# K-Wu/HET

Hardware: AMD Instinct MI355X
Metric: million edges/s (fwd+bwd) RGAT layer, ogbn-mag feat=64 (higher is better)
Workload: dtype f32; 1 GPU; RGAT layer fwd+bwd, ogbn-mag-shaped synthetic graph (N=1939743, E=21111007, R=4), feat=64, heads=4, self_loop, no optimizer step, layer flags: default; LAYER SWAP: the model script builds het_amd.layers.HET_RGATLayer (the reference's layer class name and arguments); swapping only hrt/python/backend or only kernels/__init__.py under the reference's own model code gives variants.op_by_op / variants.; edge_order=src_dst, device=AMD Radeon Graphics, torch=2.10.0+rocm7.0, hip=7.0.51831, parallelism=single GPU

## Files before the change

het_amd/_lib.py:

```python
from __future__ import annotations

import ctypes as C
import os

_HERE = os.path.dirname(os.path.abspath(__file__))
LIB_PATH = os.environ.get("HET_AMD_LIB") or os.path.join(_HERE, "libhet_amd.so")

P, I64, INT, DBL = C.c_void_p, C.c_int64, C.c_int, C.c_double

_SIGNATURES = {
    "het_grouping_create": [P, I64, P, I64, I64, P, P, P, C.POINTER(P)],
    "het_grouping_rank_of_position": [P, P, P],
    "het_grouping_segment_map": [P, I64, P, P],
    "het_grouping_gather_payload1": [P, P, I64, P, P],
    "het_rows_add_bias": [P, P, P, P, I64, I64, P],
    "het_rows_gather": [P, P, I64, I64, P, P],
    "het_rows_scatter_add": [P, P, I64, I64, P, P],
    "het_rows_scatter_add_grouped": [P, P, I64, P, I64, P],
    "het_layout_separate_coo": [P, P, P, P, I64, I64, I64, P, P, P, P, P],
    "het_layout_coo_to_csr": [P, P, P, P, I64, I64, P, P, P, P, P],
    "het_layout_transpose_csr": [P, P, P, P, I64, I64, I64, P, P, P, P, P],
    "het_layout_unique_rel_nodes": [P, I64, P, P, I64, I64, P, P, P, P, P],
    "het_rgnn_relational_matmul": [I64, P, I64, P, P, I64, P, P, P, I64, I64, I64, INT, P, P, I64, P],
    "het_backward_rgnn_relational_matmul_attn_dot_only": [P, I64, P, P, I64, I64, P, P, P, P, P, P, I64, I64, I64, INT, P, P, I64, P, P, P],
    "het_rgnn_relational_matmul_attn_dot": [I64, P, I64, P, P, I64, P, P, P, P, P, I64, I64, I64, P, P, I64, P, P, P],
    "het_backward_rgnn_relational_matmul": [I64, P, I64, P, P, I64, I64, P, P, P, P, P, I64, I64, I64, INT, INT, P, P, I64, P],
    "het_rgnn_relational_matmul_no_scatter_gather_list": [P, I64, I64, P, P, P, I64, I64, I64, INT, P],
    "het_backward_rgnn_relational_matmul_no_scatter_gather_list": [P, I64, I64, P, P, P, P, P, I64, I64, I64, INT, INT, P],
    "het_relational_fused_gat_separate_coo": [P, P, P, P, I64, I64, I64, I64, P, P, P, P, P, P, P, P, P, P, P, I64, I64, DBL, P, P, P, P],
    "het_backward_relational_fused_gat_separate_coo": [P, P, P, P, I64, I64, I64, I64, P, P, P, P, P, P, P, P, P, P, P, P, P, P, P, I64, I64, DBL, P, P, P, I64, I64, P, I64, P, P, P, P, P],
    "het_relational_fused_gat_csr": [P, P, P, P, I64, I64, P, P, I64, P, P, P, P, P, P, I64, I64, DBL, INT, P],
    "het_backward_relational_fused_gat_csr": [P, P, P, P, I64, I64, P, P, I64, P, P, P, P, P, P, P, P, P, P, I64, I64, DBL, INT, P],
    "het_hgt_fold_source_weights": [P, P, P, P, P, P, I64, I64, I64, I64, I64, INT, P, P],
    "het_hgt_fold_source_weights_backward": [P, P, P, P, P, P, P, I64, I64, I64, I64, I64, INT, P, P, P, P, P, P],
    "het_rgat_aggregate_compact": [P, P, P, P, P, P, I64, I64, I64, DBL, P, I64, P, I64, P],
    "het_rows_matmul_backward_dx": [P, I64, P, P, I64, P, P, P, I64, I64, I64, INT, P],
    "het_rows_matmul_backward_dw": [P, I64, P, P, I64, P, P, P, I64, I64, I64, INT, P],
    "het_rows_matmul_backward_dw_colsum": [P, I64, P, P, I64, P, P, P, P, I64, I64, I64, INT, P],
    "het_rows_linear_bias": [P, P, P, P, P, I64, I64, I64, P],
    "het_node_row_map": [P, I64, P, I64, I64, P, P],
    "het_rgat_node_backward_dx": [I64, I64, I64, I64, I64, P, P, P, P, P, P, P, P, P, I64, I64, I64, P, P],
    "het_node_rows_matmul_sum": [I64, I64, I64, I64, P, P, P, P, P, P, I64, I64, P, P],
    "het_node_rows_matmul_sum_bias": [I64, I64, I64, I64, P, P, P, P, P, P, P, I64, I64, P, P],
    "het_rgcn_layer_forward": [P, I64, I64, P, P, P, P, P, P, P, P, P, I64, I64, P],
    "het_rgcn_layer_backward": [P, P, I64, I64, I64, P, P, P, P, P, P, P, P, P, P, I64, I64, P, I64, P],
    "het_rgcn_layer_forward_bf16": [P, I64, I64, P, P, P, P, P, P, P, P, P, I64, I64, P],
    "het_rgcn_layer_backward_bf16": [P, P, I64, I64, I64, P, P, P, P, P, P, P, P, P, P, I64, I64, P, I64, P],
    "het_rgat_backward_compact": [P, P, P, P, P, P, P, P, P, P, P, P, P, I64, P, I64, I64, I64, I64, I64, I64, DBL, P, I64, P],
    "het_rgat_aggregate_compact_runs": [P, P, I64, P, P, P, P, P, I64, I64, I64, DBL, P, I64, P, P, P, I64, P, P, P, I64, P],
    "het_rgat_backward_compact_runs": [P, P, P, P, P, P, P, P, P, P, P, P, P, P, P, P, I64, P, I64, I64, I64, I64, I64, I64, DBL, P, P, I64, P],
    "het_hgt_aggregate_compact": [P, P, P, P, P, I64, I64, I64, I64, P, I64, P],
    "het_hgt_backward_compact": [P, P, P, P, P, P, P, P, P, I64, I64, I64, I64, P, I64, P],
    "het_hgt_aggregate_compact_bf16": [P, P, P, P, P, I64, I64, I64, I64, P, I64, P],
    "het_hgt_backward_compact_bf16": [P, P, P, P, P, P, P, P, P, I64, I64, I64, I64, P, I64, P],
    "het_rows_matmul_bf16": [P, I64, P, P, I64, P, P, P, I64, I64, P],
    "het_rows_matmul_backward_dw_bf16": [P, I64, P, P, I64, P, P, P, I64, I64, INT, P],
    "het_rows_matmul_backward_dw_bf16_bf16": [P, I64, P, P, I64, P, P, P, I64, I64, INT, P],
    "het_node_rows_matmul_sum_bf16": [I64, I64, I64, I64, P, P, P, P, P, P, I64, I64, P, P],
    "het_rgcn_layer1_separate_coo": [P, P, P, P, I64, I64, I64, P, P, P, P, I64, I64, P, P, I64, P],
    "het_backward_rgcn_layer1_separate_coo": [P, P, P, P, I64, I64, I64, P, P, P, P, P, P, P, I64, I64, P, P, I64, P],
    "het_rgcn_node_mean_aggregation_compact_as_of_node_separate_coo": [P, P, P, P, I64, I64, I64, P, P, P, P, P, I64, INT, P, P],
    "het_backward_rgcn_node_mean_aggregation_compact_as_of_node_separate_coo": [P, P, P, P, I64, I64, I64, P, P, P, P, P, P, P, I64, INT, P, I64, P],
    "het_hgt_full_graph_edge_softmax_ops_separate_coo": [P, P, P, P, I64, I64, I64, P, P, P, P, P, I64, P, P],
    "het_backward_hgt_full_graph_enorm_to_unnormalized_attn_score_separate_coo": [P, P, P, P, I64, I64, I64, P, P, P, P, P, P, P, I64, P, P],
    "het_hgt_full_graph_edge_softmax_ops_csr": [P, I64, P, P, P, I64, I64, P, P, P, P, P, I64, P, P],
    "het_hgt_full_graph_message_mean_aggregation_csr": [P, I64, P, P, P, I64, I64, P, P, P, P, P, I64, I64, P, P],
    "het_backward_hgt_full_graph_message_mean_aggregation_csr": [P, I64, P, P, P, I64, I64, P, P, P, P, I64, I64, P],
    "het_backward_hgt_full_graph_edge_softmax_ops_csr": [P, I64, P, P, P, I64, I64, I64, P, P, P, P, P, P, P, P, I64, I64, P, P],
    "het_backward_hgt_full_graph_enorm_to_unnormalized_attn_score_csr": [P, I64, P, P, P, I64, I64, I64, P, P, P, P, P, P, I64, P, P, I64, P],
    "het_hgt_full_graph_fused_message_calc_and_mean_aggregation_separate_coo": [P, P, P, P, I64, I64, I64, P, P, P, P, I64, I64, I64, P, P, I64, P],
    "het_backward_hgt_full_graph_fused_message_calc_and_mean_aggregation_separate_coo": [P, P, P, P, I64, I64, I64, P, P, P, P, P, P, P, P, I64, I64, I64, P, P, I64, P],
    "het_rgnn_inner_product_right_node_separatecoo": [I64, P, P, P, P, P, P, I64, I64, P, P, P, I64, I64, P],
    "het_backward_inner_product_right_node_separatecoo": [I64, P, P, P, P, P, P, I64, I64, P, P, P, P, P, I64, I64, INT, P, P, I64, I64, P],
    "het_hgt_full_graph_hetero_attention_ops_coo": [P, P, P, P, I64, I64, P, P, P, P, P, I64, I64, I64, P],
    "het_backward_hgt_full_graph_hetero_attention_ops_coo": [P, P, P, P, I64, I64, P, P, P, P, P, P, P, P, I64, I64, I64, P, P, I64, P, I64, P],
}


class HetError(RuntimeError):
    pass


class HetUnsupported(HetError, NotImplementedError):
    """A configuration of the reference's model code that this build names but does not implement (the message says which
    reference op it would need and what to use instead) -- raised where the reference's name is reached, instead of an
    AttributeError from a missing function."""


_lib = None


def lib() -> C.CDLL:
    global _lib
    if _lib is None:
        if not os.path.exists(LIB_PATH):
            raise HetError(
                f"{LIB_PATH} not found: build the HIP library first (python -c 'import __graft_entry__ as g; g.build()' "
                "or make -C het_amd/csrc). het_amd has no CPU fallback.")
        L = C.CDLL(LIB_PATH)
        L.het_build_info.restype = C.c_char_p
        L.het_last_error.restype = C.c_char_p
        L.het_grouping_destroy.argtypes = [P]
        L.het_grouping_destroy.restype = None
        L.het_grouping_note_stream.argtypes = [P, P]
        L.het_grouping_note_stream.restype = None
        L.het_grouping_num_segments.argtypes = [P]
        L.het_grouping_num_segments.restype = I64
        L.het_grouping_bytes.argtypes = [P]
        L.het_grouping_bytes.restype = I64
        L.het_rgat_aggregate_compact_workspace.argtypes = [P, I64, I64]
        L.het_rgat_aggregate_compact_workspace.restype = I64
        L.het_rgat_aggregate_compact_runs_workspace.argtypes = [P, P, I64, I64, I64, P]
        L.het_rgat_aggregate_compact_runs_workspace.restype = I64
        L.het_rgat_backward_compact_runs_workspace.argtypes = [P, I64, I64, I64, I64, INT, INT, P]
        L.het_rgat_backward_compact_runs_workspace.restype = I64
        L.het_rgat_backward_compact_workspace.argtypes = [I64, I64, I64, I64, INT]
        L.het_rgat_backward_compact_workspace.restype = I64
        L.het_hgt_aggregate_compact_workspace.argtypes = [P, I64, I64]
        L.het_hgt_aggregate_compact_workspace.restype = I64
        L.het_hgt_backward_compact_workspace.argtypes = [I64, I64]
        L.het_hgt_backward_compact_workspace.restype = I64
        L.het_hgt_compact_shape_ok.argtypes = [I64, I64]
        L.het_hgt_compact_shape_ok.restype = INT
        L.het_node_rows_matmul_sum_ok.argtypes = [I64, I64, I64]
        L.het_node_rows_matmul_sum_ok.restype = INT
        L.het_rgcn_layer_ok.argtypes = [I64, I64, I64]
        L.het_rgcn_layer_ok.restype = INT
        L.het_rgcn_layer_backward_workspace.argtypes = [I64, I64]
        L.het_rgcn_layer_backward_workspace.restype = I64
        L.het_rgat_node_gemm_ok.argtypes = [I64, I64, I64, I64]
        L.het_rgat_node_gemm_ok.restype = INT
        L.het_set_allocator.argtypes = [P, P, P]
        L.het_set_allocator.restype = INT
        L.het_allocator_is_external.argtypes = []
        L.het_allocator_is_external.restype = INT
        L.het_kernel_timing_enable.argtypes = [INT]
        L.het_kernel_timing_enable.restype = INT
        L.het_kernel_timing_read.argtypes = [C.c_char_p, C.POINTER(C.c_double), C.POINTER(I64)]
        L.het_kernel_timing_read.restype = INT
        for name, args in _SIGNATURES.items():
            f = getattr(L, name, None)
            if f is None:
                raise HetError(f"{LIB_PATH} does not export {name}: rebuild it (make -C het_amd/csrc)")
            f.argtypes = args
            f.restype = INT
        _lib = L
    return _lib


_ALLOC_FN = C.CFUNCTYPE(C.c_void_p, C.c_size_t, C.c_void_p, C.c_void_p)
_FREE_FN = C.CFUNCTYPE(None, C.c_void_p, C.c_void_p)
_alloc_cbs = None


def use_torch_allocator(on: bool = True) -> bool:
    global _alloc_cbs
    L = lib()
    if not on:
        L.het_set_allocator(None, None, None)
        return False
    import torch

    def _alloc(nbytes, stream, _user):
        try:
            return int(torch.cuda.caching_allocator_alloc(int(nbytes), stream=int(stream or 0)))
        except BaseException:
            return None

    def _free(ptr, _user):
        try:
            torch.cuda.caching_allocator_delete(int(ptr))
        except BaseException:
            pass

    cbs = (_ALLOC_FN(_alloc), _FREE_FN(_free))
    rc = L.het_set_allocator(C.cast(cbs[0], C.c_void_p), C.cast(cbs[1], C.c_void_p), None)
    if rc != 0:
        raise HetError(f"het_set_allocator failed (code {rc}): {L.het_last_error().decode()}")
    _alloc_cbs = (_alloc_cbs or ()) + (cbs,)
    return True


def allocator_is_external() -> bool:
    return bool(lib().het_allocator_is_external())


def call(name: str, *args) -> None:
    L = lib()
    rc = getattr(L, name)(*args)
    if rc != 0:
        raise HetError(f"{name} failed (code {rc}): {L.het_last_error().decode()}")


def kernel_timing(on: bool) -> None:
    rc = lib().het_kernel_timing_enable(int(bool(on)))
    if rc != 0:
        raise HetError(f"het_kernel_timing_enable failed (code {rc})")


def kernel_timing_read(prefix: str):
    L = lib()
    ms, n = C.c_double(0.0), C.c_int64(0)
    rc = L.het_kernel_timing_read(prefix.encode(), C.byref(ms), C.byref(n))
    if rc != 0:
        raise HetError(f"het_kernel_timing_read failed (code {rc}): {L.het_last_error().decode()}")
    return ms.value, n.value


def build_info() -> str:
    return lib().het_build_info().decode()
```

het_amd/backend/rgat_fused_layer.py:

```python
import os

import torch as th

from ..plan import consistent as _consistent_plan

from .. import kernels as _k
from ..kernels import K


_OFFS = {}
PER_EDGE = os.environ.get("HET_RGAT_PER_EDGE") == "1"
LITERAL_ER = os.environ.get("HET_RGAT_LITERAL_ER") == "1"
OVERLAP = os.environ.get("HET_RGAT_OVERLAP", "1") != "0"


def _mulfirst_shape_ok(H, Kd):
    return H in (1, 2, 4, 8) and Kd >= 4 * H and Kd & (Kd - 1) == 0 and Kd <= 256


def _has_single_sided_lists(g):
    return "unique_node_indices_single_sided" in getattr(g, "graph_data", {}).get("separate", {})


def effective_flags(g, W, compact, direct, mulfirst):
    R, H, Kd, D = W.shape
    if not compact and not PER_EDGE and (_has_single_sided_lists(g) or hasattr(g, "generate_separate_unique_node_indices_single_sided_for_each_etype")):
        compact, direct = True, True
    if not mulfirst and not LITERAL_ER and _mulfirst_shape_ok(H, Kd):
        mulfirst = True
    return bool(compact), bool(direct), bool(mulfirst)


def _destinations_below(col, nd):
    return col.numel() == 0 or _k._derived_get("col_max", (col,), lambda: int(col.max())) < nd


def _lists(g):
    s = g.get_separate_coo_original()
    by_src = {"separate_coo_rel_ptrs": s["rel_ptrs"], "separate_coo_node_indices": s["row_indices"], "separate_coo_eids": s["eids"]}
    by_dst = {"separate_coo_rel_ptrs": s["rel_ptrs"], "separate_coo_node_indices": s["col_indices"], "separate_coo_eids": s["eids"]}
    return s, by_src, by_dst


def _compact_dicts(g, direct):
    ss = g.get_separate_unique_node_indices_single_sided()
    if direct:
        inv = g.get_separate_unique_node_indices_single_sided_inverse_idx()
        d = {"edata_idx_to_inverse_idx_row": inv["inverse_indices_row"], "edata_idx_to_inverse_idx_col": inv["inverse_indices_col"]}
        return ss, 4, d, d
    fwd = {"unique_srcs_and_dests_rel_ptrs": ss["rel_ptrs_row"], "unique_srcs_and_dests_rel_ptrs_col": ss["rel_ptrs_col"],
           "unique_srcs_and_dests_node_indices_row": ss["node_indices_row"],
           "unique_srcs_and_dests_node_indices_col": ss["node_indices_col"]}
    bwd = {"unique_srcs_and_dests_rel_ptrs": ss["rel_ptrs_row"], "unique_srcs_and_dests_rel_col": ss["rel_ptrs_col"],
           "unique_srcs_and_dests_node_indices_row": ss["node_indices_row"],
           "unique_srcs_and_dests_node_indices_col": ss["node_indices_col"]}
    return ss, 3, fwd, bwd


def _edge_rows(g, ss, direct, rp, row, col, eids):
    sep = getattr(g, "graph_data", {}).get("separate", {}).get("unique_node_indices_single_sided", {})
    if "inverse_indices_row" in sep and getattr(g, "sequential_eids_format", None) == "separate_coo":
        return sep["inverse_indices_row"], sep["inverse_indices_col"]
    maps = (ss["rel_ptrs_row"], ss["node_indices_row"], ss["rel_ptrs_col"], ss["node_indices_col"])
    return _k._src_rows_by_position(3, maps, rp, row, eids), _k._dst_rows_by_position(3, maps, rp, col, eids)


def rgat_layer_fused_ok(g, x, W, slope, compact, mulfirst=False):
    R, H, Kd, D = W.shape
    if not (_k._plan.is_enabled() and x.is_cuda and x.dim() == 2 and slope >= 0 and g.get_num_edges() > 0
            and _k.gat_grouped_shape_ok(H, D)):
        return False
    compact, _, mulfirst_eff = effective_flags(g, W, compact, True, mulfirst)
    if mulfirst and not _mulfirst_shape_ok(H, Kd):
        return False
    mulfirst = mulfirst_eff
    if not _k.matmul_attn_dot_ok(H, Kd, D):
        return compact and mulfirst and H & (H - 1) == 0
    if compact or mulfirst:
        return True
    _, _, by_dst = _lists(g)
    return _k.matmul_attn_dot_only_ok(by_dst, W, x)


_SIDE = {}


def _side_stream(dev):
    s = _SIDE.get(dev)
    if s is None:
        s = _SIDE[dev] = th.cuda.Stream(device=dev)
    return s


def _halo_pieces(g, ss, plan):
    key = ("halo_pieces", plan.chunks, plan.n_own, plan.n_halo)
    hit = g._plans.get(key)
    if hit is None:
        rp_row, nodes = ss["rel_ptrs_row"], ss["node_indices_row"]
        R = rp_row.numel() - 1
        rel = th.repeat_interleave(th.arange(R, device=nodes.device), rp_row[1:] - rp_row[:-1])
        cuts = [(0, plan.n_own + plan.halo_chunk_ptr[1])] + [(plan.n_own + plan.halo_chunk_ptr[c], plan.n_own + plan.halo_chunk_ptr[c + 1])
                                                             for c in range(1, plan.chunks)]
        hit = []
        for a, b in cuts:
            sel = th.nonzero((nodes >= a) & (nodes < b)).flatten()
            rp_c = th.zeros(R + 1, dtype=th.int64, device=nodes.device)
            rp_c[1:] = th.cumsum(th.bincount(rel[sel], minlength=R), 0)
            hit.append((rp_c, nodes[sel].contiguous(), sel.contiguous()))
        assert sum(int(h[2].numel()) for h in hit) == nodes.numel()
        g._plans[key] = hit
    return hit


@_consistent_plan
class RgatLayerFunction(th.autograd.Function):
    @staticmethod
    def forward(ctx, g, compact, direct, mulfirst, slope, num_dst, halo, x, W, attn_l, attn_r, loop_w, bias):
        x, W, attn_l, attn_r = x.contiguous(), W.contiguous(), attn_l.contiguous(), attn_r.contiguous()
        if halo is not None:
            assert compact and mulfirst and loop_w is not None, "rgat_layer_halo_ok guards this path"
            x = halo.start_push(x)
        s, by_src, by_dst = _lists(g)
        rp, row, col, eids = s["rel_ptrs"], s["row_indices"], s["col_indices"], s["eids"]
        E, N = eids.numel(), x.shape[0]
        R, H, Kd, D = W.shape
        X = H * D
        new = lambda *shape: th.empty(shape, dtype=x.dtype, device=x.device)
        sm, ret = new(N, H), new(N, H, D)
        nd = N if num_dst is None else min(int(num_dst), N)
        offs = h = None
        if loop_w is not None:
            loop_w = loop_w.contiguous()
            offs = _OFFS.get((nd, x.device))
            if offs is None:
                if len(_OFFS) > 64:
                    _OFFS.clear()
                offs = _OFFS[(nd, x.device)] = th.tensor([0, nd], dtype=th.int64, device=x.device)
        wa = None
        if mulfirst:
            wa = th.bmm(W.view(-1, Kd, D), attn_r.view(-1, D, 1)).view(R, H, Kd, 1)
        if compact:
            ss = g.get_separate_unique_node_indices_single_sided()
            d_row = {"unique_srcs_and_dests_rel_ptrs": ss["rel_ptrs_row"], "unique_srcs_and_dests_node_indices": ss["node_indices_row"]}
            d_col = {"unique_srcs_and_dests_rel_ptrs": ss["rel_ptrs_col"], "unique_srcs_and_dests_node_indices": ss["node_indices_col"]}
            featc = new(ss["node_indices_row"].numel(), H, D)
            elc = new(featc.shape[0], H)
            erc = new(ss["node_indices_col"].numel(), H)
            side = None
            fused_loop = loop_w is not None and _k.rows_linear_bias_ok(Kd, X)
            if OVERLAP and halo is None and fused_loop and mulfirst:
                main, side = th.cuda.current_stream(x.device), _side_stream(x.device)
                h = x.new_empty((nd, X))
                side.wait_stream(main)
            if mulfirst:
                with th.cuda.stream(side if side is not None else th.cuda.current_stream(x.device)):
                    K.rgnn_relational_matmul(d_col, 1, wa, x, erc.view(-1, H, 1), True)
                saved = (featc, elc, erc)
            else:
                featd = new(erc.shape[0], H, D)
                _k.matmul_attn_dot(d_col, 1, W, x, featd, attn_r, erc)
                saved = (featc, elc, erc, featd)
            if fused_loop:
                bias_c = None if bias is None else bias.contiguous()
                if side is not None:
                    with th.cuda.stream(side):
                        _k.rows_linear_bias(offs, x[:nd], loop_w, bias_c, out=h)
                else:
                    h = _k.rows_linear_bias(offs, x[:nd], loop_w, bias_c)
            dot_ok = _k.matmul_attn_dot_ok(H, Kd, D)
            piecewise = halo is not None and halo.chunks > 1 and dot_ok
            if piecewise:
                for c, (rp_c, nodes_c, rows_c) in enumerate(_halo_pieces(g, ss, halo.plan)):
                    halo.wait_push_piece(c)
                    _k.matmul_attn_dot_rows(rp_c, nodes_c, rows_c, W, x, featc, attn_l, elc)
                halo.finish_push()
            elif halo is not None:
                halo.finish_push()
            if piecewise:
                pass
            elif dot_ok:
                _k.matmul_attn_dot(d_row, 1, W, x, featc, attn_l, elc)
            else:
                K.rgnn_relational_matmul(d_row, 1, W, x, featc, True)
                K.rgnn_relational_matmul_no_scatter_gather_list(ss["rel_ptrs_row"], attn_l.unsqueeze(-1), featc, elc.view(-1, H, 1))
            if side is not None:
                th.cuda.current_stream(x.device).wait_stream(side)
            srow, drow = _edge_rows(g, ss, direct, rp, row, col, eids)
            run_sums = _k.rgat_runs_shape_ok(H, D)
            grp = _k.rgat_compact_groupings(col, srow, drow, N, featc.shape[0], erc.shape[0], rel_ptrs=rp if run_sums else None,
                                            drow_nodes=ss["node_indices_col"], drow_rel_ptrs=ss["rel_ptrs_col"])
            ctx.runs = _k.rgat_aggregate_compact(grp, featc, elc, erc, sm, ret, slope, h_inout=h, num_rels=R,
                                                 attn_l=attn_l.contiguous() if run_sums else None, feat_rel_ptrs=ss["rel_ptrs_row"] if run_sums else None)
            ctx.grp = grp
            ex = x.new_empty(0)
        else:
            rank = _k.gat_rank_of_position(rp, row, col, eids, N)
            by_dst_s = {"separate_coo_rel_ptrs": rp, "separate_coo_node_indices": col, "separate_coo_eids": rank}
            feat, el_s, er_s, exs = new(E, H, D), new(E, H), new(E, H), new(E, H)
            _k.matmul_attn_dot(by_src, 0, W, x, feat, attn_l, el_s, dot_rows=rank)
            if mulfirst:
                K.rgnn_relational_matmul(by_dst_s, 0, wa, x, er_s.view(E, H, 1), True)
                saved = (feat, exs)
            else:
                comp = _k.matmul_attn_dot(by_dst_s, 0, W, x, None, attn_r, er_s)
                assert comp is not None
                saved = (feat, exs, comp)
            used = _k.fused_gat_forward(eids, rp, row, col, 0, {}, feat, None, None, sm, None, ret, slope, exs,
                                        el_sorted=el_s, er_sorted=er_s)
            assert used
            ex = x.new_empty(0)
        if h is None:
            out = ret.view(N, X)[:nd]
            loop = None
            if loop_w is not None:
                loop = new(nd, X)
                K.rgnn_relational_matmul_no_scatter_gather_list(offs, loop_w.view(1, 1, Kd, X), x[:nd], loop)
            h = _k.rows_add_bias(out, loop, None if bias is None else bias.contiguous()) if (loop is not None or bias is not None) else out.clone()
        ctx.halo = halo
        ctx.g, ctx.compact, ctx.mulfirst, ctx.slope, ctx.nd = g, compact, mulfirst, slope, nd
        ctx.has_loop, ctx.has_bias = loop_w is not None, bias is not None
        ctx.save_for_backward(x, W, attn_l, attn_r, loop_w if loop_w is not None else x.new_empty(0), offs if offs is not None else eids,
                              sm, ex, ret, *saved)
        return h

    @staticmethod
    def backward(ctx, grad_h):
        x, W, attn_l, attn_r, loop_w, offs, sm, ex, ret, *saved = ctx.saved_tensors
        g, nd, slope = ctx.g, ctx.nd, ctx.slope
        s, by_src, by_dst = _lists(g)
        rp, row, col, eids = s["rel_ptrs"], s["row_indices"], s["col_indices"], s["eids"]
        N, Kd = x.shape
        E = eids.numel()
        R, H, _, D = W.shape
        X = H * D
        grad_h = grad_h.contiguous()
        if ctx.halo is not None:
            return RgatLayerFunction._backward_with_halo(ctx, grad_h)
        grad_bias = grad_h.sum(0) if (ctx.has_bias and not ctx.compact) else None
        Wt = th.transpose(W, 2, 3).contiguous()
        if ctx.compact and ctx.mulfirst and _k.rgat_node_gemm_ok(R, H, Kd, D) and _destinations_below(col, nd):
            return RgatLayerFunction._backward_node_major(ctx, grad_h, Wt)
        grad_W = th.zeros_like(W)
        grad_loop = None
        if ctx.has_loop:
            grad_x = th.empty_like(x) if nd == N else th.zeros_like(x)
            grad_loop = th.empty_like(loop_w)
            _k.matmul_no_scatter_gather_backward(offs, loop_w.view(1, 1, Kd, X).transpose(2, 3).contiguous(), x[:nd], grad_h,
                                                 grad_x[:nd], grad_loop.view(1, 1, Kd, X), accumulate=False)
        else:
            grad_x = th.zeros_like(x)
        dst_prefix = ctx.compact and _destinations_below(col, nd)
        if nd == N or dst_prefix:
            go = grad_h.view(nd, H, D)
        else:
            go = th.zeros((N, H, D), dtype=x.dtype, device=x.device)
            go.view(N, X)[:nd] = grad_h
        ndp = nd if dst_prefix else N
        mulfirst = ctx.mulfirst
        if mulfirst:
            wa_t = th.bmm(W.view(-1, Kd, D), attn_r.view(-1, D, 1)).view(R, H, 1, Kd)
            grad_wa = th.zeros((R, H, Kd, 1), dtype=x.dtype, device=x.device)
        if ctx.compact:
            featc, elc, erc = saved[:3]
            featd = None if mulfirst else saved[3]
            ss = g.get_separate_unique_node_indices_single_sided()
            d_row = {"unique_srcs_and_dests_rel_ptrs": ss["rel_ptrs_row"], "unique_srcs_and_dests_node_indices": ss["node_indices_row"]}
            d_col = {"unique_srcs_and_dests_rel_ptrs": ss["rel_ptrs_col"], "unique_srcs_and_dests_node_indices": ss["node_indices_col"]}
            g_featc, g_elc, g_erc = th.empty_like(featc), th.empty_like(elc), th.empty_like(erc)
            if ctx.has_bias:
                grad_bias = th.empty(X, dtype=x.dtype, device=x.device)
            _k.rgat_backward_compact(ctx.grp, featc, elc, erc, sm[:ndp], ret[:ndp], go, g_featc, g_elc, g_erc, slope, fold_attn_l=attn_l,
                                     row_rel_ptrs=ss["rel_ptrs_row"], grad_bias=grad_bias if ctx.has_bias else None, bias_rows=nd,
                                     runs=ctx.runs, drow_nodes=ss["node_indices_col"])
            grad_attn_l, grad_attn_r = th.empty_like(attn_l), th.empty_like(attn_r)
            _k.matmul_no_scatter_gather_backward(ss["rel_ptrs_row"], attn_l.unsqueeze(2), featc, g_elc, None,
                                                 grad_attn_l.unsqueeze(-1), accumulate=False)
            _k.matmul_backward(d_row, 1, Wt, x, g_featc, grad_x, grad_W, True, accumulate=True, distinct_rows=True)
            if mulfirst:
                _k.matmul_backward(d_col, 1, wa_t, x, g_erc.view(-1, H, 1), grad_x, grad_wa, True, accumulate=True, distinct_rows=True)
            else:
                g_featd = th.empty_like(featd)
                _k.matmul_no_scatter_gather_backward(ss["rel_ptrs_col"], attn_r.unsqueeze(2), featd, g_erc, g_featd,
                                                     grad_attn_r.unsqueeze(-1), accumulate=False)
                _k.matmul_backward(d_col, 1, Wt, x, g_featd, grad_x, grad_W, True, accumulate=True, distinct_rows=True)
        else:
            feat, exs = saved[:2]
            rank = _k.gat_rank_of_position(rp, row, col, eids, N)
            by_dst = {"separate_coo_rel_ptrs": rp, "separate_coo_node_indices": col, "separate_coo_eids": rank}
            g_feat, g_el = th.empty_like(feat), th.empty_like(exs)
            grad_attn_l = th.zeros_like(attn_l)
            if R <= 8:
                _k.fused_gat_backward(eids, rp, row, col, 0, {}, feat, None, None, sm, None, ret, go, g_feat, None, None, slope,
                                      exs, fold_attn_l=attn_l, grad_fold_attn_l=grad_attn_l, grad_el_sorted=g_el)
            else:
                g_el_e = th.empty_like(exs)
                _k.fused_gat_backward(eids, rp, row, col, 0, {}, feat, None, None, sm, None, ret, go, g_feat, g_el_e, g_el_e, slope,
                                      exs, fold_attn_l=attn_l, grad_el_sorted=g_el)
                by_eid = {"separate_coo_rel_ptrs": rp, "separate_coo_node_indices": eids, "separate_coo_eids": eids}
                _k.matmul_backward(by_eid, 0, attn_l.unsqueeze(2), feat, g_el_e, None, grad_attn_l.unsqueeze(-1), False,
                                   accumulate=False)
            _k.matmul_backward(by_src, 0, Wt, x, g_feat, grad_x, grad_W, True, accumulate=True)
            if mulfirst:
                _k.matmul_backward(by_dst, 0, wa_t, x, g_el.view(E, H, 1), grad_x, grad_wa, True, accumulate=True)
            else:
                grad_attn_r = th.zeros_like(attn_r)
                ok = _k.matmul_attn_dot_only_backward(by_dst, Wt, x, attn_r, g_el, grad_x, grad_W, comp_rows=saved[2],
                                                      grad_dot_w=grad_attn_r, accumulate=True)
                assert ok, "the grouping of the forward pass is gone"
        if mulfirst:
            grad_W.addcmul_(grad_wa, attn_r.view(R, H, 1, D))
            grad_attn_r = (W * grad_wa).sum(2)
        return None, None, None, None, None, None, None, grad_x, grad_W, grad_attn_l, grad_attn_r, grad_loop, grad_bias


    @staticmethod
    def _backward_node_major(ctx, grad_h, Wt):
        x, W, attn_l, attn_r, loop_w, offs, sm, ex, ret, featc, elc, erc = ctx.saved_tensors
        g, nd, slope = ctx.g, ctx.nd, ctx.slope
        N, Kd = x.shape
        R, H, _, D = W.shape
        X = H * D
        ss = g.get_separate_unique_node_indices_single_sided()
        rp_row = ss["rel_ptrs_row"]
        row_map = _k.node_row_map(rp_row, ss["node_indices_row"], N)
        dst_map = _k.node_row_map(ss["rel_ptrs_col"], ss["node_indices_col"], N)
        go = grad_h.view(nd, H, D)
        attn_in_pass = ctx.runs is not None and R <= 8
        g_featc, g_erc = th.empty_like(featc), th.empty_like(erc)
        g_elc = None if attn_in_pass else th.empty_like(elc)
        grad_bias = th.empty(X, dtype=x.dtype, device=x.device) if ctx.has_bias else None
        grad_loop = th.empty_like(loop_w) if ctx.has_loop else None
        bias_in_dw = ctx.has_bias and ctx.has_loop
        main, side = th.cuda.current_stream(x.device), _side_stream(x.device) if OVERLAP else None
        if side is not None and ctx.has_loop:
            side.wait_stream(main)
            with th.cuda.stream(side):
                _k.rows_matmul_backward_dw(offs, None, x[:nd], grad_h, grad_loop.view(1, 1, Kd, X), accumulate=False,
                                           colsum=grad_bias if bias_in_dw else None)
        grad_attn_l = th.empty_like(attn_l)
        _k.rgat_backward_compact(ctx.grp, featc, elc, erc, sm[:nd], ret[:nd], go, g_featc, g_elc, g_erc, slope, fold_attn_l=attn_l,
                                 row_rel_ptrs=rp_row, grad_bias=None if bias_in_dw else grad_bias, bias_rows=nd, runs=ctx.runs,
                                 drow_nodes=ss["node_indices_col"], grad_attn_l=grad_attn_l if attn_in_pass else None)
        wa_t = th.bmm(W.view(-1, Kd, D), attn_r.view(-1, D, 1)).view(R, H, Kd)
        grad_x = th.empty_like(x)
        grad_W, grad_wa = th.empty_like(W), th.empty((R, H, Kd), dtype=x.dtype, device=x.device)
        gh = grad_h if ctx.has_loop else None
        loop_wt = loop_w.t().contiguous() if ctx.has_loop else None
        d_col = {"unique_srcs_and_dests_rel_ptrs": ss["rel_ptrs_col"], "unique_srcs_and_dests_node_indices": ss["node_indices_col"]}

        def weight_gradients():
            if not attn_in_pass:
                _k.matmul_no_scatter_gather_backward(rp_row, attn_l.unsqueeze(2), featc, g_elc, None, grad_attn_l.unsqueeze(-1),
                                                     accumulate=False)
            if ctx.has_loop and side is None:
                _k.rows_matmul_backward_dw(offs, None, x[:nd], grad_h, grad_loop.view(1, 1, Kd, X), accumulate=False,
                                           colsum=grad_bias if bias_in_dw else None)
            _k.rows_matmul_backward_dw(rp_row, ss["node_indices_row"], x, g_featc.view(-1, X), grad_W, accumulate=False)
            _k.matmul_backward(d_col, 1, wa_t.view(R, H, 1, Kd), x, g_erc.view(-1, H, 1), None, grad_wa.view(R, H, Kd, 1), True,
                               accumulate=False)

        order = _k.node_order_by_presence(row_map, dst_map, split=nd if nd < N else None)

        def input_gradient():
            _k.rgat_node_backward_dx(0, N, nd, gh, loop_wt, g_featc.view(-1, X), Wt, row_map, g_erc, wa_t, dst_map, grad_x,
                                     node_order=order)
        if side is not None:
            side.wait_stream(main)
            with th.cuda.stream(side):
                weight_gradients()
            input_gradient()
            main.wait_stream(side)
        else:
            input_gradient()
            weight_gradients()
        grad_W.addcmul_(grad_wa.unsqueeze(-1), attn_r.view(R, H, 1, D))
        grad_attn_r = (W * grad_wa.unsqueeze(-1)).sum(2)
        return None, None, None, None, None, None, None, grad_x, grad_W, grad_attn_l, grad_attn_r, grad_loop, grad_bias

    @staticmethod
    def _backward_with_halo(ctx, grad_h):
        x, W, attn_l, attn_r, loop_w, offs, sm, ex, ret, featc, elc, erc = ctx.saved_tensors
        g, nd, slope, halo = ctx.g, ctx.nd, ctx.slope, ctx.halo
        N, Kd = x.shape
        R, H, _, D = W.shape
        X = H * D
        ss = g.get_separate_unique_node_indices_single_sided()
        rp_row, rows_node = ss["rel_ptrs_row"], ss["node_indices_row"]
        d_col = {"unique_srcs_and_dests_rel_ptrs": ss["rel_ptrs_col"], "unique_srcs_and_dests_node_indices": ss["node_indices_col"]}
        Wt = th.transpose(W, 2, 3).contiguous()
        s_coo = g.get_separate_coo_original()
        assert _destinations_below(s_coo["col_indices"], nd), "a partition's edges point at owned nodes"
        go = grad_h.view(nd, H, D)
        g_featc, g_elc, g_erc = th.empty_like(featc), th.empty_like(elc), th.empty_like(erc)
        grad_bias = th.empty(X, dtype=x.dtype, device=x.device) if ctx.has_bias else None
        wa_t = th.bmm(W.view(-1, Kd, D), attn_r.view(-1, D, 1)).view(R, H, 1, Kd)
        grad_x = th.empty_like(x)
        grad_W, grad_loop = th.empty_like(W), th.empty_like(loop_w)
        grad_attn_l = th.empty_like(attn_l)
        node_major = _k.rgat_node_gemm_ok(R, H, Kd, D)
        main, side = th.cuda.current_stream(x.device), (_side_stream(x.device) if OVERLAP and x.is_cuda else None)
        bias_in_dw = ctx.has_bias
        if side is not None:
            side.wait_stream(main)
            with th.cuda.stream(side):
                _k.rows_matmul_backward_dw(offs, None, x[:nd], grad_h, grad_loop.view(1, 1, Kd, X), accumulate=False,
                                           colsum=grad_bias if bias_in_dw else None)
        if not node_major:
            grad_x[nd:].zero_()
            _k.rows_matmul_backward_dx(offs, None, loop_w.t().contiguous().view(1, 1, X, Kd), grad_h, grad_x[:nd], atomic=False)
        attn_in_pass = ctx.runs is not None and R <= 8 and x.is_cuda
        _k.rgat_backward_compact(ctx.grp, featc, elc, erc, sm[:nd], ret[:nd], go, g_featc, g_elc, g_erc, slope, fold_attn_l=attn_l,
                                 row_rel_ptrs=rp_row, grad_bias=None if bias_in_dw else grad_bias, bias_rows=nd, runs=ctx.runs,
                                 drow_nodes=ss["node_indices_col"], grad_attn_l=grad_attn_l if attn_in_pass else None)
        grad_wa = th.empty((R, H, Kd, 1), dtype=x.dtype, device=x.device) if node_major else th.zeros((R, H, Kd, 1), dtype=x.dtype, device=x.device)

        def weight_gradients():
            if side is None:
                _k.rows_matmul_backward_dw(offs, None, x[:nd], grad_h, grad_loop.view(1, 1, Kd, X), accumulate=False,
                                           colsum=grad_bias if bias_in_dw else None)
            _k.rows_matmul_backward_dw(rp_row, rows_node, x, g_featc.view(-1, X), grad_W, accumulate=False)
            if not attn_in_pass:
                _k.matmul_no_scatter_gather_backward(rp_row, attn_l.unsqueeze(2), featc, g_elc, None, grad_attn_l.unsqueeze(-1),
                                                     accumulate=False)
            if node_major:
                _k.matmul_backward(d_col, 1, wa_t, x, g_erc.view(-1, H, 1), None, grad_wa, True, accumulate=False)

        if node_major:
            row_map = _k.node_row_map(rp_row, rows_node, N)
            dst_map = _k.node_row_map(ss["rel_ptrs_col"], ss["node_indices_col"], N)
            loop_wt = loop_w.t().contiguous()
            order = _k.node_order_by_presence(row_map, dst_map, split=nd)
            args = (grad_h, loop_wt, g_featc.view(-1, X), Wt, row_map, g_erc, wa_t.view(R, H, Kd), dst_map, grad_x, order)
            _k.rgat_node_backward_dx(nd, N, nd, *args)
            halo.start_return(grad_x)
            if side is not None:
                side.wait_stream(main)
                with th.cuda.stream(side):
                    weight_gradients()
            _k.rgat_node_backward_dx(0, nd, nd, *args)
            if side is None:
                weight_gradients()
        else:
            _k.rows_matmul_backward_dx(rp_row, rows_node, Wt, g_featc.view(-1, X), grad_x, atomic=2)
            halo.start_return(grad_x)
            weight_gradients()
            _k.matmul_backward(d_col, 1, wa_t, x, g_erc.view(-1, H, 1), grad_x, grad_wa, True, accumulate=True, distinct_rows=True)
        if side is not None:
            main.wait_stream(side)
        grad_W.addcmul_(grad_wa, attn_r.view(R, H, 1, D))
        grad_attn_r = (W * grad_wa).sum(2)
        grad_own = halo.finish_return(grad_x[:nd])
        return None, None, None, None, None, None, None, grad_own, grad_W, grad_attn_l, grad_attn_r, grad_loop, grad_bias


def rgat_layer_halo_ok(g, x_own, W, slope, compact, mulfirst=False):
    R, H, Kd, D = W.shape
    if not rgat_layer_fused_ok(g, x_own, W, slope, compact, mulfirst):
        return False
    c, _, m = effective_flags(g, W, compact, True, mulfirst)
    return c and m and _k.rows_linear_bias_ok(Kd, H * D) and _k.rows_matmul_backward_split_ok(H, Kd, D)


def rgat_layer_fused(g, x, W, attn_l, attn_r, loop_w, bias, slope, compact, direct, num_dst=None, mulfirst=False, halo=None):
    compact, direct, mulfirst = effective_flags(g, W, compact, direct, mulfirst)
    if compact and not _has_single_sided_lists(g):
        g.generate_separate_unique_node_indices_single_sided_for_each_etype()
    return RgatLayerFunction.apply(g, compact, direct, mulfirst, float(slope), num_dst, halo, x, W, attn_l, attn_r, loop_w, bias)
```

het_amd/csrc/gat_compact.hip:

```cpp
#include <stdlib.h>

#include "coop.hip.h"
#include "fused_gat.hip.h"
#include "seg_reduce.hip.h"

namespace {

__device__ __forceinline__ float lrelu(float z, float slope) { return z > 0.f ? z : slope * z; }
__device__ __forceinline__ float lse_of(float m, float ssum) {
  const float L = m + __logf(ssum);
  return L == 0.f ? 1.17549435e-38f : L;
}

template <int LPR>
__global__ __launch_bounds__(kBlock) void HET_rgat_aggregate_compact(Items it, const int32_t* __restrict__ p_srow,
                                                                      const int32_t* __restrict__ p_drow,
                                                                      const float* __restrict__ feat,
                                                                      const float* __restrict__ el,
                                                                      const float* __restrict__ er,
                                                                      float* __restrict__ lse, float* __restrict__ ret,
                                                                      int H, int D, float slope, float* __restrict__ hio,
                                                                      int64_t hio_rows, float* __restrict__ part) {
  constexpr int EPW = 64 / LPR, U = 4;
  const int lane = threadIdx.x & 63;
// ... 752 lines not shown
      aq.x = fmaf(a.x, ci, aq.x); aq.y = fmaf(a.y, ci, aq.y); aq.z = fmaf(a.z, ci, aq.z); aq.w = fmaf(a.w, ci, aq.w);
      sq = fmaf(pp[2 * X + 2 * H + h], ci, sq);
    }
#pragma unroll
    for (int off = LPR; off < 64; off <<= 1) {
      aq.x += __shfl_xor(aq.x, off); aq.y += __shfl_xor(aq.y, off);
      aq.z += __shfl_xor(aq.z, off); aq.w += __shfl_xor(aq.w, off);
      sq += __shfl_xor(sq, off);
    }
    __syncthreads();
    if (slot == 0) { s_acc[wave][sub] = aq; s_sum[wave][sub] = sq; }
    __syncthreads();
    if (wave == 0 && slot == 0) {
      float4 t = s_acc[0][sub];
      float ts = s_sum[0][sub];
#pragma unroll
      for (int w = 1; w < NW; ++w) {
        const float4 a = s_acc[w][sub];
        t.x += a.x; t.y += a.y; t.z += a.z; t.w += a.w;
        ts += s_sum[w][sub];
      }
      const int64_t wrow = p_drow[it.seg_ptr[s2]];
      st4(qrow + wrow * X + x, t);
      if (x % D == 0) { qsum[wrow * H + h] = ts; qref[wrow * H + h] = L; }
    }
    i0 += n_items;
  }
}

template <int LPR>
__device__ __forceinline__ void ga_flush_atomic(float* __restrict__ out, int rel, int x, const float4& v) {
  float* p = out + (int64_t)rel * (LPR * 4) + x;
  atomic_add4(p, v);
}
template <int LPR>
__device__ __forceinline__ void ga_block_reduce(float4 ga, int rel, float* __restrict__ part, int* __restrict__ part_rel,
                                                float* __restrict__ out) {
  constexpr int X = LPR * 4, NW = kBlock / 64;
  __shared__ float sg[NW][X];
  __shared__ int sr[NW];
  const int lane = threadIdx.x & 63, wave = threadIdx.x >> 6, slot = lane / LPR, x = (lane % LPR) * 4;
  int r0 = rel;
#pragma unroll
  for (int off = LPR; off < 64; off <<= 1) r0 = max(r0, __shfl_xor(r0, off));
  if (rel >= 0 && rel != r0) {
    ga_flush_atomic<LPR>(out, rel, x, ga);
    ga = make_float4(0.f, 0.f, 0.f, 0.f);
  }
  if (rel < 0) ga = make_float4(0.f, 0.f, 0.f, 0.f);
#pragma unroll
  for (int off = LPR; off < 64; off <<= 1) {
    ga.x += __shfl_xor(ga.x, off); ga.y += __shfl_xor(ga.y, off);
    ga.z += __shfl_xor(ga.z, off); ga.w += __shfl_xor(ga.w, off);
  }
  if (slot == 0) st4(&sg[wave][x], ga);
  if (lane == 0) sr[wave] = r0;
  __syncthreads();
  if (wave == 0 && slot == 0) {
    int R0 = -1;
#pragma unroll
    for (int w = 0; w < NW; ++w) R0 = max(R0, sr[w]);
    float4 t = make_float4(0.f, 0.f, 0.f, 0.f);
#pragma unroll
    for (int w = 0; w < NW; ++w) {
      const float4 v = ld4(&sg[w][x]);
      if (sr[w] == R0) { t.x += v.x; t.y += v.y; t.z += v.z; t.w += v.w; }
      else if (sr[w] >= 0) ga_flush_atomic<LPR>(out, sr[w], x, v);
    }
    st4(part + (int64_t)blockIdx.x * X + x, t);
    if (lane == 0) part_rel[blockIdx.x] = R0;
  }
}
constexpr int kAttnFinishRows = 128;
__global__ __launch_bounds__(kBlock) void HET_rgat_attn_grad_finish(const float* __restrict__ part, const int* __restrict__ part_rel,
                                                                     int64_t P, int X, float* __restrict__ out) {
  const int x = threadIdx.x % X, sub = threadIdx.x / X, nsub = kBlock / X;
  constexpr int kRowsPerBlock = kAttnFinishRows;
  const int64_t p0 = (int64_t)blockIdx.x * kRowsPerBlock, p1 = p0 + kRowsPerBlock < P ? p0 + kRowsPerBlock : P;
  int cur = -1;
  float a = 0.f;
  for (int64_t p = p0 + sub; p < p1; p += nsub) {
    const int r = part_rel[p];
    if (r != cur) {
      if (cur >= 0) atomicAdd(out + (int64_t)cur * X + x, a);
      cur = r;
      a = 0.f;
    }
    if (r >= 0) a += part[p * X + x];
  }
  if (cur >= 0) atomicAdd(out + (int64_t)cur * X + x, a);
}

template <int LPR, int DL, bool GA, bool REC, bool W64>
__global__ __launch_bounds__(kBlock, GA ? 5 : 1) void HET_rgat_backward_src_coop(
    Packs pk, const int4* __restrict__ kp01, const float* __restrict__ feat,
    const float* __restrict__ el, const float* __restrict__ er, const float* __restrict__ pack2,
    const float* __restrict__ gradout, float* __restrict__ grad_feat, float* __restrict__ grad_el,
    float* __restrict__ tbuf, float slope, const float* __restrict__ fold_w,
    const idx_t* __restrict__ fold_row_rel_ptrs, int R, float* __restrict__ ga_part, int* __restrict__ ga_rel,
    float* __restrict__ ga_out) {
  constexpr int EPW = 64 / LPR, U = 4, X = LPR * 4, H = LPR / DL;
  constexpr int RS = het_log2_ce(LPR * 16), HS = het_log2_ce(H * 4);
  typedef typename OffSel<W64>::type O;
  static_assert(DL >= U, "a head needs at least U lanes");
  const int lane = threadIdx.x & 63;
  const int slot = lane / LPR, sub = lane % LPR, x = sub * 4, h = sub / DL, d = sub % DL;
  const O xb = (O)(sub * 16), hb = (O)(h * 4);
  const int dq = d < U ? d : U - 1;
  const int64_t pid = ((int64_t)blockIdx.x * (kBlock / 64) + (threadIdx.x >> 6)) * EPW + slot;
  if (!GA && pid >= pk.n) return;
  const int64_t pidc = pid < pk.n ? pid : pk.n - 1;
  const uint32_t pb = (uint32_t)pk.ptr[pidc];
  int b = (int)(pb & 0x7fffffffu), e = (int)((uint32_t)pk.ptr[pidc + 1] & 0x7fffffffu);
  if (!GA && (pb >> 31)) return;
  if (GA && (pid >= pk.n || (pb >> 31))) e = b;
  float4 ga = make_float4(0.f, 0.f, 0.f, 0.f);
  int jn = b + dq < e ? b + dq : e - 1;
  if (GA && jn < 0) jn = 0;
  int4 idn = kp01[jn];
  asm volatile("" ::"v"(idn.x), "v"(idn.y), "v"(idn.z), "v"(idn.w));
  int rel_cur = -1;
  float4 fcur = make_float4(0.f, 0.f, 0.f, 0.f), wcur = fcur, acc = fcur;
  float acc_el = 0.f;
  for (int j0 = b; j0 < e; j0 += U) {
    const int keyv = idn.x, dstv = idn.y, drowv = idn.z, tagv = idn.w;
    float zrv;
    float2 pkv;
    if (REC) {
      const float4 rv = ld4_at<O>(er, ((O)drowv << (HS + 2)) | (O)(h * 16));
      zrv = rv.x; pkv = make_float2(rv.y, rv.z);
    } else {
      zrv = ld1_at<O>(er, ((O)drowv << HS) | hb);
      pkv = ld2_at<O>(pack2, ((O)dstv << (HS + 1)) | (O)(h * 8));
    }
    const float zlv = ld1_at<O>(el, ((O)keyv << HS) | hb);
    int tag[U];
    float4 g[U], fl[U];
#pragma unroll
    for (int q = 0; q < U; ++q) tag[q] = head_bcast_i<DL>(tagv, q, lane);
#pragma unroll
    for (int q = 0; q < U; ++q) g[q] = ld4_at<O>(gradout, ((O)head_bcast_i<DL>(dstv, q, lane) << RS) | xb);
#pragma unroll
    for (int q = 0; q < U; ++q)
      if (j0 + q < e && (tag[q] & HET_TAG_FIRST_KEY)) fl[q] = ld4_at<O>(feat, ((O)head_bcast_i<DL>(keyv, q, lane) << RS) | xb);
    jn = j0 + U + dq < e ? j0 + U + dq : e - 1;
    idn = kp01[jn];
    const float zv = zlv + zrv;
    const float av = j0 + dq < e ? __expf(lrelu(zv, slope) - pkv.x) : 0.f;
    const float adv = av * (zv > 0.f ? 1.f : slope);
    asm volatile("" ::"v"(idn.x), "v"(idn.y), "v"(idn.z), "v"(idn.w));
    float tq[U];
#pragma unroll
    for (int q = 0; q < U; ++q) {
      const bool ok = j0 + q < e;
      if (ok && (tag[q] & HET_TAG_FIRST_KEY)) {
        fcur = fl[q];
        if (fold_w) {
          const int rel = tag[q] >> HET_TAG_REL_SHIFT;
          if (rel != rel_cur) {
            if (GA) {
              if (rel_cur >= 0) ga_flush_atomic<LPR>(ga_out, rel_cur, x, ga);
              ga = make_float4(0.f, 0.f, 0.f, 0.f);
            }
            wcur = ld4(fold_w + (int64_t)rel * X + x);
            rel_cur = rel;
          }
        }
      }
      const float a = head_bcast<DL>(av, q, lane), ad = head_bcast<DL>(adv, q, lane), gr = head_bcast<DL>(pkv.y, q, lane);
      acc.x = fmaf(a, g[q].x, acc.x); acc.y = fmaf(a, g[q].y, acc.y);
      acc.z = fmaf(a, g[q].z, acc.z); acc.w = fmaf(a, g[q].w, acc.w);
      const float dot = head_sum<DL>(dot4(g[q], fcur));
      const float t = ad * (dot - gr);
      tq[q] = t;
      acc_el += t;
      if (ok && (tag[q] & HET_TAG_LAST_KEY)) {
        const int u = head_bcast_i<DL>(keyv, q, lane);
        float4 o = acc;
        if (fold_w) {
          o.x = fmaf(acc_el, wcur.x, o.x); o.y = fmaf(acc_el, wcur.y, o.y);
          o.z = fmaf(acc_el, wcur.z, o.z); o.w = fmaf(acc_el, wcur.w, o.w);
        }
        st4_at<O>(grad_feat, ((O)u << RS) | xb, o);
        if (grad_el && d == 0) st1_at<O>(grad_el, ((O)u << HS) | hb, acc_el);
        if (GA) {
          ga.x = fmaf(acc_el, fcur.x, ga.x); ga.y = fmaf(acc_el, fcur.y, ga.y);
          ga.z = fmaf(acc_el, fcur.z, ga.z); ga.w = fmaf(acc_el, fcur.w, ga.w);
        }
        acc = make_float4(0.f, 0.f, 0.f, 0.f);
        acc_el = 0.f;
      }
    }
    if (tbuf) {
      float ts = tq[0];
#pragma unroll
      for (int q = 1; q < U; ++q) ts = d == q ? tq[q] : ts;
      if (d < U && j0 + d < e) tbuf[(int64_t)(j0 + d) * H + h] = ts;
    }
  }
  if (GA) ga_block_reduce<LPR>(ga, rel_cur, ga_part, ga_rel, ga_out);
}


template <int LPR, int DL, bool GA, bool REC, bool W64>
__global__ __launch_bounds__(kBlock) void HET_rgat_backward_src_long(
    Items it, const int32_t* __restrict__ long_items, int64_t num_long_items, const int2* __restrict__ p01,
    const float* __restrict__ feat, const float* __restrict__ el,
    const float* __restrict__ er, const float* __restrict__ pack2, const float* __restrict__ gradout,
    float* __restrict__ grad_feat, float* __restrict__ grad_el, float* __restrict__ tbuf, float slope,
    const float* __restrict__ fold_w, const idx_t* __restrict__ fold_row_rel_ptrs, int R, float* __restrict__ ga_part,
    int* __restrict__ ga_rel, float* __restrict__ ga_out) {
  constexpr int EPW = 64 / LPR, U = 4, X = LPR * 4, H = LPR / DL;
  constexpr int RS = het_log2_ce(LPR * 16), HS = het_log2_ce(H * 4);
  typedef typename OffSel<W64>::type O;
  static_assert(DL >= U, "a head needs at least U lanes");
  const int lane = threadIdx.x & 63;
  const int slot = lane / LPR, sub = lane % LPR, x = sub * 4, h = sub / DL, d = sub % DL;
  const O xb = (O)(sub * 16), hb = (O)(h * 4);
  const int dq = d < U ? d : U - 1;
  const int64_t wid = (int64_t)blockIdx.x * (kBlock / 64) + (threadIdx.x >> 6);
  if (wid >= num_long_items) {
    if (GA) ga_block_reduce<LPR>(make_float4(0.f, 0.f, 0.f, 0.f), -1, ga_part, ga_rel, ga_out);
    return;
  }
  const int item = long_items[wid];
  const int seg = it.seg[item], b = it.begin[item], e = it.end[item];
  int jn = b + slot + dq * EPW < e ? b + slot + dq * EPW : e - 1;
  int2 idn = p01[jn];
  const int64_t u = it.seg_key[seg];
  const bool whole = b == it.seg_ptr[seg] && e == it.seg_ptr[seg + 1];
  const float4 f = ld4(feat + u * X + x);
  const float zl = el[u * H + h];
  float4 acc = make_float4(0.f, 0.f, 0.f, 0.f);
  float acc_el = 0.f;
  for (int j0 = b + slot; j0 < e; j0 += EPW * U) {
    const int dstv = idn.x, drowv = idn.y;
    float zrv;
    float2 pkv;
    if (REC) {
      const float4 rv = ld4_at<O>(er, ((O)drowv << (HS + 2)) | (O)(h * 16));
      zrv = rv.x; pkv = make_float2(rv.y, rv.z);
    } else {
      zrv = ld1_at<O>(er, ((O)drowv << HS) | hb);
      pkv = ld2_at<O>(pack2, ((O)dstv << (HS + 1)) | (O)(h * 8));
    }
    float4 g[U];
#pragma unroll
    for (int q = 0; q < U; ++q) g[q] = ld4_at<O>(gradout, ((O)head_bcast_i<DL>(dstv, q, lane) << RS) | xb);
    jn = j0 + (U + dq) * EPW < e ? j0 + (U + dq) * EPW : e - 1;
    idn = p01[jn];
    const float zv = zl + zrv;
    const float av = j0 + dq * EPW < e ? __expf(lrelu(zv, slope) - pkv.x) : 0.f;
    const float adv = av * (zv > 0.f ? 1.f : slope);
    float tq[U];
#pragma unroll
    for (int q = 0; q < U; ++q) {
      const float a = head_bcast<DL>(av, q, lane), ad = head_bcast<DL>(adv, q, lane), gr = head_bcast<DL>(pkv.y, q, lane);
      acc.x = fmaf(a, g[q].x, acc.x); acc.y = fmaf(a, g[q].y, acc.y);
      acc.z = fmaf(a, g[q].z, acc.z); acc.w = fmaf(a, g[q].w, acc.w);
      const float dot = head_sum<DL>(dot4(g[q], f));
      tq[q] = ad * (dot - gr);
      acc_el += tq[q];
    }
    if (tbuf) {
      float ts = tq[0];
#pragma unroll
      for (int q = 1; q < U; ++q) ts = d == q ? tq[q] : ts;
      if (d < U && j0 + d * EPW < e) tbuf[(int64_t)(j0 + d * EPW) * H + h] = ts;
    }
  }
#pragma unroll
  for (int off = LPR; off < 64; off <<= 1) {
    acc.x += __shfl_xor(acc.x, off); acc.y += __shfl_xor(acc.y, off);
    acc.z += __shfl_xor(acc.z, off); acc.w += __shfl_xor(acc.w, off);
    acc_el += __shfl_xor(acc_el, off);
  }
  if (GA) {
    const int rel = find_segment(fold_row_rel_ptrs, R, (idx_t)u);
    const float s0 = slot == 0 ? acc_el : 0.f;
    ga_block_reduce<LPR>(make_float4(s0 * f.x, s0 * f.y, s0 * f.z, s0 * f.w), rel, ga_part, ga_rel, ga_out);
  }
  if (slot != 0) return;
  if (fold_w) {
    const float4 w = ld4(fold_w + (int64_t)find_segment(fold_row_rel_ptrs, R, (idx_t)u) * X + x);
    acc.x = fmaf(acc_el, w.x, acc.x); acc.y = fmaf(acc_el, w.y, acc.y);
    acc.z = fmaf(acc_el, w.z, acc.z); acc.w = fmaf(acc_el, w.w, acc.w);
  }
  float* gp = grad_feat + u * X + x;
  if (whole) {
    st4(gp, acc);
    if (grad_el && d == 0) grad_el[u * H + h] = acc_el;
  } else {
    atomic_add4(gp, acc);
    if (grad_el && d == 0) atomicAdd(&grad_el[u * H + h], acc_el);
  }
}

template <int LPR, int DL>
__global__ __launch_bounds__(kBlock) void HET_rgat_drow_pass(const float* __restrict__ er, const float* __restrict__ lse,
                                                              const float* __restrict__ ret, const float* __restrict__ gradout,
                                                              const float* __restrict__ qrow, const float* __restrict__ qsum,
                                                              const float* __restrict__ qref, const int64_t* __restrict__ drow_nodes,
                                                              const int32_t* __restrict__ order, int64_t n_rows,
                                                              float* __restrict__ rec4, float* __restrict__ grad_er) {
  constexpr int EPW = 64 / LPR, X = LPR * 4, H = LPR / DL, U = 2;
  const int lane = threadIdx.x & 63, wave = threadIdx.x >> 6;
  const int slot = lane / LPR, sub = lane % LPR, x = sub * 4, h = sub / DL, d = sub % DL;
  const int64_t w0 = (((int64_t)blockIdx.x * (kBlock / 64) + wave) * U) * EPW + slot;
  int64_t w[U], v[U];
  bool ok[U];
#pragma unroll
  for (int u = 0; u < U; ++u) {
    ok[u] = w0 + u * EPW < n_rows;
    const int64_t j = ok[u] ? w0 + u * EPW : n_rows - 1;
    w[u] = order ? (int64_t)order[j] : j;
    v[u] = drow_nodes[w[u]];
  }
  float4 g[U], r[U], q[U];
  float erv[U], ls[U], qs[U], rf[U];
#pragma unroll
  for (int u = 0; u < U; ++u) {
    g[u] = ld4(gradout + v[u] * X + x);
    r[u] = ld4(ret + v[u] * X + x);
    q[u] = ld4(qrow + w[u] * X + x);
    erv[u] = er[w[u] * H + h];
    ls[u] = lse[v[u] * H + h];
    qs[u] = qsum[w[u] * H + h];
    rf[u] = qref[w[u] * H + h];
  }
#pragma unroll
  for (int u = 0; u < U; ++u) {
    const float dr = head_sum<DL>(dot4(g[u], r[u])), dq = head_sum<DL>(dot4(g[u], q[u]));
    if (ok[u] && d == 0) {
      const bool has = qs[u] != 0.f;
      st4(rec4 + (w[u] * H + h) * 4, make_float4(erv[u], ls[u], has ? dr : 0.f, 0.f));
      grad_er[w[u] * H + h] = has ? __expf(rf[u] - ls[u]) * (dq - dr * qs[u]) : 0.f;
    }
  }
}

template <int LPR>
__global__ __launch_bounds__(kBlock) void HET_rgat_colsum_rows(const float* __restrict__ g, int64_t n, float* __restrict__ bias_part) {
  constexpr int EPW = 64 / LPR, X = LPR * 4, U = 4;
  const int lane = threadIdx.x & 63, wave = threadIdx.x >> 6;
  const int slot = lane / LPR, x = (lane % LPR) * 4;
  const int64_t step = (int64_t)gridDim.x * (kBlock / 64) * EPW * U;
  float4 bs = make_float4(0.f, 0.f, 0.f, 0.f);
  for (int64_t v0 = ((int64_t)blockIdx.x * (kBlock / 64) + wave) * EPW * U + slot; v0 < n; v0 += step) {
    float4 a[U];
#pragma unroll
    for (int u = 0; u < U; ++u) a[u] = v0 + u * EPW < n ? ld4(g + (v0 + u * EPW) * X + x) : make_float4(0.f, 0.f, 0.f, 0.f);
#pragma unroll
    for (int u = 0; u < U; ++u) { bs.x += a[u].x; bs.y += a[u].y; bs.z += a[u].z; bs.w += a[u].w; }
  }
#pragma unroll
  for (int off = LPR; off < 64; off <<= 1) {
    bs.x += __shfl_xor(bs.x, off); bs.y += __shfl_xor(bs.y, off);
    bs.z += __shfl_xor(bs.z, off); bs.w += __shfl_xor(bs.w, off);
  }
  if (slot == 0) st4(bias_part + ((int64_t)blockIdx.x * (kBlock / 64) + wave) * X + x, bs);
}

template <int LPR>
__global__ __launch_bounds__(kBlock) void HET_rgat_zero_long_rows(const int32_t* __restrict__ long_seg,
                                                                   const int32_t* __restrict__ seg_key, int64_t n,
                                                                   float* __restrict__ grad_feat, float* __restrict__ grad_el,
                                                                   int H) {
  constexpr int X = LPR * 4;
  const int64_t total = n * LPR;
  for (int64_t t = (int64_t)blockIdx.x * kBlock + threadIdx.x; t < total; t += (int64_t)gridDim.x * kBlock) {
    const int64_t k = t / LPR;
    const int sub = (int)(t - k * LPR);
    const int64_t u = seg_key[long_seg[k]];
    st4(grad_feat + u * X + sub * 4, make_float4(0.f, 0.f, 0.f, 0.f));
    if (grad_el && sub < H) grad_el[u * H + sub] = 0.f;
  }
}

}

static bool compact_shape_ok(int64_t H, int64_t D) {
  const int64_t X = H * D;
  return is_pow2(D) && D >= 4 && is_pow2(X) && X / 4 <= 64 && H <= X / 4;
}

extern "C" int64_t het_rgat_aggregate_compact_workspace(const het_grouping* by_dst, int64_t H, int64_t D) {
  if (!by_dst || by_dst->num_split == 0) return 0;
  return (int64_t)sizeof(float) * by_dst->num_items * (H * D + 2 * H);
}

extern "C" int het_rgat_aggregate_compact(const het_grouping* by_dst, const float* feat_c, const float* el_c,
                                          const float* er_c, float* sum, float* ret, int64_t num_nodes, int64_t H,
                                          int64_t D, double slope, float* h_inout, int64_t h_rows, void* workspace,
                                          int64_t workspace_bytes, het_stream stream) {
  const char* op = "het_rgat_aggregate_compact";
  hipStream_t s = (hipStream_t)stream;
  HET_REQUIRE(by_dst && sum && ret && num_nodes >= 0, "%s: null argument", op);
  if (!compact_shape_ok(H, D)) { het_set_error("%s: unsupported shape H=%lld D=%lld", op, (long long)H, (long long)D); return HET_ERR_UNSUPPORTED; }
  HET_REQUIRE(by_dst->R == 0 && by_dst->key_bound <= num_nodes && (by_dst->E == 0 || (by_dst->p0 && by_dst->p1 && feat_c && el_c && er_c)),
              "%s: by_dst must group the positions by destination with payload0 = feat row and payload1 = er row", op);
  const int64_t need = het_rgat_aggregate_compact_workspace(by_dst, H, D);
  HET_REQUIRE(need == 0 || (workspace && workspace_bytes >= need && aligned16(workspace)),
              "%s: a 16-byte aligned workspace of %lld bytes is needed (het_rgat_aggregate_compact_workspace)", op, (long long)need);
  const int64_t X = H * D;
  HET_HIP(hipMemsetAsync(sum, 0, sizeof(float) * num_nodes * H, s));
  if (!h_inout) HET_HIP(hipMemsetAsync(ret, 0, sizeof(float) * num_nodes * X, s));
  if (by_dst->E == 0) return HET_OK;
  const Items it = items_of(by_dst);
  const unsigned nb = (unsigned)ceil_div64(by_dst->num_items, kBlock / 64);
  float* part = static_cast<float*>(workspace);
  if (coop_shape_ok(H, D))
    if (int rc = grouping_packed_ids(by_dst, false, s)) return rc;
  {
    HET_KTIME("HET_rgat_aggregate", s);
    if (coop_shape_ok(H, D)) {
      HET_DISPATCH_COOP((int)(X / 4), (int)(D / 4),
                        hipLaunchKernelGGL((HET_rgat_aggregate_coop<LPR, DL>), dim3(nb), dim3(kBlock), 0, s, it, by_dst->p01,
                                           feat_c, el_c, er_c, sum, ret, (int)H, (float)slope, h_inout, h_rows, part));
    } else {
      HET_DISPATCH_LPR((int)(X / 4), hipLaunchKernelGGL(HET_rgat_aggregate_compact<LPR>, dim3(nb), dim3(kBlock), 0, s, it,
                                                        by_dst->p0, by_dst->p1, feat_c, el_c, er_c, sum, ret, (int)H, (int)D,
                                                        (float)slope, h_inout, h_rows, part));
    }
  }
  HET_LAUNCH_CHECK("HET_rgat_aggregate_compact");
  if (by_dst->num_split > 0) {
    const unsigned nbs = (unsigned)ceil_div64(by_dst->num_split, kBlock / 64);
    HET_DISPATCH_LPR((int)(X / 4), hipLaunchKernelGGL(HET_rgat_finish_split<LPR>, dim3(nbs), dim3(kBlock), 0, s, by_dst->split_seg,
                                                      by_dst->num_split, it, part, sum, ret, (int)H, (int)D, h_inout, h_rows));
    HET_LAUNCH_CHECK("HET_rgat_finish_split");
  }
  return HET_OK;
}

static int rgat_hub_min() {
  static const int v = [] {
    const char* e = getenv("HET_RGAT_HUB_MIN");
    const int t = e ? atoi(e) : 256;
    return t < HET_PACK_T ? HET_PACK_T : t;
  }();
  return v;
}

static int rgat_bwd_pack_t() {
  static const int v = [] {
    const char* e = getenv("HET_RGAT_BWD_PACK_T");
    const int t = e ? atoi(e) : 64;
    return t < 8 ? 8 : (t > 256 ? 256 : t);
  }();
  return v;
}

extern "C" int64_t het_rgat_aggregate_compact_runs_workspace(const het_grouping* by_dst, const het_grouping* by_dst_rel,
                                                             int64_t num_rels, int64_t H, int64_t D, het_stream stream) {
  if (!by_dst || !by_dst_rel || num_rels <= 0) return -1;
  if (grouping_hub_items(by_dst_rel, by_dst, (int)num_rels, rgat_hub_min(), (hipStream_t)stream) != HET_OK) return -1;
  return (int64_t)sizeof(float) * by_dst_rel->num_hub_items * (2 * H * D + 3 * H);
}

extern "C" int het_rgat_aggregate_compact_runs(const het_grouping* by_dst, const het_grouping* by_dst_rel, int64_t num_rels,
                                               const float* feat_c, const float* el_c, const float* er_c, float* sum, float* ret,
                                               int64_t num_nodes, int64_t H, int64_t D, double slope, float* h_inout,
                                               int64_t h_rows, float* q_rows, float* q_sum, float* q_ref, int64_t num_dst_rows,
                                               const float* attn_l, const int64_t* feat_rel_ptrs_host, void* workspace,
                                               int64_t workspace_bytes, het_stream stream) {
  const char* op = "het_rgat_aggregate_compact_runs";
  hipStream_t s = (hipStream_t)stream;
  HET_REQUIRE(by_dst && by_dst_rel && sum && ret && q_rows && q_sum && q_ref && num_nodes >= 0 && num_rels > 0, "%s: null argument", op);
  if (!compact_shape_ok(H, D) || !coop_shape_ok(H, D)) {
    het_set_error("%s: unsupported shape H=%lld D=%lld", op, (long long)H, (long long)D);
    return HET_ERR_UNSUPPORTED;
  }
  HET_REQUIRE(by_dst->R == 0 && by_dst->key_bound <= num_nodes && (by_dst->E == 0 || (by_dst->p0 && by_dst->p1 && feat_c && el_c && er_c)),
              "%s: by_dst must group the positions by destination with payload0 = feat row and payload1 = er row", op);
  HET_REQUIRE(by_dst_rel->R == 0 && by_dst_rel->E == by_dst->E && by_dst_rel->key_bound <= num_nodes * num_rels,
              "%s: by_dst_rel must group the same positions by destination * num_rels + relation", op);
  const int64_t need = het_rgat_aggregate_compact_runs_workspace(by_dst, by_dst_rel, num_rels, H, D, stream);
  if (need < 0) return HET_ERR_INVALID_ARG;
  HET_REQUIRE(need == 0 || (workspace && workspace_bytes >= need && aligned16(workspace)),
              "%s: a 16-byte aligned workspace of %lld bytes is needed (het_rgat_aggregate_compact_runs_workspace)", op, (long long)need);
  const int64_t X = H * D;
  HET_HIP(hipMemsetAsync(sum, 0, sizeof(float) * num_nodes * H, s));
  HET_HIP(hipMemsetAsync(q_sum, 0, sizeof(float) * num_dst_rows * H, s));
  if (!h_inout) HET_HIP(hipMemsetAsync(ret, 0, sizeof(float) * num_nodes * X, s));
  if (by_dst->E == 0) return HET_OK;
  if (int rc = grouping_packed_ids(by_dst, true, s)) return rc;
  if (by_dst_rel->num_hub_items > 0)
    if (int rc = grouping_packed_ids(by_dst, false, s)) return rc;
  float* part = static_cast<float*>(workspace);
  ElFold ef{};
  const bool elr = attn_l && feat_rel_ptrs_host && D == 16 && num_rels <= kElMaxRels &&
                   aligned16(attn_l);
  if (elr) {
    ef.attn = attn_l; ef.R = (int)num_rels;
    for (int k = 0; k < kElMaxRels - 1; ++k)
      ef.thr[k] = k + 1 < num_rels && feat_rel_ptrs_host[k + 1] < 0x7fffffffll ? (int)feat_rel_ptrs_host[k + 1] : 0x7fffffff;
  }
  if (int rc = grouping_tag_kp01(by_dst, 1, elr ? ef.thr : nullptr, s)) return rc;
  static const bool wide_env = [] { const char* v = getenv("HET_RGAT_WIDE_OFFSETS"); return v && v[0] == '1'; }();
  const bool w64 = wide_env || !(het_fits_u32(by_dst->key_bound, X * 4) && het_fits_u32(by_dst->p0_max + 1, X * 4) &&
                                 het_fits_u32(by_dst->p1_max + 1, X * 4));
  const int hio_rows32 = (int)(h_rows < 0 ? 0 : (h_rows > 0x7fffffffll ? 0x7fffffffll : h_rows));
  HetFork fk(s);
  {
    HET_KTIME("HET_rgat_aggregate_packs", s);
    Packs pk{by_dst->pack_ptr, by_dst->key_of_rank, by_dst->num_packs};
    const unsigned nb = (unsigned)ceil_div64(by_dst->num_packs, (int64_t)(kBlock / 64) * (64 / (X / 4)));
#define HET_PACKS_LAUNCH2(ELRV, WV)                                                                                                \
  hipLaunchKernelGGL((HET_rgat_aggregate_runs_packed<LPR, DL, ELRV, WV>), dim3(nb), dim3(kBlock), 0, s, pk, by_dst->kp01, feat_c,   \
                     el_c, er_c, sum, ret, (float)slope, h_inout, hio_rows32, q_rows, q_sum, q_ref, rgat_hub_min(), ef)
#define HET_PACKS_LAUNCH(ELRV) do { if (w64) { HET_PACKS_LAUNCH2(ELRV, true); } else { HET_PACKS_LAUNCH2(ELRV, false); } } while (0)
    if (elr) {
      switch (X / 4) {
        case 8: { constexpr int LPR = 8, DL = 4; HET_PACKS_LAUNCH(true); break; }
        case 16: { constexpr int LPR = 16, DL = 4; HET_PACKS_LAUNCH(true); break; }
        default: { constexpr int LPR = 32, DL = 4; HET_PACKS_LAUNCH(true); break; }
      }
    } else {
      HET_DISPATCH_COOP((int)(X / 4), (int)(D / 4), HET_PACKS_LAUNCH(false));
    }
#undef HET_PACKS_LAUNCH
#undef HET_PACKS_LAUNCH2
  }
  HET_LAUNCH_CHECK("HET_rgat_aggregate_runs_packed");
  if (by_dst_rel->num_hub_items > 0) {
    hipStream_t s2 = fk.side;
    const Items it = items_of(by_dst_rel);
    const int64_t n_hub = by_dst_rel->num_hub_items;
    {
      HET_KTIME("HET_rgat_aggregate_hubs", s2);
      const unsigned nbh = (unsigned)ceil_div64(n_hub, kBlock / 64);
#define HET_HUBS_LAUNCH2(ELRV, WV)                                                                                              \
  hipLaunchKernelGGL((HET_rgat_aggregate_hub_items<LPR, DL, ELRV, WV>), dim3(nbh), dim3(kBlock), 0, s2, it, by_dst_rel->hub_items,  \
                     by_dst_rel->hub_order, n_hub, by_dst->p01, feat_c, el_c, er_c,                 \
                     (float)slope, part, ef)
#define HET_HUBS_LAUNCH(ELRV) do { if (w64) { HET_HUBS_LAUNCH2(ELRV, true); } else { HET_HUBS_LAUNCH2(ELRV, false); } } while (0)
      if (elr) {
        switch (X / 4) {
          case 8: { constexpr int LPR = 8, DL = 4; HET_HUBS_LAUNCH(true); break; }
          case 16: { constexpr int LPR = 16, DL = 4; HET_HUBS_LAUNCH(true); break; }
          default: { constexpr int LPR = 32, DL = 4; HET_HUBS_LAUNCH(true); break; }
        }
      } else {
        HET_DISPATCH_COOP((int)(X / 4), (int)(D / 4), HET_HUBS_LAUNCH(false));
      }
#undef HET_HUBS_LAUNCH
#undef HET_HUBS_LAUNCH2
    }
    HET_LAUNCH_CHECK("HET_rgat_aggregate_hub_items");
    const unsigned nbs = (unsigned)by_dst_rel->num_hub_segs;
    {
    HET_KTIME("HET_rgat_aggregate_finish", s2);
    HET_DISPATCH_LPR((int)(X / 4), hipLaunchKernelGGL(HET_rgat_finish_hubs<LPR>, dim3(nbs), dim3(kBlock), 0, s2, by_dst_rel->hub_rec,
                                                      by_dst_rel->num_hub_segs, it, by_dst->p1, part, sum, ret, (int)H, (int)D,
                                                      h_inout, h_rows, q_rows, q_sum, q_ref));
    }
    HET_LAUNCH_CHECK("HET_rgat_finish_hubs");
  }
  HET_HIP(fk.join());
  return HET_OK;
}

extern "C" int64_t het_rgat_backward_compact_workspace(int64_t num_nodes, int64_t num_edges, int64_t H, int64_t D, int with_bias) {
  const int64_t n_pack = (num_nodes * 2 * H + 3) / 4 * 4, n_tbuf = (num_edges * H + 3) / 4 * 4;
  return (int64_t)sizeof(float) * (n_pack + n_tbuf + (with_bias ? (int64_t)2048 * (kBlock / 64) * H * D : 0));
}

struct RunSums {
  const float *q_rows, *q_sum, *q_ref;
  const int64_t* drow_nodes;
};
static int64_t attn_grad_partial_rows(const PackView& pv, int64_t X) {
  const int64_t nb = ceil_div64(pv.num_packs, (int64_t)(kBlock / 64) * (64 / (X / 4)));
  const int64_t nbl = ceil_div64(pv.num_long_items, kBlock / 64);
  return nb + nbl;
}

static int rgat_backward_compact_impl(const char* op, const het_grouping* by_srow, const het_grouping* by_drow, const RunSums* runs,
                                      float* grad_attn_l, const float* feat_c, const float* el_c, const float* er_c, const float* sum, const float* ret,
                                      const float* gradout, float* grad_feat_c, float* grad_el_c, float* grad_er_c,
                                      const float* fold_attn_l, const int64_t* row_rel_ptrs, int64_t num_rels,
                                      float* grad_bias, int64_t bias_rows, int64_t num_nodes, int64_t num_src_rows,
                                      int64_t num_dst_rows, int64_t H, int64_t D, double slope, void* workspace,
                                      int64_t workspace_bytes, het_stream stream) {
  hipStream_t s = (hipStream_t)stream;
  HET_REQUIRE(by_srow && (by_drow || runs) && sum && ret && gradout && grad_feat_c && grad_er_c, "%s: null argument", op);
  HET_REQUIRE(grad_el_c || (runs && fold_attn_l && grad_attn_l && coop_shape_ok(H, D)),
              "%s: grad_el_c may only be NULL in the run-sum form with fold_attn_l and grad_attn_l (cooperative shapes)", op);
  if (!compact_shape_ok(H, D) || !segment_rows_supported((int)H) || slope < 0 || (runs && !coop_shape_ok(H, D))) {
    het_set_error("%s: unsupported shape H=%lld D=%lld (or slope < 0)", op, (long long)H, (long long)D);
    return HET_ERR_UNSUPPORTED;
  }
  const int64_t E = by_srow->E, X = H * D;
  HET_REQUIRE(by_srow->R == 0 && by_srow->key_bound <= num_src_rows && (E == 0 || (by_srow->p0 && by_srow->p1)),
              "%s: by_srow groups the positions by feat row (payload0 = destination, payload1 = er row)", op);
  HET_REQUIRE(runs || (by_drow->R == 0 && by_drow->E == E && by_drow->S == num_dst_rows && (E == 0 || by_drow->p0)),
              "%s: by_drow groups the positions by er row with payload0 = their rank in by_srow and has one segment per er row", op);
  HET_REQUIRE(!fold_attn_l || (row_rel_ptrs && num_rels > 0), "%s: fold_attn_l needs the relation pointers of the feat rows", op);
  const bool coop = coop_shape_ok(H, D);
  HET_REQUIRE(!grad_attn_l || (coop && fold_attn_l && num_rels <= 8), "%s: grad_attn_l needs the cooperative shapes, fold_attn_l and <= 8 relations", op);
  PackView pv;
  if (int rc = grouping_pack_view(by_srow, s, rgat_bwd_pack_t(), &pv)) return rc;
  constexpr int kBiasBlocks = 2048;
  const int64_t bias_part_rows = grad_bias ? (int64_t)kBiasBlocks * (kBlock / 64) : 0;
  const int64_t ga_rows = (grad_attn_l && E > 0) ? attn_grad_partial_rows(pv, X) : 0, n_ga = (ga_rows * (X + 1) + 3) / 4 * 4;
  const int64_t n_pack = (num_nodes * 2 * H + 3) / 4 * 4, n_tbuf = runs ? 0 : (E * H + 3) / 4 * 4;
  const bool use_rec = runs && E > 0 && num_dst_rows > 0;
  const int64_t n_rec = runs ? num_dst_rows * H * 4 : 0;
  const int64_t need = (int64_t)sizeof(float) * (n_pack + n_tbuf + bias_part_rows * X + n_ga + n_rec);
  HET_REQUIRE(workspace && workspace_bytes >= need && aligned16(workspace),
              "%s: a 16-byte aligned workspace of %lld bytes is needed (het_rgat_backward_compact_workspace)", op, (long long)need);
  float* pack = (float*)workspace;
  float* tbuf = runs ? nullptr : pack + n_pack;
  float* bias_part = grad_bias ? pack + n_pack + n_tbuf : nullptr;
  float* ga_part = ga_rows ? pack + n_pack + n_tbuf + bias_part_rows * X : nullptr;
  int* ga_rel = ga_rows ? reinterpret_cast<int*>(ga_part + ga_rows * X) : nullptr;
  float* rec4 = use_rec ? pack + n_pack + n_tbuf + bias_part_rows * X + n_ga : nullptr;
  if (grad_attn_l) HET_HIP(hipMemsetAsync(grad_attn_l, 0, sizeof(float) * num_rels * X, s));
  if (by_srow->S != num_src_rows) {
    HET_HIP(hipMemsetAsync(grad_feat_c, 0, sizeof(float) * num_src_rows * X, s));
    if (grad_el_c) HET_HIP(hipMemsetAsync(grad_el_c, 0, sizeof(float) * num_src_rows * H, s));
  }
  if (num_nodes > 0 && !use_rec) {
    const unsigned nbp = grad_bias ? kBiasBlocks : grid_for(num_nodes * (X / 4));
    {
      HET_KTIME("HET_rgat_backward_dst_pack", s);
      HET_DISPATCH_LPR((int)(X / 4), hipLaunchKernelGGL(HET_rgat_dst_pack<LPR>, dim3(nbp), dim3(kBlock), 0, s, sum, ret, gradout,
                                                        pack, num_nodes, (int)H, (int)D, bias_part, bias_rows, (int)coop));
    }
    HET_LAUNCH_CHECK("HET_rgat_dst_pack");
  } else if (grad_bias && num_nodes <= 0) {
    HET_HIP(hipMemsetAsync(grad_bias, 0, sizeof(float) * X, s));
  }
  if (E == 0) {
    if (grad_bias && num_nodes > 0) {
      hipLaunchKernelGGL(HET_rgat_colsum_finish, dim3((unsigned)X), dim3(kBlock), 0, s, bias_part, bias_part_rows, (int)X, grad_bias);
      HET_LAUNCH_CHECK("HET_rgat_colsum_finish");
    }
    HET_HIP(hipMemsetAsync(grad_er_c, 0, sizeof(float) * num_dst_rows * H, s));
    return HET_OK;
  }
  Packs pk{pv.pack_ptr, by_srow->key_of_rank, pv.num_packs};
  const unsigned nb = (unsigned)ceil_div64(pv.num_packs, (int64_t)(kBlock / 64) * (64 / (X / 4)));
  if (use_rec) {
    if (int rc = grouping_value_order(by_srow, runs->drow_nodes, num_dst_rows, s)) return rc;
    HET_KTIME("HET_rgat_backward_drow_pass", s);
    const unsigned nbd = (unsigned)ceil_div64(num_dst_rows, (int64_t)(kBlock / 64) * (64 / (X / 4)) * 2);
    HET_DISPATCH_COOP((int)(X / 4), (int)(D / 4),
                      hipLaunchKernelGGL((HET_rgat_drow_pass<LPR, DL>), dim3(nbd), dim3(kBlock), 0, s, er_c, sum, ret, gradout,
                                         runs->q_rows, runs->q_sum, runs->q_ref, runs->drow_nodes, by_srow->val_order, num_dst_rows, rec4,
                                         grad_er_c));
    HET_LAUNCH_CHECK("HET_rgat_drow_pass");
  }
  const float* er_arg = use_rec ? rec4 : er_c;
  bool w64 = true;
  if (coop) {
    if (int rc = grouping_packed_ids(by_srow, true, s)) return rc;
    if (pv.num_long_items > 0)
      if (int rc = grouping_packed_ids(by_srow, false, s)) return rc;
    if (fold_attn_l) {
      if (int rc = grouping_tag_kp01_dev(by_srow, 0, row_rel_ptrs, (int)num_rels, s)) return rc;
    } else {
      if (int rc = grouping_tag_kp01(by_srow, 0, nullptr, s)) return rc;
    }
    static const bool wide_env = [] { const char* v = getenv("HET_RGAT_WIDE_OFFSETS"); return v && v[0] == '1'; }();
    w64 = wide_env || !(het_fits_u32(num_src_rows, X * 4) && het_fits_u32(by_srow->p0_max + 1, X * 4) &&
                        het_fits_u32(by_srow->p1_max + 1, H * 16) && het_fits_u32(by_srow->p1_max + 1, X * 4));
  }
  HetFork fk(s);
  hipStream_t s2 = fk.side;
  if (grad_bias && num_nodes > 0) {
    if (use_rec) {
      HET_DISPATCH_LPR((int)(X / 4), hipLaunchKernelGGL(HET_rgat_colsum_rows<LPR>, dim3(kBiasBlocks), dim3(kBlock), 0, s2, gradout,
                                                        bias_rows < num_nodes ? bias_rows : num_nodes, bias_part));
      HET_LAUNCH_CHECK("HET_rgat_colsum_rows");
    }
    hipLaunchKernelGGL(HET_rgat_colsum_finish, dim3((unsigned)X), dim3(kBlock), 0, s2, bias_part, bias_part_rows, (int)X, grad_bias);
    HET_LAUNCH_CHECK("HET_rgat_colsum_finish");
  }
  if (by_srow->num_split > 0) {
    HET_DISPATCH_LPR((int)(X / 4), hipLaunchKernelGGL(HET_rgat_zero_long_rows<LPR>, dim3(grid_for(by_srow->num_split * (X / 4))),
                                                      dim3(kBlock), 0, s2, by_srow->split_seg, by_srow->seg_key, by_srow->num_split,
                                                      grad_feat_c, grad_el_c, (int)H));
    HET_LAUNCH_CHECK("HET_rgat_zero_long_rows");
  }
  if (coop) {
    {
      HET_KTIME("HET_rgat_backward_src_short", s);
#define HET_SRC_COOP2(GA_, REC_, W_, gp_, gr_, go_)                                                                              \
  HET_DISPATCH_COOP((int)(X / 4), (int)(D / 4),                                                                                 \
                    hipLaunchKernelGGL((HET_rgat_backward_src_coop<LPR, DL, GA_, REC_, W_>), dim3(nb), dim3(kBlock), 0, s, pk,   \
                                       by_srow->kp01, feat_c, el_c, er_arg, pack, gradout, grad_feat_c, grad_el_c, tbuf,         \
                                       (float)slope, fold_attn_l, row_rel_ptrs, (int)num_rels, gp_, gr_, go_))
#define HET_SRC_COOP(GA_, REC_, gp_, gr_, go_) \
  do { if (w64) { HET_SRC_COOP2(GA_, REC_, true, gp_, gr_, go_); } else { HET_SRC_COOP2(GA_, REC_, false, gp_, gr_, go_); } } while (0)
      if (ga_rows) {
        if (use_rec) { HET_SRC_COOP(true, true, ga_part, ga_rel, grad_attn_l); } else { HET_SRC_COOP(true, false, ga_part, ga_rel, grad_attn_l); }
      } else {
        if (use_rec) { HET_SRC_COOP(false, true, nullptr, nullptr, nullptr); } else { HET_SRC_COOP(false, false, nullptr, nullptr, nullptr); }
      }
#undef HET_SRC_COOP
#undef HET_SRC_COOP2
    }
    HET_LAUNCH_CHECK("HET_rgat_backward_src_coop");
    if (pv.num_long_items > 0) {
      const Items it = items_of(by_srow);
      const unsigned nbl = (unsigned)ceil_div64(pv.num_long_items, kBlock / 64);
      int* ga_rel_long = ga_rel ? ga_rel + nb : nullptr;
      HET_KTIME("HET_rgat_backward_src_long", s2);
#define HET_SRC_LONG2(GA_, REC_, W_, gp_, gr_, go_)                                                                              \
  HET_DISPATCH_COOP((int)(X / 4), (int)(D / 4),                                                                                 \
                    hipLaunchKernelGGL((HET_rgat_backward_src_long<LPR, DL, GA_, REC_, W_>), dim3(nbl), dim3(kBlock), 0, s2, it, \
                                       pv.long_items, pv.num_long_items, by_srow->p01, feat_c, el_c, er_arg, pack,   \
                                       gradout, grad_feat_c, grad_el_c, tbuf, (float)slope, fold_attn_l, row_rel_ptrs,           \
                                       (int)num_rels, gp_, gr_, go_))
#define HET_SRC_LONG(GA_, REC_, gp_, gr_, go_) \
  do { if (w64) { HET_SRC_LONG2(GA_, REC_, true, gp_, gr_, go_); } else { HET_SRC_LONG2(GA_, REC_, false, gp_, gr_, go_); } } while (0)
      if (ga_rows) {
        if (use_rec) { HET_SRC_LONG(true, true, ga_part + (int64_t)nb * X, ga_rel_long, grad_attn_l); }
        else { HET_SRC_LONG(true, false, ga_part + (int64_t)nb * X, ga_rel_long, grad_attn_l); }
      } else {
        if (use_rec) { HET_SRC_LONG(false, true, nullptr, nullptr, nullptr); } else { HET_SRC_LONG(false, false, nullptr, nullptr, nullptr); }
      }
#undef HET_SRC_LONG
#undef HET_SRC_LONG2
    }
  } else {
    const int skip_long = pv.num_long_items > 0 ? 1 : 0;
    {
      HET_KTIME("HET_rgat_backward_src_short", s);
      HET_DISPATCH_LPR((int)(X / 4),
                       hipLaunchKernelGGL((HET_rgat_backward_src_packed<LPR, 4>), dim3(nb), dim3(kBlock), 0, s, pk, by_srow->p0,
                                          by_srow->p1, feat_c, el_c, er_c, pack, gradout, grad_feat_c, grad_el_c, tbuf, (int)H,
                                          (int)D, (float)slope, fold_attn_l, row_rel_ptrs, (int)num_rels, skip_long));
    }
    if (skip_long) {
      HET_LAUNCH_CHECK("HET_rgat_backward_src_packed");
      const Items it = items_of(by_srow);
      const unsigned nbl = (unsigned)ceil_div64(pv.num_long_items, kBlock / 64);
      HET_KTIME("HET_rgat_backward_src_long", s2);
      HET_DISPATCH_LPR((int)(X / 4),
                       hipLaunchKernelGGL(HET_rgat_backward_src_long_any<LPR>, dim3(nbl), dim3(kBlock), 0, s2, it, pv.long_items,
                                          pv.num_long_items, by_srow->p0, by_srow->p1, feat_c, el_c, er_c, pack, gradout,
                                          grad_feat_c, grad_el_c, tbuf, (int)H, (int)D, (float)slope, fold_attn_l, row_rel_ptrs,
                                          (int)num_rels));
    }
  }
  HET_LAUNCH_CHECK("HET_rgat_backward_src_packed");
  HET_HIP(fk.join());
  if (ga_rows) {
    hipLaunchKernelGGL(HET_rgat_attn_grad_finish, dim3((unsigned)ceil_div64(ga_rows, kAttnFinishRows)), dim3(kBlock), 0, s, ga_part, ga_rel, ga_rows,
                       (int)X, grad_attn_l);
    HET_LAUNCH_CHECK("HET_rgat_attn_grad_finish");
  }
  if (runs) return HET_OK;
  return launch_segment_sum(by_drow, tbuf, grad_er_c, (int)H, nullptr, s);
}

extern "C" int het_rgat_backward_compact(const het_grouping* by_srow, const het_grouping* by_drow, const float* feat_c,
                                         const float* el_c, const float* er_c, const float* sum, const float* ret,
                                         const float* gradout, float* grad_feat_c, float* grad_el_c, float* grad_er_c,
                                         const float* fold_attn_l, const int64_t* row_rel_ptrs, int64_t num_rels,
                                         float* grad_bias, int64_t bias_rows, int64_t num_nodes, int64_t num_src_rows,
                                         int64_t num_dst_rows, int64_t H, int64_t D, double slope, void* workspace,
                                         int64_t workspace_bytes, het_stream stream) {
  HET_REQUIRE(by_drow, "het_rgat_backward_compact: null argument");
  return rgat_backward_compact_impl("het_rgat_backward_compact", by_srow, by_drow, nullptr, nullptr, feat_c, el_c, er_c, sum, ret, gradout,
                                    grad_feat_c, grad_el_c, grad_er_c, fold_attn_l, row_rel_ptrs, num_rels, grad_bias, bias_rows,
                                    num_nodes, num_src_rows, num_dst_rows, H, D, slope, workspace, workspace_bytes, stream);
}

extern "C" int64_t het_rgat_backward_compact_runs_workspace(const het_grouping* by_srow, int64_t num_nodes, int64_t num_dst_rows,
                                                            int64_t H, int64_t D, int with_bias, int with_attn_grad,
                                                            het_stream stream) {
  if (!by_srow || num_dst_rows < 0) return -1;
  int64_t bytes = het_rgat_backward_compact_workspace(num_nodes, 0, H, D, with_bias);
  if (coop_shape_ok(H, D)) bytes += (int64_t)sizeof(float) * num_dst_rows * H * 4;
  if (with_attn_grad && by_srow->E > 0) {
    PackView pv;
    if (grouping_pack_view(by_srow, (hipStream_t)stream, rgat_bwd_pack_t(), &pv) != HET_OK) return -1;
    bytes += (int64_t)sizeof(float) * ((attn_grad_partial_rows(pv, H * D) * (H * D + 1) + 3) / 4 * 4);
  }
  return bytes;
}

extern "C" int het_rgat_backward_compact_runs(const het_grouping* by_srow, const float* q_rows, const float* q_sum, const float* q_ref,
                                              const int64_t* drow_nodes, const float* feat_c, const float* el_c, const float* er_c,
                                              const float* sum, const float* ret, const float* gradout, float* grad_feat_c,
                                              float* grad_el_c, float* grad_er_c, const float* fold_attn_l,
                                              const int64_t* row_rel_ptrs, int64_t num_rels, float* grad_bias, int64_t bias_rows,
                                              int64_t num_nodes, int64_t num_src_rows, int64_t num_dst_rows, int64_t H, int64_t D,
                                              double slope, float* grad_attn_l, void* workspace, int64_t workspace_bytes,
                                              het_stream stream) {
  HET_REQUIRE(q_rows && q_sum && q_ref && (drow_nodes || num_dst_rows == 0), "het_rgat_backward_compact_runs: null argument");
  const RunSums runs{q_rows, q_sum, q_ref, drow_nodes};
  return rgat_backward_compact_impl("het_rgat_backward_compact_runs", by_srow, nullptr, &runs, grad_attn_l, feat_c, el_c, er_c, sum, ret, gradout,
                                    grad_feat_c, grad_el_c, grad_er_c, fold_attn_l, row_rel_ptrs, num_rels, grad_bias, bias_rows,
                                    num_nodes, num_src_rows, num_dst_rows, H, D, slope, workspace, workspace_bytes, stream);
}
```

het_amd/kernels.py:

```python
from __future__ import annotations

import ctypes as C
from collections import OrderedDict
from typing import Dict, List, Optional

import torch

from . import _lib, graph as _graph, plan as _plan

Tensor = torch.Tensor
NAMESPACE = "torch_hrt"
import os as _os
COMPILED_LIB = _os.environ.get("HET_TORCH_HRT_LIB") or None
if COMPILED_LIB:
    torch.ops.load_library(COMPILED_LIB)
    _libdef = None
else:
    _libdef = torch.library.Library(NAMESPACE, "DEF")
_registered: List[str] = []
if _os.environ.get("HET_TORCH_ALLOCATOR", "1") != "0" and torch.cuda.is_available():
    _lib.use_torch_allocator()


def _p(t: Optional[Tensor]):
# ... 296 lines not shown


def matmul_no_scatter_gather_backward(ntype_offset_ptrs, weights_transposed, inputs, gradout, grad_input, grad_weights,
                                      accumulate: bool):
    _chk("backward_rgnn_relational_matmul_no_scatter_gather_list",
         tuple(t for t in (weights_transposed, inputs, gradout, grad_input, grad_weights) if t is not None), (ntype_offset_ptrs,))
    T, H, D, K = weights_transposed.shape
    n = inputs.shape[0]
    per_head = int(H > 1 and inputs.numel() == n * H * K)
    _call(gradout, "het_backward_rgnn_relational_matmul_no_scatter_gather_list", _p(ntype_offset_ptrs), T, n,
          _p(weights_transposed), _p(inputs), _p(gradout), _p(grad_input), _p(grad_weights), H, K, D, per_head,
          int(accumulate), _stream(gradout))


def _gat_maps(kind: int, d: Dict[str, Tensor], backward: bool):
    if kind == 0:
        return None, None, None, None
    if kind == 1:
        rp, nodes = d["unique_srcs_and_dests_rel_ptrs"], d["unique_srcs_and_dests_node_indices"]
        return rp, nodes, rp, nodes
    if kind == 3:
        rpc = d.get("unique_srcs_and_dests_rel_ptrs_col")
        if rpc is None:
            rpc = d["unique_srcs_and_dests_rel_col"]
        return (d["unique_srcs_and_dests_rel_ptrs"], d["unique_srcs_and_dests_node_indices_row"], rpc,
                d["unique_srcs_and_dests_node_indices_col"])
    if kind == 4:
        return d["edata_idx_to_inverse_idx_row"], None, d["edata_idx_to_inverse_idx_col"], None
    if kind == 2:
        m = d["edata_idx_to_inverse_idx"]
        return m, None, m, None
    raise _lib.HetError(f"relational_fused_gat: CompactAsOfNodeKind {kind} is not supported")


_derived: "OrderedDict[tuple, tuple]" = OrderedDict()
_DERIVED_MAX = 64
import threading as _threading
_derived_lock = _threading.RLock()


def _derived_get(tag, tensors, build):
    key = (tag,) + tuple(_plan._ident(t) for t in tensors)
    with _derived_lock:
        hit = _derived.get(key)
        if hit is None:
            hit = (build(), tensors)
            _derived[key] = hit
            while len(_derived) > _DERIVED_MAX:
                _derived.popitem(last=False)
        else:
            _derived.move_to_end(key)
        return hit[0]


def _rows_by_search(rel_ptrs, nodes, ua, ub):
    R = rel_ptrs.numel() - 1
    bound = int(max(int(nodes.max().item()), int(ub.max().item()))) + 1
    rel_e = torch.repeat_interleave(torch.arange(R, device=nodes.device), rel_ptrs[1:] - rel_ptrs[:-1])
    rel_u = torch.repeat_interleave(torch.arange(R, device=nodes.device), ua[1:] - ua[:-1])
    return torch.searchsorted(rel_u * bound + ub, rel_e * bound + nodes).contiguous()


def _gat_direct(kind, maps, rel_ptrs, row, col, eids):
    if kind == 2:
        return 4, maps
    if kind not in (1, 3) or not _plan.is_enabled() or eids.numel() == 0:
        return kind, maps

    def build():
        srow = _src_rows_by_position(kind, maps, rel_ptrs, row, eids)
        drow = _dst_rows_by_position(kind, maps, rel_ptrs, col, eids)
        n = int(eids.max().item()) + 1
        mr = torch.empty(n, dtype=torch.int64, device=eids.device)
        mc = torch.empty(n, dtype=torch.int64, device=eids.device)
        mr[eids] = srow
        mc[eids] = drow
        return (mr, None, mc, None)

    return 4, _derived_get(("gatmap", kind), (maps[0], maps[1], maps[2], maps[3], rel_ptrs, row, col, eids), build)


def _src_rows_by_position(kind, maps, rel_ptrs, row, eids):
    ra, rb = maps[0], maps[1]
    if kind == 4:
        return _derived_get("srow4", (ra, eids), lambda: ra[eids].contiguous())
    return _derived_get("srow", (ra, rb, rel_ptrs, row), lambda: _rows_by_search(rel_ptrs, row, ra, rb))


def _dst_rows_by_position(kind, maps, rel_ptrs, col, eids):
    ca, cb = maps[2], maps[3]
    if kind == 4:
        return _derived_get("drow4", (ca, eids), lambda: ca[eids].contiguous())
    return _derived_get("drow", (ca, cb, rel_ptrs, col), lambda: _rows_by_search(rel_ptrs, col, ca, cb))


def _csr_compact_maps(row_ptrs, col, eids, reltypes, uniq_rel_ptrs, uniq_nodes, rows_are_dst: bool):
    def build():
        E = eids.numel()
        rows = _graph.csr_to_coo_rows(row_ptrs).contiguous()
        src, dst = (col, rows) if rows_are_dst else (rows, col)
        R = uniq_rel_ptrs.numel() - 1
        bound = int(max(int(row_ptrs.numel()) - 1, int(uniq_nodes.max().item()) + 1 if uniq_nodes.numel() else 1))
        rel_u = torch.repeat_interleave(torch.arange(R, device=col.device), uniq_rel_ptrs[1:] - uniq_rel_ptrs[:-1])
        keys = rel_u * bound + uniq_nodes
        n = int(eids.max().item()) + 1 if E else 0
        mr = torch.empty(n, dtype=torch.int64, device=col.device)
        mc = torch.empty(n, dtype=torch.int64, device=col.device)
        mr[eids] = torch.searchsorted(keys, reltypes * bound + src)
        mc[eids] = torch.searchsorted(keys, reltypes * bound + dst)
        return rows, {"edata_idx_to_inverse_idx_row": mr, "edata_idx_to_inverse_idx_col": mc}
    return _derived_get(("csrcompact", rows_are_dst), (row_ptrs, col, eids, reltypes, uniq_rel_ptrs, uniq_nodes), build)


def _csr_expanded_rows(row_ptrs, num_edges):
    return _derived_get(("csr", num_edges), (row_ptrs,),
                        lambda: (_graph.csr_to_coo_rows(row_ptrs).contiguous(),
                                 torch.tensor([0, num_edges], dtype=torch.int64, device=row_ptrs.device)))


def _rel_by_position(rel_ptrs, num_positions):
    R = rel_ptrs.numel() - 1
    return _derived_get(("rel", num_positions), (rel_ptrs,),
                        lambda: torch.repeat_interleave(torch.arange(R, device=rel_ptrs.device), rel_ptrs[1:] - rel_ptrs[:-1],
                                                        output_size=num_positions).contiguous())


def _by_dst(kind, maps, rel_ptrs, row, col, eids, num_nodes):
    if not _plan.is_enabled():
        return None
    p1 = _rel_by_position(rel_ptrs, eids.numel()) if kind == 0 else _src_rows_by_position(kind, maps, rel_ptrs, row, eids)
    return _plan.get_grouping(None, col, num_nodes, eids, p1)


@_op("relational_fused_gat_separate_coo(Tensor separate_coo_eids, Tensor separate_coo_rel_ptrs, "
     "Tensor separate_coo_row_indices, Tensor separate_coo_col_indices, int IntKind, "
     "Dict(str, Tensor) args_tensor_dict, Tensor feat_src, Tensor el, Tensor er, Tensor(a!) sum, Tensor(b!) exp, "
     "Tensor(c!) ret, float slope) -> ()")
def relational_fused_gat_separate_coo(separate_coo_eids, separate_coo_rel_ptrs, separate_coo_row_indices,
                                      separate_coo_col_indices, IntKind, args_tensor_dict, feat_src, el, er, sum, exp,
                                      ret, slope):
    exs = None
    if (A5_SORTED_STREAM and IntKind == 0 and slope >= 0 and _plan.is_enabled() and separate_coo_eids.numel() > 0 and exp.dim() >= 2
            and gat_grouped_shape_ok(sum.shape[1], ret.numel() // max(1, ret.shape[0] * sum.shape[1]))):
        exs = torch.empty((separate_coo_eids.numel(), sum.shape[1]), dtype=exp.dtype, device=exp.device)
    wrote = fused_gat_forward(separate_coo_eids, separate_coo_rel_ptrs, separate_coo_row_indices, separate_coo_col_indices,
                              IntKind, args_tensor_dict, feat_src, el, er, sum, exp, ret, slope, exs)
    _sorted_stream_put(exp, el, er, separate_coo_eids, separate_coo_col_indices, float(slope), exs if wrote else None)


def gat_grouped_shape_ok(H: int, D: int) -> bool:
    X = H * D
    return D >= 4 and D & (D - 1) == 0 and X & (X - 1) == 0 and X // 4 <= 64


def fused_gat_forward(separate_coo_eids, separate_coo_rel_ptrs, separate_coo_row_indices, separate_coo_col_indices,
                      IntKind, args_tensor_dict, feat_src, el, er, sum, exp, ret, slope, exp_sorted, el_sorted=None,
                      er_sorted=None):
    name = "relational_fused_gat_separate_coo"
    maps = _gat_maps(IntKind, args_tensor_dict, False)
    _chk(name, tuple(t for t in (feat_src, el, er, sum, exp, ret, el_sorted, er_sorted) if t is not None),
         (separate_coo_eids, separate_coo_rel_ptrs, separate_coo_row_indices, separate_coo_col_indices)
         + tuple(m for m in maps if m is not None))
    IntKind, maps = _gat_direct(IntKind, maps, separate_coo_rel_ptrs, separate_coo_row_indices, separate_coo_col_indices,
                                separate_coo_eids)
    E, N, H = separate_coo_eids.numel(), ret.shape[0], sum.shape[1]
    D = feat_src.numel() // (feat_src.shape[0] * H) if feat_src.numel() else ret.numel() // max(1, N * H)
    g = _by_dst(IntKind, maps, separate_coo_rel_ptrs, separate_coo_row_indices, separate_coo_col_indices,
                separate_coo_eids, N)
    _call(ret, "het_relational_fused_gat_separate_coo", _p(separate_coo_eids), _p(separate_coo_rel_ptrs),
          _p(separate_coo_row_indices), _p(separate_coo_col_indices), separate_coo_rel_ptrs.numel() - 1, E, N, IntKind,
          _p(maps[0]), _p(maps[1]), _p(maps[2]), _p(maps[3]), _p(feat_src), _p(el), _p(er), _p(sum), _p(exp), _p(ret),
          None if g is None else _p(exp_sorted), H, D, float(slope), None if g is None else g.handle, _p(el_sorted),
          _p(er_sorted), _stream(ret))
    return g is not None and exp_sorted is not None



import weakref as _weakref
A5_SORTED_STREAM = _os.environ.get("HET_A5_SORTED_STREAM", "1") != "0"
_sorted_streams: "OrderedDict[tuple, tuple]" = OrderedDict()
_SORTED_STREAMS_MAX = 2
sorted_stream_hits = 0


def _sorted_stream_key(exp, el, er, eids, col, slope):
    return (_plan._ident(exp)[:2], _plan._ident(el), _plan._ident(er), _plan._ident(eids), _plan._ident(col), slope, exp.device.index)


def _sorted_stream_put(exp, el, er, eids, col, slope, exs):
    key = _sorted_stream_key(exp, el, er, eids, col, slope)
    with _derived_lock:
        _sorted_streams.pop(key, None)
        if exs is not None:
            _sorted_streams[key] = (exs, exp._version, tuple(_weakref.ref(t) for t in (exp, el, er)))
            while len(_sorted_streams) > _SORTED_STREAMS_MAX:
                _sorted_streams.popitem(last=False)


def _sorted_stream_get(exp, el, er, eids, col, slope):
    global sorted_stream_hits
    if not (A5_SORTED_STREAM and _plan.is_enabled()) or exp is None or el is None or er is None:
        return None
    with _derived_lock:
        hit = _sorted_streams.get(_sorted_stream_key(exp, el, er, eids, col, slope))
        if hit is None:
            return None
        exs, version, refs = hit
        if exp._version != version or any(r() is None for r in refs):
            return None
        sorted_stream_hits += 1
        return exs


@_op("backward_relational_fused_gat_separate_coo(Tensor separate_coo_eids, Tensor separate_coo_rel_ptrs, "
     "Tensor separate_coo_row_indices, Tensor separate_coo_col_indices, int IntKind, "
     "Dict(str, Tensor) args_tensor_dict, Tensor feat_src, Tensor el, Tensor er, Tensor sum, Tensor exp, Tensor ret, "
     "Tensor gradout, Tensor(a!) grad_feat_src, Tensor(b!) grad_el, Tensor(c!) grad_er, float slope) -> ()")
def backward_relational_fused_gat_separate_coo(separate_coo_eids, separate_coo_rel_ptrs, separate_coo_row_indices,
                                               separate_coo_col_indices, IntKind, args_tensor_dict, feat_src, el, er,
                                               sum, exp, ret, gradout, grad_feat_src, grad_el, grad_er, slope):
    exs = _sorted_stream_get(exp, el, er, separate_coo_eids, separate_coo_col_indices, float(slope)) if IntKind == 0 else None
    fused_gat_backward(separate_coo_eids, separate_coo_rel_ptrs, separate_coo_row_indices, separate_coo_col_indices,
                       IntKind, args_tensor_dict, feat_src, el, er, sum, exp, ret, gradout, grad_feat_src, grad_el,
                       grad_er, slope, exs)


def fused_gat_backward(separate_coo_eids, separate_coo_rel_ptrs, separate_coo_row_indices, separate_coo_col_indices,
                       IntKind, args_tensor_dict, feat_src, el, er, sum, exp, ret, gradout, grad_feat_src, grad_el,
                       grad_er, slope, exp_sorted, fold_attn_l=None, grad_fold_attn_l=None, fold_row_rel_ptrs=None,
                       grad_el_sorted=None):
    name = "backward_relational_fused_gat_separate_coo"
    maps = _gat_maps(IntKind, args_tensor_dict, True)
    _chk(name, tuple(t for t in (feat_src, el, er, sum, exp, ret, gradout, grad_feat_src, grad_el, grad_er, grad_el_sorted,
                                 exp_sorted) if t is not None),
         (separate_coo_eids, separate_coo_rel_ptrs, separate_coo_row_indices, separate_coo_col_indices)
         + tuple(m for m in maps if m is not None))
    IntKind, maps = _gat_direct(IntKind, maps, separate_coo_rel_ptrs, separate_coo_row_indices, separate_coo_col_indices,
                                separate_coo_eids)
    E, N, H = separate_coo_eids.numel(), ret.shape[0], sum.shape[1]
    D = ret.numel() // max(1, N * H)
    g = _by_dst(0, maps, separate_coo_rel_ptrs, separate_coo_row_indices, separate_coo_col_indices,
                separate_coo_eids, N) if IntKind == 0 else None
    gs = gd = ws = None
    if IntKind != 0 and _plan.is_enabled() and slope >= 0 and gat_grouped_shape_ok(H, D) and E > 0:
        srow = _src_rows_by_position(IntKind, maps, separate_coo_rel_ptrs, separate_coo_row_indices, separate_coo_eids)
        drow = _dst_rows_by_position(IntKind, maps, separate_coo_rel_ptrs, separate_coo_col_indices, separate_coo_eids)
        gs = _plan.get_grouping(None, srow, feat_src.shape[0], separate_coo_eids, separate_coo_col_indices)
        gd = _plan.get_grouping(None, drow, er.shape[0], separate_coo_eids, None)
        ws = torch.empty(N * 2 * H + E * H, dtype=torch.float32, device=ret.device)
    if IntKind == 0 and g is not None and grad_fold_attn_l is not None:
        ws = torch.empty(64 * grad_fold_attn_l.numel(), dtype=torch.float32, device=ret.device)
    _call(ret, "het_backward_relational_fused_gat_separate_coo", _p(separate_coo_eids), _p(separate_coo_rel_ptrs),
          _p(separate_coo_row_indices), _p(separate_coo_col_indices), separate_coo_rel_ptrs.numel() - 1, E, N, IntKind,
          _p(maps[0]), _p(maps[1]), _p(maps[2]), _p(maps[3]), _p(feat_src), _p(el), _p(er), _p(sum), _p(exp), _p(ret),
          None if g is None else _p(exp_sorted), _p(gradout), _p(grad_feat_src), _p(grad_el), _p(grad_er), H, D,
          float(slope), None if g is None else g.handle, None if gs is None else gs.handle,
          None if gd is None else gd.handle, feat_src.shape[0], E if er is None else er.shape[0], _p(ws), 0 if ws is None else ws.numel() * 4,
          None if fold_attn_l is None else _p(fold_attn_l), None if grad_fold_attn_l is None else _p(grad_fold_attn_l),
          None if fold_row_rel_ptrs is None else _p(fold_row_rel_ptrs), _p(grad_el_sorted), _stream(ret))


def grouping_rank_of_position(g):
    r = getattr(g, "rank_of_position", None)
    if r is None:
        keys = g._keep[1]
        r = torch.empty(keys.numel(), dtype=torch.int64, device=keys.device)
        _call(r, "het_grouping_rank_of_position", g.handle, _p(r), _stream(r))
        g.rank_of_position = r
    return r


def rgat_runs_shape_ok(H: int, D: int) -> bool:
    X = H * D
    return X in (32, 64, 128) and D >= 16 and D & (D - 1) == 0 and X % D == 0


def rgat_compact_groupings(col, srow, drow, num_nodes, num_src_rows, num_dst_rows, rel_ptrs=None, drow_nodes=None,
                           drow_rel_ptrs=None):
    by_dst = _plan.get_grouping(None, col, num_nodes, srow, drow)
    by_srow = _plan.get_grouping(None, srow, num_src_rows, col, drow)
    if by_dst is None or by_srow is None:
        return None
    if rel_ptrs is not None and num_nodes * (rel_ptrs.numel() - 1) >= 2 ** 31:
        rel_ptrs = None
    if rel_ptrs is not None:
        R = rel_ptrs.numel() - 1

        def build():
            rel = torch.repeat_interleave(torch.arange(R, dtype=torch.int64, device=col.device), rel_ptrs[1:] - rel_ptrs[:-1])
            if drow_nodes is not None:
                ok = bool((drow_nodes[drow] == col).all()) and drow.numel() == rel.numel()
                if ok and drow_rel_ptrs is not None:
                    ok = bool(((drow >= drow_rel_ptrs[rel]) & (drow < drow_rel_ptrs[rel + 1])).all())
                if not ok:
                    raise _lib.HetError("rgat_compact_groupings: the run-sum form needs every er row to be the (relation, "
                                        "destination) pair of its edges")
            return (col * R + rel).contiguous()
        key = _derived_get("dst_rel_key", (col, rel_ptrs, drow) + ((drow_nodes,) if drow_nodes is not None else ()), build)
        return by_dst, by_srow, None, _plan.get_grouping(None, key, num_nodes * R, None, None)
    by_drow = _plan.get_grouping(None, drow, num_dst_rows, grouping_rank_of_position(by_srow), None)
    return by_dst, by_srow, by_drow, None


def rgat_aggregate_compact(groupings, feat_c, el_c, er_c, sum, ret, slope, h_inout=None, num_rels=None, attn_l=None,
                           feat_rel_ptrs=None):
    _chk("rgat_aggregate_compact", tuple(t for t in (feat_c, el_c, er_c, sum, ret, h_inout) if t is not None))
    N, H = sum.shape[0], sum.shape[1]
    D = ret.numel() // max(1, N * H)
    if groupings[3] is not None:
        S_col = er_c.shape[0]
        q_rows = torch.empty((S_col, H, D), dtype=ret.dtype, device=ret.device)
        q_sum, q_ref = torch.empty_like(er_c), torch.empty_like(er_c)
        with torch.cuda.device(ret.device):
            nbytes = int(_lib.lib().het_rgat_aggregate_compact_runs_workspace(groupings[0].handle, groupings[3].handle, int(num_rels), H, D,
                                                                              _stream(ret)))
        if nbytes < 0:
            raise _lib.HetError("het_rgat_aggregate_compact_runs_workspace: " + _lib.lib().het_last_error().decode())
        ws = torch.empty((nbytes + 3) // 4, dtype=torch.float32, device=ret.device) if nbytes else None
        host_ptrs = None
        if attn_l is not None and feat_rel_ptrs is not None:
            _chk("rgat_aggregate_compact", (attn_l,), (feat_rel_ptrs,))
            lst = _derived_get("rel_ptrs_host", (feat_rel_ptrs,), lambda: feat_rel_ptrs.tolist())
            host_ptrs = (C.c_int64 * len(lst))(*lst)
        _call(ret, "het_rgat_aggregate_compact_runs", groupings[0].handle, groupings[3].handle, int(num_rels), _p(feat_c), _p(el_c),
              _p(er_c), _p(sum), _p(ret), N, H, D, float(slope), _p(h_inout), 0 if h_inout is None else h_inout.shape[0],
              _p(q_rows), _p(q_sum), _p(q_ref), S_col, _p(attn_l) if host_ptrs is not None else None, host_ptrs, _p(ws), nbytes,
              _stream(ret))
        return q_rows, q_sum, q_ref
    nbytes = int(_lib.lib().het_rgat_aggregate_compact_workspace(groupings[0].handle, H, D))
    ws = torch.empty((nbytes + 3) // 4, dtype=torch.float32, device=ret.device) if nbytes else None
    _call(ret, "het_rgat_aggregate_compact", groupings[0].handle, _p(feat_c), _p(el_c), _p(er_c), _p(sum), _p(ret), N, H, D,
          float(slope), _p(h_inout), 0 if h_inout is None else h_inout.shape[0], _p(ws), nbytes, _stream(ret))
    return None


def rows_matmul_backward_split_ok(H: int, K: int, D: int) -> bool:
    return K in (32, 64, 128) and H * D in (32, 64, 128)


def rows_matmul_backward_dx(rel_ptrs, gather_idx, weights_transposed, gradout, grad_x, atomic):
    _chk("rows_matmul_backward_dx", (weights_transposed, gradout, grad_x), (rel_ptrs,) + (() if gather_idx is None else (gather_idx,)))
    R, H, D, K = weights_transposed.shape
    _call(gradout, "het_rows_matmul_backward_dx", _p(rel_ptrs), R, _p(gather_idx), None, gradout.shape[0], _p(weights_transposed),
          _p(gradout), _p(grad_x), H, K, D, int(atomic), _stream(gradout))


def rows_matmul_backward_dw(rel_ptrs, gather_idx, x, gradout, grad_w, accumulate: bool, colsum: Optional[Tensor] = None):
    _chk("rows_matmul_backward_dw", (x, gradout, grad_w) + (() if colsum is None else (colsum,)),
         (rel_ptrs,) + (() if gather_idx is None else (gather_idx,)))
    R, H, K, D = grad_w.shape
    if colsum is None:
        _call(gradout, "het_rows_matmul_backward_dw", _p(rel_ptrs), R, _p(gather_idx), None, gradout.shape[0], _p(x), _p(gradout),
              _p(grad_w), H, K, D, int(accumulate), _stream(gradout))
        return
    assert colsum.numel() == H * D, "rows_matmul_backward_dw: colsum must hold H*D floats"
    _call(gradout, "het_rows_matmul_backward_dw_colsum", _p(rel_ptrs), R, _p(gather_idx), None, gradout.shape[0], _p(x), _p(gradout),
          _p(grad_w), _p(colsum), H, K, D, int(accumulate), _stream(gradout))


def rgat_node_gemm_ok(R: int, H: int, K: int, D: int) -> bool:
    return bool(_lib.lib().het_rgat_node_gemm_ok(R, H, K, D))


def node_row_map(rel_ptrs, nodes, num_nodes: int):
    def build():
        R = rel_ptrs.numel() - 1
        m = torch.empty((R, num_nodes), dtype=torch.int32, device=nodes.device)
        _call(nodes, "het_node_row_map", _p(rel_ptrs), R, _p(nodes), nodes.numel(), num_nodes, _p(m), _stream(nodes))
        return m
    _chk("node_row_map", (), (rel_ptrs, nodes))
    return _derived_get(("nodemap", num_nodes), (rel_ptrs, nodes), build)


def node_order_by_presence(row_map, dst_map=None, split=None):
    def build():
        R, N = row_map.shape
        w = (1 << torch.arange(R, device=row_map.device, dtype=torch.int64)).view(R, 1)
        mask = ((row_map >= 0).to(torch.int64) * w).sum(0)
        if dst_map is not None:
            mask = mask | (((dst_map >= 0).to(torch.int64) * w).sum(0) << R)
        if split is not None:
            mask = mask | ((torch.arange(N, device=row_map.device) >= int(split)).to(torch.int64) << (2 * R))
        return torch.argsort(mask, stable=True).to(torch.int32).contiguous()
    return _derived_get(("node_order", None if split is None else int(split)), (row_map,) + (() if dst_map is None else (dst_map,)), build)


def rgat_node_backward_dx(n_begin, n_end, n_loop, grad_h, loop_wt, g_rows, weights_t, row_map, g_er, wa_t, dst_map, grad_x,
                          node_order=None):
    _chk("rgat_node_backward_dx", tuple(t for t in (grad_h, loop_wt, g_rows, weights_t, g_er, wa_t, grad_x) if t is not None))
    R, H, D, K = weights_t.shape
    _call(grad_x, "het_rgat_node_backward_dx", int(n_begin), int(n_end), int(n_loop), grad_x.shape[0], R, _p(grad_h), _p(loop_wt),
          _p(g_rows), _p(weights_t), _p(row_map), _p(g_er), _p(wa_t), _p(dst_map), _p(grad_x), H, K, D, _p(node_order),
          _stream(grad_x))


def node_rows_matmul_sum_ok(num_sources: int, KS: int, XO: int) -> bool:
    return bool(_lib.lib().het_node_rows_matmul_sum_ok(int(num_sources), int(KS), int(XO)))


def _node_rows_matmul_sum(entry, n_begin, n_end, sources, out, node_order, bias_slot):
    N, XO = out.shape
    S = len(sources)
    KS = sources[0][3].shape[0]
    ptrs = (C.c_void_p * S)(*[src[0].data_ptr() + 4 * int(src[1]) for src in sources])
    strides = (C.c_int64 * S)(*[src[0].shape[1] if src[0].dim() == 2 else src[0].numel() // src[0].shape[0] for src in sources])
    maps = (C.c_void_p * S)(*[None if src[2] is None else src[2].data_ptr() for src in sources])
    ident = (C.c_int64 * S)(*[min(N, src[0].shape[0]) if src[2] is None else 0 for src in sources])
    wts = (C.c_void_p * S)(*[src[3].data_ptr() for src in sources])
    for src in sources:
        assert src[3].shape == (KS, XO) and src[3].is_contiguous() and (src[2] is None or (src[2].dtype == torch.int32 and src[2].numel() == N))
    _call(out, entry, int(n_begin), int(n_end), N, S, ptrs, strides, maps, ident, wts, *((None,) if bias_slot else ()), _p(out), KS, XO,
          _p(node_order), _stream(out))


def node_rows_matmul_sum(n_begin, n_end, sources, out, node_order=None):
    _chk("node_rows_matmul_sum", tuple(t for src in sources for t in (src[0], src[3])) + (out,))
    _node_rows_matmul_sum("het_node_rows_matmul_sum_bias", n_begin, n_end, sources, out, node_order, True)


def rows_linear_bias_ok(K: int, X: int) -> bool:
    return K in (32, 64, 128) and X in (32, 64, 128)


def rows_linear_bias(offsets, x, w, bias, out=None):
    _chk("rows_linear_bias", tuple(t for t in (x, w, bias, out) if t is not None), (offsets,))
    if out is None:
        out = torch.empty((x.shape[0], w.shape[1]), dtype=x.dtype, device=x.device)
    _call(x, "het_rows_linear_bias", _p(offsets), _p(x), _p(w), _p(bias), _p(out), x.shape[0], w.shape[0], w.shape[1], _stream(x))
    return out


def rgat_backward_compact(groupings, feat_c, el_c, er_c, sum, ret, gradout, grad_feat_c, grad_el_c, grad_er_c, slope,
                          fold_attn_l=None, row_rel_ptrs=None, grad_bias=None, bias_rows=0, runs=None, drow_nodes=None,
                          grad_attn_l=None):
    _chk("rgat_backward_compact", tuple(t for t in (feat_c, el_c, er_c, sum, ret, gradout, grad_feat_c, grad_el_c, grad_er_c,
                                                    fold_attn_l, grad_bias, grad_attn_l) + (tuple(runs) if runs else ()) if t is not None),
         tuple(t for t in (row_rel_ptrs, drow_nodes) if t is not None))
    N, H = sum.shape[0], sum.shape[1]
    D = ret.numel() // max(1, N * H)
    if runs:
        with torch.cuda.device(ret.device):
            nbytes = int(_lib.lib().het_rgat_backward_compact_runs_workspace(groupings[1].handle, N, er_c.shape[0], H, D, int(grad_bias is not None),
                                                                             int(grad_attn_l is not None), _stream(ret)))
        if nbytes < 0:
            raise _lib.HetError("het_rgat_backward_compact_runs_workspace: " + _lib.lib().het_last_error().decode())
    else:
        assert grad_attn_l is None, "grad_attn_l comes with the run-sum form"
        nbytes = int(_lib.lib().het_rgat_backward_compact_workspace(N, groupings[1]._keep[1].numel(), H, D, int(grad_bias is not None)))
    ws = torch.empty((nbytes + 3) // 4, dtype=torch.float32, device=ret.device)
    head = (_p(feat_c), _p(el_c), _p(er_c), _p(sum), _p(ret), _p(gradout), _p(grad_feat_c), _p(grad_el_c), _p(grad_er_c),
            _p(fold_attn_l), _p(row_rel_ptrs), 0 if row_rel_ptrs is None else row_rel_ptrs.numel() - 1, _p(grad_bias),
            int(bias_rows), N, feat_c.shape[0], er_c.shape[0], H, D, float(slope))
    tail = (_p(ws), ws.numel() * 4, _stream(ret))
    if runs:
        _call(ret, "het_rgat_backward_compact_runs", groupings[1].handle, _p(runs[0]), _p(runs[1]), _p(runs[2]), _p(drow_nodes), *head,
              _p(grad_attn_l), *tail)
    else:
        _call(ret, "het_rgat_backward_compact", groupings[1].handle, groupings[2].handle, *head, *tail)


def hgt_fold_source_weights(k_lin, v_lin, rel_att, rel_msg, rel_pri, src_type, transpose_att: bool):
    _chk("hgt_fold_source_weights", (k_lin, v_lin, rel_att, rel_msg, rel_pri), (src_type,))
    R, H, dk, _ = rel_att.shape
    T, K_in = k_lin.shape[0], k_lin.shape[2]
    w = torch.empty((R, 1, K_in, 2 * H * dk), dtype=k_lin.dtype, device=k_lin.device)
    _call(w, "het_hgt_fold_source_weights", _p(k_lin), _p(v_lin), _p(rel_att), _p(rel_msg), _p(rel_pri), _p(src_type), T, R, H, dk, K_in,
          int(transpose_att), _p(w), _stream(w))
    return w


def hgt_fold_source_weights_backward(grad_w, k_lin, v_lin, rel_att, rel_msg, rel_pri, src_type, transpose_att: bool):
    _chk("hgt_fold_source_weights_backward", (grad_w, k_lin, v_lin, rel_att, rel_msg, rel_pri), (src_type,))
    R, H, dk, _ = rel_att.shape
    T, K_in = k_lin.shape[0], k_lin.shape[2]
    outs = tuple(torch.empty_like(t) for t in (k_lin, v_lin, rel_att, rel_msg, rel_pri))
    _call(grad_w, "het_hgt_fold_source_weights_backward", _p(grad_w), _p(k_lin), _p(v_lin), _p(rel_att), _p(rel_msg), _p(rel_pri),
          _p(src_type), T, R, H, dk, K_in, int(transpose_att), *(_p(o) for o in outs), _stream(grad_w))
    return outs


def hgt_compact_shape_ok(H: int, D: int) -> bool:
    return bool(_lib.lib().het_hgt_compact_shape_ok(int(H), int(D)))


def destination_lists(col, offsets):
    def build():
        nodes, inv = torch.unique(col, return_inverse=True)
        ptrs = torch.searchsorted(nodes, offsets.to(nodes.dtype)).contiguous()
        return nodes.contiguous(), inv.contiguous(), ptrs
    return _derived_get("dst_lists", (col, offsets), build)


def hgt_compact_groupings(col, srow, num_nodes, num_src_rows):
    by_dst = _plan.get_grouping(None, col, num_nodes, srow, None)
    by_srow = _plan.get_grouping(None, srow, num_src_rows, col, None)
    return None if by_dst is None or by_srow is None else (by_dst, by_srow)


def hgt_aggregate_compact(groupings, kv_c, q, lsum, out):
    _chk("hgt_aggregate_compact", (kv_c, q, lsum, out))
    N, H = lsum.shape
    D = out.numel() // max(1, N * H)
    nbytes = int(_lib.lib().het_hgt_aggregate_compact_workspace(groupings[0].handle, H, D))
    ws = torch.empty((nbytes + 3) // 4, dtype=torch.float32, device=out.device) if nbytes else None
    _call(out, "het_hgt_aggregate_compact", groupings[0].handle, _p(kv_c), _p(q), _p(lsum), _p(out), N, kv_c.shape[0], H, D,
          _p(ws), nbytes, _stream(out))


def hgt_backward_compact(groupings, kv_c, q, lsum, out, gradout, grad_kv_c, grad_q):
    _chk("hgt_backward_compact", (kv_c, q, lsum, out, gradout, grad_kv_c, grad_q))
    N, H = lsum.shape
    D = out.numel() // max(1, N * H)
    nbytes = int(_lib.lib().het_hgt_backward_compact_workspace(N, H))
    ws = torch.empty((nbytes + 3) // 4, dtype=torch.float32, device=out.device)
    _call(out, "het_hgt_backward_compact", groupings[0].handle, groupings[1].handle, _p(kv_c), _p(q), _p(lsum), _p(out),
          _p(gradout), _p(grad_kv_c), _p(grad_q), N, kv_c.shape[0], H, D, _p(ws), ws.numel() * 4, _stream(out))


def gat_rank_of_position(rel_ptrs, row, col, eids, num_nodes):
    g = _by_dst(0, (None, None, None, None), rel_ptrs, row, col, eids, num_nodes)
    if g is None:
        return None
    r = getattr(g, "rank_of_position", None)
    if r is None:
        r = torch.empty(eids.numel(), dtype=torch.int64, device=eids.device)
        _call(r, "het_grouping_rank_of_position", g.handle, _p(r), _stream(r))
        g.rank_of_position = r
    return r


@_op("relational_fused_gat_csr(Tensor incsr_row_ptr, Tensor incsr_col_indices, Tensor incsr_eids, Tensor incsr_reltypes, "
     "Tensor unique_srcs_and_dests_rel_ptrs, Tensor unique_srcs_and_dests_node_indices, Tensor feat_src, Tensor el, "
     "Tensor er, Tensor(a!) sum, Tensor(b!) exp, Tensor(c!) ret, float slope, bool CompactAsOfNodeFlag=False) -> ()")
def relational_fused_gat_csr(incsr_row_ptr, incsr_col_indices, incsr_eids, incsr_reltypes,
                             unique_srcs_and_dests_rel_ptrs, unique_srcs_and_dests_node_indices, feat_src, el, er, sum,
                             exp, ret, slope, CompactAsOfNodeFlag=False):
    _chk("relational_fused_gat_csr", (feat_src, el, er, sum, exp, ret),
         (incsr_row_ptr, incsr_col_indices, incsr_eids, incsr_reltypes))
    N, E, H = incsr_row_ptr.numel() - 1, incsr_eids.numel(), el.shape[1]
    D = ret.numel() // max(1, N * H)
    if not CompactAsOfNodeFlag and _plan.is_enabled() and E > 0 and gat_grouped_shape_ok(H, D):
        dst, rp1 = _csr_expanded_rows(incsr_row_ptr, E)
        fused_gat_forward(incsr_eids, rp1, incsr_col_indices, dst, 0, {}, feat_src, el, er, sum, exp, ret, slope, None)
        return
    if CompactAsOfNodeFlag and _plan.is_enabled() and E > 0 and gat_grouped_shape_ok(H, D):
        dst, maps = _csr_compact_maps(incsr_row_ptr, incsr_col_indices, incsr_eids, incsr_reltypes,
                                      unique_srcs_and_dests_rel_ptrs, unique_srcs_and_dests_node_indices, True)
        _, rp1 = _csr_expanded_rows(incsr_row_ptr, E)
        fused_gat_forward(incsr_eids, rp1, incsr_col_indices, dst, 4, maps, feat_src, el, er, sum, exp, ret, slope, None)
        return
    _call(ret, "het_relational_fused_gat_csr", _p(incsr_row_ptr), _p(incsr_col_indices), _p(incsr_eids),
          _p(incsr_reltypes), N, E, _p(unique_srcs_and_dests_rel_ptrs), _p(unique_srcs_and_dests_node_indices),
          max(0, unique_srcs_and_dests_rel_ptrs.numel() - 1), _p(feat_src), _p(el), _p(er), _p(sum), _p(exp), _p(ret),
          H, D, float(slope), int(CompactAsOfNodeFlag), _stream(ret))


@_op("backward_relational_fused_gat_csr(Tensor outcsr_row_ptr, Tensor outcsr_col_indices, Tensor outcsr_eids, "
     "Tensor outcsr_reltypes, Tensor unique_srcs_and_dests_rel_ptrs, Tensor unique_srcs_and_dests_node_indices, "
     "Tensor feat_src, Tensor el, Tensor er, Tensor sum, Tensor exp, Tensor ret, Tensor gradout, "
     "Tensor(a!) grad_feat_src, Tensor(b!) grad_el, Tensor(c!) grad_er, float slope, bool CompactAsOfNodeFlag=False) -> ()")
def backward_relational_fused_gat_csr(outcsr_row_ptr, outcsr_col_indices, outcsr_eids, outcsr_reltypes,
                                      unique_srcs_and_dests_rel_ptrs, unique_srcs_and_dests_node_indices, feat_src, el,
                                      er, sum, exp, ret, gradout, grad_feat_src, grad_el, grad_er, slope,
                                      CompactAsOfNodeFlag=False):
    _chk("backward_relational_fused_gat_csr", (feat_src, el, er, sum, exp, ret, gradout, grad_feat_src, grad_el, grad_er),
         (outcsr_row_ptr, outcsr_col_indices, outcsr_eids, outcsr_reltypes))
    N, E, H = outcsr_row_ptr.numel() - 1, outcsr_eids.numel(), el.shape[1]
    D = ret.numel() // max(1, N * H)
    if not CompactAsOfNodeFlag and _plan.is_enabled() and E > 0 and gat_grouped_shape_ok(H, D) and slope >= 0:
        src, rp1 = _csr_expanded_rows(outcsr_row_ptr, E)
        fused_gat_backward(outcsr_eids, rp1, src, outcsr_col_indices, 0, {}, feat_src, el, er, sum, exp, ret, gradout,
                           grad_feat_src, grad_el, grad_er, slope, None)
        return
    if CompactAsOfNodeFlag and _plan.is_enabled() and E > 0 and gat_grouped_shape_ok(H, D) and slope >= 0:
        src, maps = _csr_compact_maps(outcsr_row_ptr, outcsr_col_indices, outcsr_eids, outcsr_reltypes,
                                      unique_srcs_and_dests_rel_ptrs, unique_srcs_and_dests_node_indices, False)
        _, rp1 = _csr_expanded_rows(outcsr_row_ptr, E)
        gf, gl, gr = torch.zeros_like(grad_feat_src), torch.zeros_like(grad_el), torch.zeros_like(grad_er)
        fused_gat_backward(outcsr_eids, rp1, src, outcsr_col_indices, 4, maps, feat_src, el, er, sum, exp, ret, gradout,
                           gf, gl, gr, slope, None)
        grad_feat_src += gf
        grad_el += gl
        grad_er += gr
        return
    _call(ret, "het_backward_relational_fused_gat_csr", _p(outcsr_row_ptr), _p(outcsr_col_indices), _p(outcsr_eids),
          _p(outcsr_reltypes), N, E, _p(unique_srcs_and_dests_rel_ptrs), _p(unique_srcs_and_dests_node_indices),
          max(0, unique_srcs_and_dests_rel_ptrs.numel() - 1), _p(feat_src), _p(el), _p(er), _p(sum), _p(exp), _p(ret),
          _p(gradout), _p(grad_feat_src), _p(grad_el), _p(grad_er), H, D, float(slope), int(CompactAsOfNodeFlag),
          _stream(ret))


@_op("rgcn_layer1_separate_coo(Tensor separate_coo_relptrs, Tensor separate_coo_eids, Tensor separate_coo_row_indices, "
     "Tensor separate_coo_col_indices, Tensor node_feat_input, Tensor weights, Tensor edge_norm, "
     "Tensor(a!) node_feat_output) -> ()")
def rgcn_layer1_separate_coo(separate_coo_relptrs, separate_coo_eids, separate_coo_row_indices,
                             separate_coo_col_indices, node_feat_input, weights, edge_norm, node_feat_output):
    _chk("rgcn_layer1_separate_coo", (node_feat_input, weights, edge_norm, node_feat_output),
         (separate_coo_relptrs, separate_coo_eids, separate_coo_row_indices, separate_coo_col_indices))
    R, K, D = weights.shape
    N = node_feat_output.shape[0]
    g = _plan.get_grouping(separate_coo_relptrs, separate_coo_col_indices, N, separate_coo_row_indices, separate_coo_eids)
    ws = None if g is None else torch.empty(max(1, g.num_segments) * K, dtype=torch.float32, device=weights.device)
    _call(node_feat_output, "het_rgcn_layer1_separate_coo", _p(separate_coo_relptrs), _p(separate_coo_eids),
          _p(separate_coo_row_indices), _p(separate_coo_col_indices), R, separate_coo_eids.numel(), N,
          _p(node_feat_input), _p(weights), _p(edge_norm), _p(node_feat_output), K, D, None if g is None else g.handle,
          _p(ws), 0 if ws is None else ws.numel() * 4, _stream(node_feat_output))


@_op("backward_rgcn_layer1_separate_coo(Tensor separate_coo_relptrs, Tensor separate_coo_eids, "
     "Tensor separate_coo_row_indices, Tensor separate_coo_col_indices, Tensor node_feat_input, "
     "Tensor weights_transposed, Tensor edge_norm, Tensor(a!) grad_edge_norm, Tensor(b!) delta_node_feat_input, "
     "Tensor delta_node_feat_output, Tensor(c!) delta_weights) -> ()")
def backward_rgcn_layer1_separate_coo(separate_coo_relptrs, separate_coo_eids, separate_coo_row_indices,
                                      separate_coo_col_indices, node_feat_input, weights_transposed, edge_norm,
                                      grad_edge_norm, delta_node_feat_input, delta_node_feat_output, delta_weights):
    _chk("backward_rgcn_layer1_separate_coo",
         (node_feat_input, weights_transposed, edge_norm, delta_node_feat_input, delta_node_feat_output, delta_weights),
         (separate_coo_relptrs, separate_coo_eids, separate_coo_row_indices, separate_coo_col_indices))
    R, D, K = weights_transposed.shape
    N = delta_node_feat_output.shape[0]
    g = _plan.get_grouping(separate_coo_relptrs, separate_coo_row_indices, node_feat_input.shape[0],
                           separate_coo_col_indices, separate_coo_eids)
    ws = None if g is None else torch.empty(max(1, g.num_segments) * D, dtype=torch.float32, device=delta_weights.device)
    _call(delta_weights, "het_backward_rgcn_layer1_separate_coo", _p(separate_coo_relptrs), _p(separate_coo_eids),
          _p(separate_coo_row_indices), _p(separate_coo_col_indices), R, separate_coo_eids.numel(), N,
          _p(node_feat_input), _p(weights_transposed), _p(edge_norm), _p(grad_edge_norm), _p(delta_node_feat_input),
          _p(delta_node_feat_output), _p(delta_weights), K, D, None if g is None else g.handle, _p(ws),
          0 if ws is None else ws.numel() * 4, _stream(delta_weights))


def rgcn_layer_ok(R: int, K: int, D: int) -> bool:
    return bool(_lib.lib().het_rgcn_layer_ok(int(R), int(K), int(D)))


def _grouping_segment_map(g, rel_ptrs, keys, num_keys: int):
    def build():
        R = rel_ptrs.numel() - 1
        m = torch.empty((R, num_keys), dtype=torch.int32, device=keys.device)
        _call(keys, "het_grouping_segment_map", g.handle, num_keys, _p(m), _stream(keys))
        return m
    return _derived_get(("segmap", num_keys), (rel_ptrs, keys), build)


def rgcn_layer_plan(rel_ptrs, eids, row, col, num_nodes: int):
    gd = _plan.get_grouping(rel_ptrs, col, num_nodes, row, eids)
    gs = _plan.get_grouping(rel_ptrs, row, num_nodes, col, eids)
    if gd is None or gs is None:
        return None
    dst_map = _grouping_segment_map(gd, rel_ptrs, col, num_nodes)
    src_map = _grouping_segment_map(gs, rel_ptrs, row, num_nodes)
    return gd, gs, dst_map, node_order_by_presence(dst_map), src_map, node_order_by_presence(src_map)


def scale_in_rank_order(g, values):
    if g is None or values is None:
        return None
    ident = _plan._ident(values)
    with _derived_lock:
        hit = getattr(g, "_scale_sorted", None)
        if hit is not None and hit[0] == ident:
            return hit[2]
        if getattr(g, "_scale_seen", None) != ident:
            g._scale_seen, g._scale_sorted = ident, None
            return None
        out = torch.empty_like(values, memory_format=torch.contiguous_format)
        H = values.numel() // max(1, values.shape[0])
        _call(values, "het_grouping_gather_payload1", g.handle, _p(values), H, _p(out), _stream(values))
        g._scale_sorted = (ident, values, out)
        return out


def rgcn_layer_forward(plan, x, weights, norm, bias):
    gd, _, dst_map, dst_order, _, _ = plan
    _chk("rgcn_layer_forward", tuple(t for t in (x, weights, norm, bias) if t is not None))
    R, K, D = weights.shape
    N = dst_map.shape[1]
    ssum = torch.empty((max(1, gd.num_segments), K), dtype=torch.float32, device=x.device)
    ret = torch.empty((N, D), dtype=torch.float32, device=x.device)
    _call(ret, "het_rgcn_layer_forward", gd.handle, R, N, _p(x), _p(weights), _p(norm), _p(scale_in_rank_order(gd, norm)), _p(bias),
          _p(dst_map), _p(dst_order),
          _p(ssum), _p(ret), K, D, _stream(ret))
    return ret, ssum


def rgcn_layer_backward(plan, ssum, weights_t, norm, gradout, want_bias: bool, want_x: bool = True):
    gd, gs, _, _, src_map, src_order = plan
    _chk("rgcn_layer_backward", (ssum, weights_t, norm, gradout))
    R, D, K = weights_t.shape
    N = src_map.shape[1]
    dev = gradout.device
    grad_x = torch.empty((N, K), dtype=torch.float32, device=dev) if want_x else None
    grad_w = torch.empty((R, K, D), dtype=torch.float32, device=dev)
    grad_bias = torch.empty((D,), dtype=torch.float32, device=dev) if want_bias else None
    nbytes = int(_lib.lib().het_rgcn_layer_backward_workspace(gs.num_segments, D))
    ws = torch.empty((nbytes + 3) // 4, dtype=torch.float32, device=dev)
    _call(gradout, "het_rgcn_layer_backward", gs.handle, gd.handle, R, N, gradout.shape[0], _p(ssum), _p(weights_t), _p(norm),
          _p(scale_in_rank_order(gs, norm) if want_x else None),
          _p(gradout), _p(src_map), _p(src_order), _p(grad_x), _p(grad_w), _p(grad_bias), K, D, _p(ws),
          ws.numel() * 4, _stream(gradout))
    return grad_x, grad_w, grad_bias


def _chk_bf16(name: str, rows=(), floats=()):
    for t in rows:
        if not (t.is_cuda and t.dtype == torch.bfloat16 and t.is_contiguous()):
            raise _lib.HetError(f"{name}: expected contiguous bfloat16 GPU activation rows, got {t.dtype} on {t.device}"
                                f"{'' if t.is_contiguous() else ' (non-contiguous)'}")
    _chk(name, floats)


def rgcn_layer_forward_bf16(plan, x, weights, norm, bias):
    gd, _, dst_map, dst_order, _, _ = plan
    _chk_bf16("rgcn_layer_forward_bf16", (x,), tuple(t for t in (weights, norm, bias) if t is not None))
    R, K, D = weights.shape
    N = dst_map.shape[1]
    ssum = torch.empty((max(1, gd.num_segments), K), dtype=torch.float32, device=x.device)
    ret = torch.empty((N, D), dtype=torch.bfloat16, device=x.device)
    _call(ret, "het_rgcn_layer_forward_bf16", gd.handle, R, N, _p(x), _p(weights), _p(norm), _p(scale_in_rank_order(gd, norm)),
          _p(bias), _p(dst_map), _p(dst_order), _p(ssum), _p(ret), K, D, _stream(ret))
    return ret, ssum


def rgcn_layer_backward_bf16(plan, ssum, weights_t, norm, gradout, want_bias: bool, want_x: bool = True):
    gd, gs, _, _, src_map, src_order = plan
    _chk_bf16("rgcn_layer_backward_bf16", (gradout,), (ssum, weights_t, norm))
    R, D, K = weights_t.shape
    N = src_map.shape[1]
    dev = gradout.device
    grad_x = torch.empty((N, K), dtype=torch.bfloat16, device=dev) if want_x else None
    grad_w = torch.empty((R, K, D), dtype=torch.float32, device=dev)
    grad_bias = torch.empty((D,), dtype=torch.float32, device=dev) if want_bias else None
    nbytes = int(_lib.lib().het_rgcn_layer_backward_workspace(gs.num_segments, D))
    ws = torch.empty((nbytes + 3) // 4, dtype=torch.float32, device=dev)
    _call(gradout, "het_rgcn_layer_backward_bf16", gs.handle, gd.handle, R, N, gradout.shape[0], _p(ssum), _p(weights_t), _p(norm),
          _p(scale_in_rank_order(gs, norm) if want_x else None),
          _p(gradout), _p(src_map), _p(src_order), _p(grad_x), _p(grad_w), _p(grad_bias), K, D, _p(ws),
          ws.numel() * 4, _stream(gradout))
    return grad_x, grad_w, grad_bias


def rows_matmul_bf16_ok(K: int, X: int) -> bool:
    return K in (32, 64) and X in (32, 64, 128)


def rows_matmul_bf16(rel_ptrs, gather_idx, scatter_idx, weights, x, out):
    lists = tuple(t for t in (gather_idx, scatter_idx) if t is not None)
    _chk_bf16("rows_matmul_bf16", (x, out), (weights,))
    _chk("rows_matmul_bf16", (), (rel_ptrs,) + lists)
    R, _, K, X = weights.shape
    n = lists[0].numel() if lists else x.shape[0]
    if x.shape[-1] != K or out.shape[-1] != X or (gather_idx is None and x.shape[0] < n) or (scatter_idx is None and out.shape[0] < n):
        raise _lib.HetError(f"rows_matmul_bf16: x {tuple(x.shape)} / out {tuple(out.shape)} do not fit weights {tuple(weights.shape)} and {n} rows")
    _call(out, "het_rows_matmul_bf16", _p(rel_ptrs), R, _p(gather_idx), _p(scatter_idx), n, _p(weights), _p(x), _p(out), K, X,
          _stream(out))


def rows_matmul_backward_dw_bf16(rel_ptrs, gather_idx, x, gradout, grad_w, accumulate: bool, g_rows=None):
    lists = tuple(t for t in (gather_idx, g_rows) if t is not None)
    g_bf16 = gradout.dtype == torch.bfloat16
    _chk_bf16("rows_matmul_backward_dw_bf16", (x, gradout) if g_bf16 else (x,), (grad_w,) if g_bf16 else (gradout, grad_w))
    _chk("rows_matmul_backward_dw_bf16", (), (rel_ptrs,) + lists)
# ... 421 lines not shown
```

include/het_amd.h:

```cpp
#ifndef HET_AMD_H
#define HET_AMD_H

#include <stddef.h>
#include <stdint.h>

#ifdef __cplusplus
extern "C" {
#endif

#define HET_OK 0
#define HET_ERR_INVALID_ARG 1
#define HET_ERR_HIP 2
#define HET_ERR_UNSUPPORTED 3

typedef void* het_stream;
typedef uint16_t het_bf16;

#define HET_KIND_DISABLED 0
#define HET_KIND_ENABLED 1
#define HET_KIND_DIRECT_INDEX 2
#define HET_KIND_DUAL_LIST 3
#define HET_KIND_DUAL_LIST_DIRECT_INDEX 4

const char* het_build_info(void);
const char* het_last_error(void);

int het_kernel_timing_enable(int on);
int het_kernel_timing_read(const char* name_prefix, double* total_ms, int64_t* launches);

typedef void* (*het_alloc_fn)(size_t bytes, het_stream stream, void* user);
typedef void (*het_free_fn)(void* ptr, void* user);
int het_set_allocator(het_alloc_fn alloc, het_free_fn free_, void* user);
int het_allocator_is_external(void);
typedef struct het_grouping het_grouping;
int het_grouping_create(const int64_t* rel_ptrs , int64_t num_rels,
                        const int64_t* keys , int64_t num_positions, int64_t key_bound,
                        const int64_t* payload0, const int64_t* payload1,
                        het_stream stream, het_grouping** out);
void het_grouping_destroy(het_grouping* g);
void het_grouping_note_stream(const het_grouping* g, het_stream stream);
int64_t het_grouping_num_segments(const het_grouping* g);
int64_t het_grouping_bytes(const het_grouping* g);
int het_grouping_rank_of_position(const het_grouping* g, int64_t* out, het_stream stream);
int het_grouping_segment_map(const het_grouping* g, int64_t num_keys, int32_t* map, het_stream stream);
int het_grouping_gather_payload1(const het_grouping* g, const float* values, int64_t H, float* out, het_stream stream);

int het_rgnn_relational_matmul(int64_t kind, const int64_t* rel_ptrs, int64_t num_rels,
                               const int64_t* gather_idx, const int64_t* scatter_idx, int64_t num_rows,
                               const float* weights, const float* x, float* ret,
                               int64_t H, int64_t K, int64_t D, int in1head,
                               const het_grouping* by_rel_gather, void* workspace, int64_t workspace_bytes,
                               het_stream stream);

int het_rgnn_relational_matmul_attn_dot(int64_t kind, const int64_t* rel_ptrs, int64_t num_rels,
                                        const int64_t* gather_idx, const int64_t* scatter_idx, int64_t num_rows,
                                        const float* weights, const float* x, float* ret, const float* dot_w,
                                        float* dot_out, int64_t H, int64_t K, int64_t D,
                                        const het_grouping* by_rel_gather, void* workspace, int64_t workspace_bytes,
                                        float* comp_rows, const het_grouping* dot_grouping, het_stream stream);

int het_backward_rgnn_relational_matmul_attn_dot_only(const int64_t* rel_ptrs, int64_t num_rels, const int64_t* gather_idx,
                                                      const int64_t* scatter_idx, int64_t num_rows, int64_t num_x_rows,
                                                      const float* weights_t, const float* x, const float* dot_w,
                                                      const float* grad_dot, float* grad_x, float* grad_w, int64_t H,
                                                      int64_t K, int64_t D, int accumulate,
                                                      const het_grouping* by_rel_gather, void* workspace,
                                                      int64_t workspace_bytes, const float* comp_rows,
                                                      float* grad_dot_w, het_stream stream);

#define HET_ACC_ADD 1
#define HET_ACC_DISTINCT_ROWS 2
int het_backward_rgnn_relational_matmul(int64_t kind, const int64_t* rel_ptrs, int64_t num_rels,
                                        const int64_t* gather_idx, const int64_t* scatter_idx, int64_t num_rows,
                                        int64_t num_x_rows ,
                                        const float* weights_t, const float* x, const float* gradout,
                                        float* grad_x, float* grad_w,
                                        int64_t H, int64_t K, int64_t D, int in1head, int accumulate,
                                        const het_grouping* by_rel_gather, void* workspace,
                                        int64_t workspace_bytes, het_stream stream);

int het_rgnn_relational_matmul_no_scatter_gather_list(const int64_t* offsets, int64_t num_types, int64_t num_rows,
                                                      const float* weights, const float* x, float* ret,
                                                      int64_t H, int64_t K, int64_t D, int x_per_head,
                                                      het_stream stream);
int het_backward_rgnn_relational_matmul_no_scatter_gather_list(const int64_t* offsets, int64_t num_types,
                                                               int64_t num_rows, const float* weights_t,
                                                               const float* x, const float* gradout,
                                                               float* grad_x, float* grad_w,
                                                               int64_t H, int64_t K, int64_t D, int x_per_head,
                                                               int accumulate, het_stream stream);

int het_relational_fused_gat_separate_coo(const int64_t* eids, const int64_t* rel_ptrs, const int64_t* row,
                                          const int64_t* col, int64_t num_rels, int64_t num_edges,
                                          int64_t num_nodes, int64_t kind,
                                          const int64_t* map_row_a, const int64_t* map_row_b,
                                          const int64_t* map_col_a, const int64_t* map_col_b,
                                          const float* feat, const float* el, const float* er,
                                          float* sum, float* exp, float* ret, float* exp_sorted,
                                          int64_t H, int64_t D, double slope,
                                          const het_grouping* by_dst, const float* el_sorted, const float* er_sorted,
                                          het_stream stream);

int het_backward_relational_fused_gat_separate_coo(const int64_t* eids, const int64_t* rel_ptrs,
                                                   const int64_t* row, const int64_t* col, int64_t num_rels,
                                                   int64_t num_edges, int64_t num_nodes, int64_t kind,
                                                   const int64_t* map_row_a, const int64_t* map_row_b,
                                                   const int64_t* map_col_a, const int64_t* map_col_b,
                                                   const float* feat, const float* el, const float* er,
                                                   const float* sum, const float* exp, const float* ret,
                                                   const float* exp_sorted,
                                                   const float* gradout, float* grad_feat, float* grad_el,
                                                   float* grad_er, int64_t H, int64_t D, double slope,
                                                   const het_grouping* by_dst, const het_grouping* by_src_row,
                                                   const het_grouping* by_dst_row, int64_t n_src_rows,
                                                   int64_t n_dst_rows, void* workspace, int64_t workspace_bytes,
                                                   const float* fold_attn_l, float* grad_fold_attn_l,
                                                   const int64_t* fold_row_rel_ptrs, float* grad_el_sorted,
                                                   het_stream stream);

int het_relational_fused_gat_csr(const int64_t* in_row_ptrs, const int64_t* in_col, const int64_t* in_eids,
                                 const int64_t* in_reltypes, int64_t num_nodes, int64_t num_edges,
                                 const int64_t* uniq_rel_ptrs, const int64_t* uniq_node_idx, int64_t num_rels,
                                 const float* feat, const float* el, const float* er,
                                 float* sum, float* exp, float* ret, int64_t H, int64_t D, double slope,
                                 int compact, het_stream stream);
int het_backward_relational_fused_gat_csr(const int64_t* out_row_ptrs, const int64_t* out_col,
                                          const int64_t* out_eids, const int64_t* out_reltypes,
                                          int64_t num_nodes, int64_t num_edges,
                                          const int64_t* uniq_rel_ptrs, const int64_t* uniq_node_idx,
                                          int64_t num_rels, const float* feat, const float* el, const float* er,
                                          const float* sum, const float* exp, const float* ret,
                                          const float* gradout, float* grad_feat, float* grad_el, float* grad_er,
                                          int64_t H, int64_t D, double slope, int compact, het_stream stream);

int het_rgcn_layer1_separate_coo(const int64_t* rel_ptrs, const int64_t* eids, const int64_t* row,
                                 const int64_t* col, int64_t num_rels, int64_t num_edges, int64_t num_nodes,
                                 const float* x, const float* weights, const float* norm, float* ret,
                                 int64_t K, int64_t D, const het_grouping* by_rel_dst, void* workspace,
                                 int64_t workspace_bytes, het_stream stream);
int het_backward_rgcn_layer1_separate_coo(const int64_t* rel_ptrs, const int64_t* eids, const int64_t* row,
                                          const int64_t* col, int64_t num_rels, int64_t num_edges,
                                          int64_t num_nodes, const float* x, const float* weights_t,
                                          const float* norm, float* grad_norm, float* grad_x,
                                          const float* gradout, float* grad_w, int64_t K, int64_t D,
                                          const het_grouping* by_rel_src, void* workspace, int64_t workspace_bytes,
                                          het_stream stream);

int het_rgcn_node_mean_aggregation_compact_as_of_node_separate_coo(
    const int64_t* eids, const int64_t* rel_ptrs, const int64_t* row, const int64_t* col, int64_t num_rels,
    int64_t num_edges, int64_t num_nodes, const int64_t* map_a, const int64_t* map_b, const float* feat,
    const float* enorm, float* ret, int64_t X, int direct, const het_grouping* by_dst, het_stream stream);
int het_backward_rgcn_node_mean_aggregation_compact_as_of_node_separate_coo(
    const int64_t* eids, const int64_t* rel_ptrs, const int64_t* row, const int64_t* col, int64_t num_rels,
    int64_t num_edges, int64_t num_nodes, const int64_t* map_a, const int64_t* map_b, const float* feat,
    const float* enorm, const float* ret, const float* gradout, float* grad_feat, int64_t X, int direct,
    const het_grouping* by_src_row, int64_t n_src_rows, het_stream stream);

int het_hgt_full_graph_edge_softmax_ops_separate_coo(const int64_t* row, const int64_t* col, const int64_t* eids,
                                                     const int64_t* rel_ptrs, int64_t num_rels, int64_t num_edges,
                                                     int64_t num_nodes, const float* score, const float* mu,
                                                     float* sum, float* m, float* a, int64_t H,
                                                     const het_grouping* by_dst, het_stream stream);
int het_backward_hgt_full_graph_enorm_to_unnormalized_attn_score_separate_coo(
    const int64_t* row, const int64_t* col, const int64_t* eids, const int64_t* rel_ptrs, int64_t num_rels,
    int64_t num_edges, int64_t num_nodes, const float* score, const float* a, const float* grad_a, const float* mu,
    float* grad_score, float* grad_mu, float* tmp, int64_t H, const het_grouping* by_dst, het_stream stream);

int het_hgt_full_graph_edge_softmax_ops_csr(const int64_t* row_ptrs, int64_t row_ptrs_len, const int64_t* col_indices,
                                            const int64_t* eids, const int64_t* reltypes, int64_t num_nodes,
                                            int64_t num_edges, const float* score, const float* mu, float* sum, float* m,
                                            float* a, int64_t H, const het_grouping* by_dst, het_stream stream);
int het_hgt_full_graph_message_mean_aggregation_csr(const int64_t* row_ptrs, int64_t row_ptrs_len, const int64_t* col_indices,
                                                    const int64_t* reltypes, const int64_t* eids, int64_t num_nodes,
                                                    int64_t num_edges, const float* edge_messages,
                                                    const float* edge_attn_score, const float* sum, const float* mu,
                                                    float* ret, int64_t H, int64_t dk, const het_grouping* by_dst,
                                                    het_stream stream);
int het_backward_hgt_full_graph_message_mean_aggregation_csr(const int64_t* row_ptrs, int64_t row_ptrs_len,
                                                             const int64_t* col_indices, const int64_t* reltypes,
                                                             const int64_t* eids, int64_t num_nodes, int64_t num_edges,
                                                             const float* sum, const float* normalized_attn_score,
                                                             const float* gradout, float* grad_message, int64_t H,
                                                             int64_t dk, het_stream stream);
int het_backward_hgt_full_graph_edge_softmax_ops_csr(const int64_t* row_ptrs, int64_t row_ptrs_len, const int64_t* col_indices,
                                                     const int64_t* eids, const int64_t* reltypes, int64_t num_nodes,
                                                     int64_t num_edges, int64_t num_rels, const float* message,
                                                     const float* score, const float* normalized_attn_score,
                                                     const float* out, const float* gradout, const float* mu,
                                                     float* grad_attn_score, float* grad_mu, int64_t H, int64_t dk,
                                                     const het_grouping* by_dst, het_stream stream);
int het_backward_hgt_full_graph_enorm_to_unnormalized_attn_score_csr(
    const int64_t* row_ptrs, int64_t row_ptrs_len, const int64_t* col_indices, const int64_t* eids, const int64_t* reltypes,
    int64_t num_nodes, int64_t num_edges, int64_t num_rels, const float* score, const float* normalized_attn_score,
    const float* grad_normalized_attn_score, const float* mu, float* grad_score, float* grad_mu, int64_t H,
    const het_grouping* by_dst, void* workspace, int64_t workspace_bytes, het_stream stream);

int het_hgt_full_graph_fused_message_calc_and_mean_aggregation_separate_coo(
    const int64_t* rel_ptrs, const int64_t* eids, const int64_t* row, const int64_t* col, int64_t num_rels,
    int64_t num_edges, int64_t num_nodes, const float* v, const float* weights, const float* a, float* new_h,
    int64_t H, int64_t dk, int64_t dout, const het_grouping* by_rel_dst, void* workspace, int64_t workspace_bytes,
    het_stream stream);
int het_backward_hgt_full_graph_fused_message_calc_and_mean_aggregation_separate_coo(
    const int64_t* rel_ptrs, const int64_t* eids, const int64_t* row, const int64_t* col, int64_t num_rels,
    int64_t num_edges, int64_t num_nodes, const float* v, const float* weights_t, const float* a, const float* new_h,
    float* grad_v, float* grad_w, float* grad_a, const float* gradout, int64_t H, int64_t dk, int64_t dout,
    const het_grouping* by_rel_src, void* workspace, int64_t workspace_bytes, het_stream stream);

int het_rgnn_inner_product_right_node_separatecoo(int64_t kind, const int64_t* map_a, const int64_t* map_b,
                                                  const int64_t* rel_ptrs, const int64_t* eids, const int64_t* row,
                                                  const int64_t* col, int64_t num_rels, int64_t num_edges,
                                                  const float* left, const float* right, float* out, int64_t H,
                                                  int64_t D, het_stream stream);
int het_backward_inner_product_right_node_separatecoo(int64_t kind, const int64_t* map_a, const int64_t* map_b,
                                                      const int64_t* rel_ptrs, const int64_t* eids,
                                                      const int64_t* row, const int64_t* col, int64_t num_rels,
                                                      int64_t num_edges, const float* left, const float* right,
                                                      const float* gradout, float* grad_left, float* grad_right,
                                                      int64_t H, int64_t D, int accumulate,
                                                      const het_grouping* by_right, const het_grouping* by_left,
                                                      int64_t n_left_rows, int64_t n_right_rows, het_stream stream);

int het_hgt_full_graph_hetero_attention_ops_coo(const int64_t* row, const int64_t* col, const int64_t* eids,
                                                const int64_t* rel_ptrs, int64_t num_rels, int64_t num_edges,
                                                const float* k, const float* q, const float* weights, float* inner,
                                                float* score, int64_t H, int64_t dk, int64_t dout, het_stream stream);
int het_backward_hgt_full_graph_hetero_attention_ops_coo(const int64_t* row, const int64_t* col, const int64_t* eids,
                                                         const int64_t* rel_ptrs, int64_t num_rels, int64_t num_edges,
                                                         float* grad_w, const float* weights_t, const float* k,
                                                         const float* q, const float* inner, const float* grad_score,
                                                         float* grad_k, float* grad_q, int64_t H, int64_t dk,
                                                         int64_t dout, const het_grouping* by_dst,
                                                         const het_grouping* by_rel_src, int64_t n_q_rows,
                                                         void* workspace, int64_t workspace_bytes, het_stream stream);

int het_hgt_compact_shape_ok(int64_t H, int64_t D);
int het_hgt_aggregate_compact(const het_grouping* by_dst, const float* kv_c, const float* q, float* lsum, float* out,
                              int64_t num_nodes, int64_t num_src_rows, int64_t H, int64_t D, void* workspace,
                              int64_t workspace_bytes, het_stream stream);
int64_t het_hgt_aggregate_compact_workspace(const het_grouping* by_dst, int64_t H, int64_t D);
int64_t het_hgt_backward_compact_workspace(int64_t num_nodes, int64_t H);
int het_hgt_backward_compact(const het_grouping* by_dst, const het_grouping* by_srow, const float* kv_c, const float* q,
                             const float* lsum, const float* out, const float* gradout, float* grad_kv_c, float* grad_q,
                             int64_t num_nodes, int64_t num_src_rows, int64_t H, int64_t D, void* workspace,
                             int64_t workspace_bytes, het_stream stream);

int het_hgt_aggregate_compact_bf16(const het_grouping* by_dst, const het_bf16* kv_c, const het_bf16* q, float* lsum, het_bf16* out,
                                   int64_t num_nodes, int64_t num_src_rows, int64_t H, int64_t D, void* workspace,
                                   int64_t workspace_bytes, het_stream stream);
int het_hgt_backward_compact_bf16(const het_grouping* by_dst, const het_grouping* by_srow, const het_bf16* kv_c, const het_bf16* q,
                                  const float* lsum, const het_bf16* out, const het_bf16* gradout, float* grad_kv_c, float* grad_q,
                                  int64_t num_nodes, int64_t num_src_rows, int64_t H, int64_t D, void* workspace,
                                  int64_t workspace_bytes, het_stream stream);

int het_hgt_fold_source_weights(const float* k_lin, const float* v_lin, const float* rel_att, const float* rel_msg,
                                const float* rel_pri, const int64_t* src_type, int64_t num_types, int64_t num_rels, int64_t H,
                                int64_t dk, int64_t K_in, int transpose_att, float* w_kv, het_stream stream);
int het_hgt_fold_source_weights_backward(const float* grad_w_kv, const float* k_lin, const float* v_lin, const float* rel_att,
                                         const float* rel_msg, const float* rel_pri, const int64_t* src_type, int64_t num_types,
                                         int64_t num_rels, int64_t H, int64_t dk, int64_t K_in, int transpose_att, float* grad_k_lin,
                                         float* grad_v_lin, float* grad_att, float* grad_msg, float* grad_pri, het_stream stream);

int het_rgat_aggregate_compact(const het_grouping* by_dst, const float* feat_c, const float* el_c, const float* er_c,
                               float* sum, float* ret, int64_t num_nodes, int64_t H, int64_t D, double slope,
                               float* h_inout, int64_t h_rows, void* workspace, int64_t workspace_bytes, het_stream stream);
int64_t het_rgat_aggregate_compact_workspace(const het_grouping* by_dst, int64_t H, int64_t D);
int64_t het_rgat_backward_compact_workspace(int64_t num_nodes, int64_t num_edges, int64_t H, int64_t D, int with_bias);
int het_rgat_backward_compact(const het_grouping* by_srow, const het_grouping* by_drow, const float* feat_c,
                              const float* el_c, const float* er_c, const float* sum, const float* ret,
                              const float* gradout, float* grad_feat_c, float* grad_el_c, float* grad_er_c,
                              const float* fold_attn_l, const int64_t* row_rel_ptrs, int64_t num_rels,
                              float* grad_bias, int64_t bias_rows, int64_t num_nodes, int64_t num_src_rows,
                              int64_t num_dst_rows, int64_t H, int64_t D, double slope, void* workspace,
                              int64_t workspace_bytes, het_stream stream);

int64_t het_rgat_aggregate_compact_runs_workspace(const het_grouping* by_dst, const het_grouping* by_dst_rel, int64_t num_rels,
                                                  int64_t H, int64_t D, het_stream stream);
int het_rgat_aggregate_compact_runs(const het_grouping* by_dst, const het_grouping* by_dst_rel, int64_t num_rels,
                                    const float* feat_c, const float* el_c, const float* er_c, float* sum, float* ret,
                                    int64_t num_nodes, int64_t H, int64_t D, double slope, float* h_inout, int64_t h_rows,
                                    float* q_rows, float* q_sum, float* q_ref, int64_t num_dst_rows, const float* attn_l,
                                    const int64_t* feat_rel_ptrs_host, void* workspace, int64_t workspace_bytes, het_stream stream);
int het_rgat_backward_compact_runs(const het_grouping* by_srow, const float* q_rows, const float* q_sum, const float* q_ref,
                                   const int64_t* drow_nodes, const float* feat_c, const float* el_c, const float* er_c,
                                   const float* sum, const float* ret, const float* gradout, float* grad_feat_c,
                                   float* grad_el_c, float* grad_er_c, const float* fold_attn_l, const int64_t* row_rel_ptrs,
                                   int64_t num_rels, float* grad_bias, int64_t bias_rows, int64_t num_nodes,
                                   int64_t num_src_rows, int64_t num_dst_rows, int64_t H, int64_t D, double slope,
                                   float* grad_attn_l, void* workspace, int64_t workspace_bytes, het_stream stream);
int64_t het_rgat_backward_compact_runs_workspace(const het_grouping* by_srow, int64_t num_nodes, int64_t num_dst_rows, int64_t H,
                                                 int64_t D, int with_bias, int with_attn_grad, het_stream stream);

int het_rows_matmul_backward_dx(const int64_t* rel_ptrs, int64_t num_rels, const int64_t* gather_idx, const int64_t* g_rows,
                                int64_t num_rows, const float* weights_t, const float* gradout, float* grad_x, int64_t H,
                                int64_t K, int64_t D, int atomic, het_stream stream);
int het_rows_matmul_backward_dw(const int64_t* rel_ptrs, int64_t num_rels, const int64_t* gather_idx, const int64_t* g_rows,
                                int64_t num_rows, const float* x, const float* gradout, float* grad_w, int64_t H, int64_t K,
                                int64_t D, int accumulate, het_stream stream);
int het_rows_matmul_backward_dw_colsum(const int64_t* rel_ptrs, int64_t num_rels, const int64_t* gather_idx,
                                       const int64_t* g_rows, int64_t num_rows, const float* x, const float* gradout,
                                       float* grad_w, float* colsum, int64_t H, int64_t K, int64_t D, int accumulate,
                                       het_stream stream);

int het_rows_matmul_bf16(const int64_t* rel_ptrs, int64_t num_rels, const int64_t* gather_idx, const int64_t* scatter_idx,
                         int64_t num_rows, const float* weights, const het_bf16* x, het_bf16* out, int64_t K, int64_t X,
                         het_stream stream);
int het_rows_matmul_backward_dw_bf16(const int64_t* rel_ptrs, int64_t num_rels, const int64_t* gather_idx, const int64_t* g_rows,
                                     int64_t num_rows, const het_bf16* x, const float* gradout, float* grad_w, int64_t K, int64_t X,
                                     int accumulate, het_stream stream);
int het_rows_matmul_backward_dw_bf16_bf16(const int64_t* rel_ptrs, int64_t num_rels, const int64_t* gather_idx, const int64_t* g_rows,
                                          int64_t num_rows, const het_bf16* x, const het_bf16* gradout, float* grad_w, int64_t K,
                                          int64_t X, int accumulate, het_stream stream);

int het_rgat_node_gemm_ok(int64_t num_rels, int64_t H, int64_t K, int64_t D);
int het_node_row_map(const int64_t* rel_ptrs, int64_t num_rels, const int64_t* nodes, int64_t num_rows, int64_t num_nodes,
                     int32_t* map, het_stream stream);
int het_rgat_node_backward_dx(int64_t n_begin, int64_t n_end, int64_t n_loop, int64_t num_nodes, int64_t num_rels,
                              const float* grad_h, const float* loop_wt, const float* g_rows, const float* weights_t,
                              const int32_t* row_map, const float* g_er, const float* wa_t, const int32_t* dst_map,
                              float* grad_x, int64_t H, int64_t K, int64_t D, const int32_t* node_order, het_stream stream);

int het_node_rows_matmul_sum_ok(int64_t num_sources, int64_t KS, int64_t XO);
int het_node_rows_matmul_sum(int64_t n_begin, int64_t n_end, int64_t num_nodes, int64_t num_sources,
                             const float* const* rows, const int64_t* row_strides, const int32_t* const* maps,
                             const int64_t* ident_rows, const float* const* weights_t, float* out, int64_t KS, int64_t XO,
                             const int32_t* node_order, het_stream stream);

int het_node_rows_matmul_sum_bias(int64_t n_begin, int64_t n_end, int64_t num_nodes, int64_t num_sources,
                                  const float* const* rows, const int64_t* row_strides, const int32_t* const* maps,
                                  const int64_t* ident_rows, const float* const* weights_t, const float* bias, float* out,
                                  int64_t KS, int64_t XO, const int32_t* node_order, het_stream stream);

int het_node_rows_matmul_sum_bf16(int64_t n_begin, int64_t n_end, int64_t num_nodes, int64_t num_sources,
                                  const float* const* rows, const int64_t* row_strides, const int32_t* const* maps,
                                  const int64_t* ident_rows, const float* const* weights_t, het_bf16* out, int64_t KS, int64_t XO,
                                  const int32_t* node_order, het_stream stream);

int het_rgcn_layer_ok(int64_t num_rels, int64_t K, int64_t D);
int64_t het_rgcn_layer_backward_workspace(int64_t n_src_rows, int64_t D);
int het_rgcn_layer_forward(const het_grouping* by_rel_dst, int64_t num_rels, int64_t num_nodes, const float* x,
                           const float* weights, const float* norm, const float* norm_sorted, const float* bias,
                           const int32_t* dst_map, const int32_t* node_order, float* ssum, float* ret, int64_t K, int64_t D,
                           het_stream stream);
int het_rgcn_layer_backward(const het_grouping* by_rel_src, const het_grouping* by_rel_dst, int64_t num_rels,
                            int64_t num_src_nodes, int64_t num_dst_nodes, const float* ssum, const float* weights_t,
                            const float* norm, const float* norm_sorted, const float* gradout, const int32_t* src_map,
                            const int32_t* node_order, float* grad_x, float* grad_w, float* grad_bias, int64_t K, int64_t D, void* workspace,
                            int64_t workspace_bytes, het_stream stream);
int het_rgcn_layer_forward_bf16(const het_grouping* by_rel_dst, int64_t num_rels, int64_t num_nodes, const het_bf16* x,
                                const float* weights, const float* norm, const float* norm_sorted, const float* bias,
                                const int32_t* dst_map, const int32_t* node_order, float* ssum, het_bf16* ret, int64_t K, int64_t D,
                                het_stream stream);
int het_rgcn_layer_backward_bf16(const het_grouping* by_rel_src, const het_grouping* by_rel_dst, int64_t num_rels,
                                 int64_t num_src_nodes, int64_t num_dst_nodes, const float* ssum, const float* weights_t,
                                 const float* norm, const float* norm_sorted, const het_bf16* gradout, const int32_t* src_map,
                                 const int32_t* node_order, het_bf16* grad_x, float* grad_w, float* grad_bias, int64_t K, int64_t D,
                                 void* workspace, int64_t workspace_bytes, het_stream stream);

int het_rows_linear_bias(const int64_t* offsets, const float* x, const float* w, const float* bias, float* out,
                         int64_t num_rows, int64_t K, int64_t X, het_stream stream);

int het_rows_add_bias(const float* a, const float* b, const float* bias, float* out, int64_t num_rows, int64_t X,
                      het_stream stream);

int het_rows_gather(const float* x, const int64_t* idx, int64_t num_rows, int64_t X, float* out, het_stream stream);
int het_rows_scatter_add(const float* src, const int64_t* idx, int64_t num_rows, int64_t X, float* out, het_stream stream);
int het_rows_scatter_add_grouped(const het_grouping* by_idx, const float* src, int64_t X, float* out, int64_t out_rows,
                                 het_stream stream);

int het_layout_separate_coo(const int64_t* row, const int64_t* col, const int64_t* rel, const int64_t* eids,
                            int64_t num_edges, int64_t num_rels, int64_t eid_bound, int64_t* out_rel_ptrs,
                            int64_t* out_row, int64_t* out_col, int64_t* out_eids, het_stream stream);
int het_layout_coo_to_csr(const int64_t* row, const int64_t* col, const int64_t* rel, const int64_t* eids,
                          int64_t num_edges, int64_t num_rows, int64_t* out_row_ptrs, int64_t* out_col, int64_t* out_rel,
                          int64_t* out_eids, het_stream stream);
int het_layout_transpose_csr(const int64_t* row_ptrs, const int64_t* col, const int64_t* eids, const int64_t* rel,
                             int64_t num_rows, int64_t num_edges, int64_t num_cols, int64_t* out_row_ptrs, int64_t* out_col,
                             int64_t* out_eids, int64_t* out_rel, het_stream stream);
int het_layout_unique_rel_nodes(const int64_t* rel_ptrs, int64_t num_rels, const int64_t* nodes_a, const int64_t* nodes_b,
                                int64_t num_edges, int64_t num_nodes, int64_t* out_nodes, int64_t* out_rel_ptrs,
                                int64_t* out_inverse, int64_t* out_count, het_stream stream);

#ifdef __cplusplus
}
#endif
#endif
```

Before: 6026 million edges/s.

## Fold RGAT parameter prep and attention-grad reductions into dedicated fused kernels

```diff
diff --git a/het_amd/_lib.py b/het_amd/_lib.py
--- a/het_amd/_lib.py
+++ b/het_amd/_lib.py
@@ -33,6 +33,8 @@
     "het_backward_relational_fused_gat_csr": [P, P, P, P, I64, I64, P, P, I64, P, P, P, P, P, P, P, P, P, P, I64, I64, DBL, INT, P],
     "het_hgt_fold_source_weights": [P, P, P, P, P, P, I64, I64, I64, I64, I64, INT, P, P],
     "het_hgt_fold_source_weights_backward": [P, P, P, P, P, P, P, I64, I64, I64, I64, I64, INT, P, P, P, P, P, P],
+    "het_rgat_fold_params": [P, P, P, I64, I64, I64, I64, P, P, P, P],
+    "het_rgat_fold_params_backward": [P, P, P, I64, I64, I64, I64, P, P, P, P, I64, P, P],
     "het_rgat_aggregate_compact": [P, P, P, P, P, P, I64, I64, I64, DBL, P, I64, P, I64, P],
     "het_rows_matmul_backward_dx": [P, I64, P, P, I64, P, P, P, I64, I64, I64, INT, P],
     "het_rows_matmul_backward_dw": [P, I64, P, P, I64, P, P, P, I64, I64, I64, INT, P],
@@ -49,6 +51,10 @@
     "het_rgat_backward_compact": [P, P, P, P, P, P, P, P, P, P, P, P, P, I64, P, I64, I64, I64, I64, I64, I64, DBL, P, I64, P],
     "het_rgat_aggregate_compact_runs": [P, P, I64, P, P, P, P, P, I64, I64, I64, DBL, P, I64, P, P, P, I64, P, P, P, I64, P],
     "het_rgat_backward_compact_runs": [P, P, P, P, P, P, P, P, P, P, P, P, P, P, P, P, I64, P, I64, I64, I64, I64, I64, I64, DBL, P, P, I64, P],
+    "het_rgat_aggregate_compact_runs_prepare": [P, P, I64, I64, I64, P],
+    "het_rgat_aggregate_compact_runs_prepared": [P, P, I64, P, P, P, P, P, I64, I64, I64, DBL, P, I64, P, P, P, I64, P, P, P, I64, P],
+    "het_rgat_backward_compact_runs_partials": [P, P, P, P, P, P, P, P, P, P, P, P, P, P, P, P, I64, P, I64, I64, I64, I64, I64, I64, DBL, P, P, I64, P, P],
+    "het_rgat_attn_grad_finish": [P, P, I64, I64, P, P],
     "het_hgt_aggregate_compact": [P, P, P, P, P, I64, I64, I64, I64, P, I64, P],
     "het_hgt_backward_compact": [P, P, P, P, P, P, P, P, P, I64, I64, I64, I64, P, I64, P],
     "het_hgt_aggregate_compact_bf16": [P, P, P, P, P, I64, I64, I64, I64, P, I64, P],
diff --git a/het_amd/backend/rgat_fused_layer.py b/het_amd/backend/rgat_fused_layer.py
--- a/het_amd/backend/rgat_fused_layer.py
+++ b/het_amd/backend/rgat_fused_layer.py
@@ -16,6 +16,13 @@
 
 def _mulfirst_shape_ok(H, Kd):
     return H in (1, 2, 4, 8) and Kd >= 4 * H and Kd & (Kd - 1) == 0 and Kd <= 256
+
+
+def _fold_ok(compact, mulfirst, halo, x, W, loop_w, col, nd):
+    R, H, Kd, D = W.shape
+    return (OVERLAP and halo is None and compact and mulfirst and loop_w is not None and x.dtype == th.float32
+            and _k.rows_linear_bias_ok(Kd, H * D) and _k.rgat_runs_shape_ok(H, D) and R <= 8 and _k.rgat_fold_params_ok(W, loop_w)
+            and _k.rgat_node_gemm_ok(R, H, Kd, D) and _destinations_below(col, nd))
 
 
 def _has_single_sided_lists(g):
@@ -137,7 +144,9 @@
                     _OFFS.clear()
                 offs = _OFFS[(nd, x.device)] = th.tensor([0, nd], dtype=th.int64, device=x.device)
         wa = None
-        if mulfirst:
+        folded = ()
+        fold = _fold_ok(compact, mulfirst, halo, x, W, loop_w, col, nd)
+        if mulfirst and not fold:
             wa = th.bmm(W.view(-1, Kd, D), attn_r.view(-1, D, 1)).view(R, H, Kd, 1)
         if compact:
             ss = g.get_separate_unique_node_indices_single_sided()
@@ -151,9 +160,14 @@
             if OVERLAP and halo is None and fused_loop and mulfirst:
                 main, side = th.cuda.current_stream(x.device), _side_stream(x.device)
                 h = x.new_empty((nd, X))
+                if fold:
+                    folded = (new(R, H, Kd), new(R, H, D, Kd), new(X, Kd))
                 side.wait_stream(main)
             if mulfirst:
                 with th.cuda.stream(side if side is not None else th.cuda.current_stream(x.device)):
+                    if fold:
+                        _k.rgat_fold_params(W, attn_r, loop_w, out=folded)
+                        wa = folded[0].view(R, H, Kd, 1)
                     K.rgnn_relational_matmul(d_col, 1, wa, x, erc.view(-1, H, 1), True)
                 saved = (featc, elc, erc)
             else:
@@ -183,14 +197,16 @@
             else:
                 K.rgnn_relational_matmul(d_row, 1, W, x, featc, True)
                 K.rgnn_relational_matmul_no_scatter_gather_list(ss["rel_ptrs_row"], attn_l.unsqueeze(-1), featc, elc.view(-1, H, 1))
-            if side is not None:
-                th.cuda.current_stream(x.device).wait_stream(side)
             srow, drow = _edge_rows(g, ss, direct, rp, row, col, eids)
             run_sums = _k.rgat_runs_shape_ok(H, D)
             grp = _k.rgat_compact_groupings(col, srow, drow, N, featc.shape[0], erc.shape[0], rel_ptrs=rp if run_sums else None,
                                             drow_nodes=ss["node_indices_col"], drow_rel_ptrs=ss["rel_ptrs_col"])
+            prepared = _k.rgat_aggregate_compact_prepare(grp, erc, sm, ret) if fold and grp is not None and grp[3] is not None else None
+            if side is not None:
+                th.cuda.current_stream(x.device).wait_stream(side)
             ctx.runs = _k.rgat_aggregate_compact(grp, featc, elc, erc, sm, ret, slope, h_inout=h, num_rels=R,
-                                                 attn_l=attn_l.contiguous() if run_sums else None, feat_rel_ptrs=ss["rel_ptrs_row"] if run_sums else None)
+                                                 attn_l=attn_l.contiguous() if run_sums else None, feat_rel_ptrs=ss["rel_ptrs_row"] if run_sums else None,
+                                                 prepared=prepared)
             ctx.grp = grp
             ex = x.new_empty(0)
         else:
@@ -219,8 +235,9 @@
         ctx.halo = halo
         ctx.g, ctx.compact, ctx.mulfirst, ctx.slope, ctx.nd = g, compact, mulfirst, slope, nd
         ctx.has_loop, ctx.has_bias = loop_w is not None, bias is not None
+        ctx.folded = bool(folded)
         ctx.save_for_backward(x, W, attn_l, attn_r, loop_w if loop_w is not None else x.new_empty(0), offs if offs is not None else eids,
-                              sm, ex, ret, *saved)
+                              sm, ex, ret, *saved, *folded)
         return h
 
     @staticmethod
@@ -237,9 +254,9 @@
         if ctx.halo is not None:
             return RgatLayerFunction._backward_with_halo(ctx, grad_h)
         grad_bias = grad_h.sum(0) if (ctx.has_bias and not ctx.compact) else None
+        if ctx.compact and ctx.mulfirst and _k.rgat_node_gemm_ok(R, H, Kd, D) and _destinations_below(col, nd):
+            return RgatLayerFunction._backward_node_major(ctx, grad_h, saved[-2] if ctx.folded else th.transpose(W, 2, 3).contiguous())
         Wt = th.transpose(W, 2, 3).contiguous()
-        if ctx.compact and ctx.mulfirst and _k.rgat_node_gemm_ok(R, H, Kd, D) and _destinations_below(col, nd):
-            return RgatLayerFunction._backward_node_major(ctx, grad_h, Wt)
         grad_W = th.zeros_like(W)
         grad_loop = None
         if ctx.has_loop:
@@ -315,7 +332,7 @@
 
     @staticmethod
     def _backward_node_major(ctx, grad_h, Wt):
-        x, W, attn_l, attn_r, loop_w, offs, sm, ex, ret, featc, elc, erc = ctx.saved_tensors
+        x, W, attn_l, attn_r, loop_w, offs, sm, ex, ret, featc, elc, erc, *folded = ctx.saved_tensors
         g, nd, slope = ctx.g, ctx.nd, ctx.slope
         N, Kd = x.shape
         R, H, _, D = W.shape
@@ -338,14 +355,23 @@
                 _k.rows_matmul_backward_dw(offs, None, x[:nd], grad_h, grad_loop.view(1, 1, Kd, X), accumulate=False,
                                            colsum=grad_bias if bias_in_dw else None)
         grad_attn_l = th.empty_like(attn_l)
-        _k.rgat_backward_compact(ctx.grp, featc, elc, erc, sm[:nd], ret[:nd], go, g_featc, g_elc, g_erc, slope, fold_attn_l=attn_l,
-                                 row_rel_ptrs=rp_row, grad_bias=None if bias_in_dw else grad_bias, bias_rows=nd, runs=ctx.runs,
-                                 drow_nodes=ss["node_indices_col"], grad_attn_l=grad_attn_l if attn_in_pass else None)
-        wa_t = th.bmm(W.view(-1, Kd, D), attn_r.view(-1, D, 1)).view(R, H, Kd)
+        fold = bool(folded) and side is not None and attn_in_pass
+        partials = _k.rgat_backward_compact(ctx.grp, featc, elc, erc, sm[:nd], ret[:nd], go, g_featc, g_elc, g_erc, slope, fold_attn_l=attn_l,
+                                            row_rel_ptrs=rp_row, grad_bias=None if bias_in_dw else grad_bias, bias_rows=nd, runs=ctx.runs,
+                                            drow_nodes=ss["node_indices_col"], grad_attn_l=grad_attn_l if attn_in_pass else None,
+                                            attn_partials=fold)
+        if folded:
+            wa_t = folded[0]
+        else:
+            wa_t = th.bmm(W.view(-1, Kd, D), attn_r.view(-1, D, 1)).view(R, H, Kd)
         grad_x = th.empty_like(x)
         grad_W, grad_wa = th.empty_like(W), th.empty((R, H, Kd), dtype=x.dtype, device=x.device)
+        grad_attn_r = th.empty_like(attn_r) if fold else None
         gh = grad_h if ctx.has_loop else None
-        loop_wt = loop_w.t().contiguous() if ctx.has_loop else None
+        if folded:
+            loop_wt = folded[2]
+        else:
+            loop_wt = loop_w.t().contiguous() if ctx.has_loop else None
         d_col = {"unique_srcs_and_dests_rel_ptrs": ss["rel_ptrs_col"], "unique_srcs_and_dests_node_indices": ss["node_indices_col"]}
 
         def weight_gradients():
@@ -358,6 +384,8 @@
             _k.rows_matmul_backward_dw(rp_row, ss["node_indices_row"], x, g_featc.view(-1, X), grad_W, accumulate=False)
             _k.matmul_backward(d_col, 1, wa_t.view(R, H, 1, Kd), x, g_erc.view(-1, H, 1), None, grad_wa.view(R, H, Kd, 1), True,
                                accumulate=False)
+            if fold:
+                _k.rgat_fold_params_backward(W, attn_r, grad_wa, grad_W, grad_attn_r, partials, grad_attn_l)
 
         order = _k.node_order_by_presence(row_map, dst_map, split=nd if nd < N else None)
 
@@ -373,8 +401,10 @@
         else:
             input_gradient()
             weight_gradients()
-        grad_W.addcmul_(grad_wa.unsqueeze(-1), attn_r.view(R, H, 1, D))
-        grad_attn_r = (W * grad_wa.unsqueeze(-1)).sum(2)
+        if not fold:
+            grad_W.addcmul_(grad_wa.unsqueeze(-1), attn_r.view(R, H, 1, D))
+            grad_attn_r = (W * grad_wa.unsqueeze(-1)).sum(2)
+        del partials
         return None, None, None, None, None, None, None, grad_x, grad_W, grad_attn_l, grad_attn_r, grad_loop, grad_bias
 
     @staticmethod
diff --git a/het_amd/csrc/gat_compact.hip b/het_amd/csrc/gat_compact.hip
--- a/het_amd/csrc/gat_compact.hip
+++ b/het_amd/csrc/gat_compact.hip
@@ -1078,8 +1078,11 @@
                                                               const float* __restrict__ qrow, const float* __restrict__ qsum,
                                                               const float* __restrict__ qref, const int64_t* __restrict__ drow_nodes,
                                                               const int32_t* __restrict__ order, int64_t n_rows,
-                                                              float* __restrict__ rec4, float* __restrict__ grad_er) {
+                                                              float* __restrict__ rec4, float* __restrict__ grad_er,
+                                                              float* __restrict__ zero_out, int zero_n) {
   constexpr int EPW = 64 / LPR, X = LPR * 4, H = LPR / DL, U = 2;
+  if (zero_out && blockIdx.x == 0)
+    for (int i = threadIdx.x; i < zero_n; i += kBlock) zero_out[i] = 0.f;
   const int lane = threadIdx.x & 63, wave = threadIdx.x >> 6;
   const int slot = lane / LPR, sub = lane % LPR, x = sub * 4, h = sub / DL, d = sub % DL;
   const int64_t w0 = (((int64_t)blockIdx.x * (kBlock / 64) + wave) * U) * EPW + slot;
@@ -1234,13 +1237,34 @@
   return (int64_t)sizeof(float) * by_dst_rel->num_hub_items * (2 * H * D + 3 * H);
 }
 
-extern "C" int het_rgat_aggregate_compact_runs(const het_grouping* by_dst, const het_grouping* by_dst_rel, int64_t num_rels,
+__global__ __launch_bounds__(kBlock) void HET_rgat_aggregate_prepare(float* __restrict__ a, int64_t na, float* __restrict__ b, int64_t nb) {
+  const int64_t qa = na / 4, qb = nb / 4, total = qa + qb + (na % 4) + (nb % 4);
+  const float4 z = make_float4(0.f, 0.f, 0.f, 0.f);
+  for (int64_t t = (int64_t)blockIdx.x * kBlock + threadIdx.x; t < total; t += (int64_t)gridDim.x * kBlock) {
+    if (t < qa) st4(a + t * 4, z);
+    else if (t < qa + qb) st4(b + (t - qa) * 4, z);
+    else if (t < qa + qb + na % 4) a[qa * 4 + (t - qa - qb)] = 0.f;
+    else b[qb * 4 + (t - qa - qb - na % 4)] = 0.f;
+  }
+}
+
+extern "C" int het_rgat_aggregate_compact_runs_prepare(float* sum, float* q_sum, int64_t num_nodes, int64_t num_dst_rows, int64_t H,
+                                                       het_stream stream) {
+  const char* op = "het_rgat_aggregate_compact_runs_prepare";
+  HET_REQUIRE(sum && q_sum && num_nodes >= 0 && num_dst_rows >= 0 && H > 0 && aligned16(sum, q_sum), "%s: null or misaligned argument", op);
+  const int64_t na = num_nodes * H, nb = num_dst_rows * H;
+  if (na + nb == 0) return HET_OK;
+  hipLaunchKernelGGL(HET_rgat_aggregate_prepare, dim3(grid_for(na / 4 + nb / 4 + 6)), dim3(kBlock), 0, (hipStream_t)stream, sum, na, q_sum, nb);
+  HET_LAUNCH_CHECK("HET_rgat_aggregate_prepare");
+  return HET_OK;
+}
+
+static int rgat_aggregate_compact_runs_impl(const char* op, bool prepared, const het_grouping* by_dst, const het_grouping* by_dst_rel, int64_t num_rels,
                                                const float* feat_c, const float* el_c, const float* er_c, float* sum, float* ret,
                                                int64_t num_nodes, int64_t H, int64_t D, double slope, float* h_inout,
                                                int64_t h_rows, float* q_rows, float* q_sum, float* q_ref, int64_t num_dst_rows,
                                                const float* attn_l, const int64_t* feat_rel_ptrs_host, void* workspace,
                                                int64_t workspace_bytes, het_stream stream) {
-  const char* op = "het_rgat_aggregate_compact_runs";
   hipStream_t s = (hipStream_t)stream;
   HET_REQUIRE(by_dst && by_dst_rel && sum && ret && q_rows && q_sum && q_ref && num_nodes >= 0 && num_rels > 0, "%s: null argument", op);
   if (!compact_shape_ok(H, D) || !coop_shape_ok(H, D)) {
@@ -1256,8 +1280,10 @@
   HET_REQUIRE(need == 0 || (workspace && workspace_bytes >= need && aligned16(workspace)),
               "%s: a 16-byte aligned workspace of %lld bytes is needed (het_rgat_aggregate_compact_runs_workspace)", op, (long long)need);
   const int64_t X = H * D;
-  HET_HIP(hipMemsetAsync(sum, 0, sizeof(float) * num_nodes * H, s));
-  HET_HIP(hipMemsetAsync(q_sum, 0, sizeof(float) * num_dst_rows * H, s));
+  if (!prepared) {
+    HET_HIP(hipMemsetAsync(sum, 0, sizeof(float) * num_nodes * H, s));
+    HET_HIP(hipMemsetAsync(q_sum, 0, sizeof(float) * num_dst_rows * H, s));
+  }
   if (!h_inout) HET_HIP(hipMemsetAsync(ret, 0, sizeof(float) * num_nodes * X, s));
   if (by_dst->E == 0) return HET_OK;
   if (int rc = grouping_packed_ids(by_dst, true, s)) return rc;
@@ -1337,6 +1363,28 @@
   return HET_OK;
 }
 
+extern "C" int het_rgat_aggregate_compact_runs(const het_grouping* by_dst, const het_grouping* by_dst_rel, int64_t num_rels,
+                                               const float* feat_c, const float* el_c, const float* er_c, float* sum, float* ret,
+                                               int64_t num_nodes, int64_t H, int64_t D, double slope, float* h_inout,
+                                               int64_t h_rows, float* q_rows, float* q_sum, float* q_ref, int64_t num_dst_rows,
+                                               const float* attn_l, const int64_t* feat_rel_ptrs_host, void* workspace,
+                                               int64_t workspace_bytes, het_stream stream) {
+  return rgat_aggregate_compact_runs_impl("het_rgat_aggregate_compact_runs", false, by_dst, by_dst_rel, num_rels, feat_c, el_c, er_c, sum,
+                                          ret, num_nodes, H, D, slope, h_inout, h_rows, q_rows, q_sum, q_ref, num_dst_rows, attn_l,
+                                          feat_rel_ptrs_host, workspace, workspace_bytes, stream);
+}
+
+extern "C" int het_rgat_aggregate_compact_runs_prepared(const het_grouping* by_dst, const het_grouping* by_dst_rel, int64_t num_rels,
+                                                        const float* feat_c, const float* el_c, const float* er_c, float* sum,
+                                                        float* ret, int64_t num_nodes, int64_t H, int64_t D, double slope,
+                                                        float* h_inout, int64_t h_rows, float* q_rows, float* q_sum, float* q_ref,
+                                                        int64_t num_dst_rows, const float* attn_l, const int64_t* feat_rel_ptrs_host,
+                                                        void* workspace, int64_t workspace_bytes, het_stream stream) {
+  return rgat_aggregate_compact_runs_impl("het_rgat_aggregate_compact_runs_prepared", true, by_dst, by_dst_rel, num_rels, feat_c, el_c, er_c,
+                                          sum, ret, num_nodes, H, D, slope, h_inout, h_rows, q_rows, q_sum, q_ref, num_dst_rows, attn_l,
+                                          feat_rel_ptrs_host, workspace, workspace_bytes, stream);
+}
+
 extern "C" int64_t het_rgat_backward_compact_workspace(int64_t num_nodes, int64_t num_edges, int64_t H, int64_t D, int with_bias) {
   const int64_t n_pack = (num_nodes * 2 * H + 3) / 4 * 4, n_tbuf = (num_edges * H + 3) / 4 * 4;
   return (int64_t)sizeof(float) * (n_pack + n_tbuf + (with_bias ? (int64_t)2048 * (kBlock / 64) * H * D : 0));
@@ -1358,7 +1406,7 @@
                                       const float* fold_attn_l, const int64_t* row_rel_ptrs, int64_t num_rels,
                                       float* grad_bias, int64_t bias_rows, int64_t num_nodes, int64_t num_src_rows,
                                       int64_t num_dst_rows, int64_t H, int64_t D, double slope, void* workspace,
-                                      int64_t workspace_bytes, het_stream stream) {
+                                      int64_t workspace_bytes, het_stream stream, int64_t* attn_part_info = nullptr) {
   hipStream_t s = (hipStream_t)stream;
   HET_REQUIRE(by_srow && (by_drow || runs) && sum && ret && gradout && grad_feat_c && grad_er_c, "%s: null argument", op);
   HET_REQUIRE(grad_el_c || (runs && fold_attn_l && grad_attn_l && coop_shape_ok(H, D)),
@@ -1391,8 +1439,9 @@
   float* bias_part = grad_bias ? pack + n_pack + n_tbuf : nullptr;
   float* ga_part = ga_rows ? pack + n_pack + n_tbuf + bias_part_rows * X : nullptr;
   int* ga_rel = ga_rows ? reinterpret_cast<int*>(ga_part + ga_rows * X) : nullptr;
+  if (attn_part_info) { attn_part_info[0] = ga_rows ? (int64_t)sizeof(float) * (ga_part - pack) : 0; attn_part_info[1] = ga_rows; }
   float* rec4 = use_rec ? pack + n_pack + n_tbuf + bias_part_rows * X + n_ga : nullptr;
-  if (grad_attn_l) HET_HIP(hipMemsetAsync(grad_attn_l, 0, sizeof(float) * num_rels * X, s));
+  if (grad_attn_l && !use_rec) HET_HIP(hipMemsetAsync(grad_attn_l, 0, sizeof(float) * num_rels * X, s));
   if (by_srow->S != num_src_rows) {
     HET_HIP(hipMemsetAsync(grad_feat_c, 0, sizeof(float) * num_src_rows * X, s));
     if (grad_el_c) HET_HIP(hipMemsetAsync(grad_el_c, 0, sizeof(float) * num_src_rows * H, s));
@@ -1425,7 +1474,7 @@
     HET_DISPATCH_COOP((int)(X / 4), (int)(D / 4),
                       hipLaunchKernelGGL((HET_rgat_drow_pass<LPR, DL>), dim3(nbd), dim3(kBlock), 0, s, er_c, sum, ret, gradout,
                                          runs->q_rows, runs->q_sum, runs->q_ref, runs->drow_nodes, by_srow->val_order, num_dst_rows, rec4,
-                                         grad_er_c));
+                                         grad_er_c, grad_attn_l, grad_attn_l ? (int)(num_rels * X) : 0));
     HET_LAUNCH_CHECK("HET_rgat_drow_pass");
   }
   const float* er_arg = use_rec ? rec4 : er_c;
@@ -1524,7 +1573,7 @@
   }
   HET_LAUNCH_CHECK("HET_rgat_backward_src_packed");
   HET_HIP(fk.join());
-  if (ga_rows) {
+  if (ga_rows && !attn_part_info) {
     hipLaunchKernelGGL(HET_rgat_attn_grad_finish, dim3((unsigned)ceil_div64(ga_rows, kAttnFinishRows)), dim3(kBlock), 0, s, ga_part, ga_rel, ga_rows,
                        (int)X, grad_attn_l);
     HET_LAUNCH_CHECK("HET_rgat_attn_grad_finish");
@@ -1574,3 +1623,32 @@
                                     grad_feat_c, grad_el_c, grad_er_c, fold_attn_l, row_rel_ptrs, num_rels, grad_bias, bias_rows,
                                     num_nodes, num_src_rows, num_dst_rows, H, D, slope, workspace, workspace_bytes, stream);
 }
+
+extern "C" int het_rgat_backward_compact_runs_partials(const het_grouping* by_srow, const float* q_rows, const float* q_sum,
+                                                       const float* q_ref, const int64_t* drow_nodes, const float* feat_c,
+                                                       const float* el_c, const float* er_c, const float* sum, const float* ret,
+                                                       const float* gradout, float* grad_feat_c, float* grad_el_c, float* grad_er_c,
+                                                       const float* fold_attn_l, const int64_t* row_rel_ptrs, int64_t num_rels,
+                                                       float* grad_bias, int64_t bias_rows, int64_t num_nodes, int64_t num_src_rows,
+                                                       int64_t num_dst_rows, int64_t H, int64_t D, double slope, float* grad_attn_l,
+                                                       void* workspace, int64_t workspace_bytes, int64_t* attn_part_info,
+                                                       het_stream stream) {
+  HET_REQUIRE(q_rows && q_sum && q_ref && (drow_nodes || num_dst_rows == 0) && grad_attn_l && attn_part_info,
+              "het_rgat_backward_compact_runs_partials: null argument");
+  const RunSums runs{q_rows, q_sum, q_ref, drow_nodes};
+  return rgat_backward_compact_impl("het_rgat_backward_compact_runs_partials", by_srow, nullptr, &runs, grad_attn_l, feat_c, el_c, er_c, sum,
+                                    ret, gradout, grad_feat_c, grad_el_c, grad_er_c, fold_attn_l, row_rel_ptrs, num_rels, grad_bias,
+                                    bias_rows, num_nodes, num_src_rows, num_dst_rows, H, D, slope, workspace, workspace_bytes, stream,
+                                    attn_part_info);
+}
+
+extern "C" int het_rgat_attn_grad_finish(const float* attn_part, const int32_t* attn_part_rel, int64_t attn_part_rows, int64_t X,
+                                         float* grad_attn_l, het_stream stream) {
+  HET_REQUIRE(attn_part && attn_part_rel && grad_attn_l && attn_part_rows >= 0 && X > 0 && kBlock % X == 0,
+              "het_rgat_attn_grad_finish: null argument or a row width that does not divide %d", kBlock);
+  if (attn_part_rows == 0) return HET_OK;
+  hipLaunchKernelGGL(HET_rgat_attn_grad_finish, dim3((unsigned)ceil_div64(attn_part_rows, kAttnFinishRows)), dim3(kBlock), 0,
+                     (hipStream_t)stream, attn_part, attn_part_rel, attn_part_rows, (int)X, grad_attn_l);
+  HET_LAUNCH_CHECK("HET_rgat_attn_grad_finish");
+  return HET_OK;
+}
diff --git a/het_amd/csrc/rgat_fold.hip b/het_amd/csrc/rgat_fold.hip
--- /dev/null
+++ b/het_amd/csrc/rgat_fold.hip
@@ -0,0 +1,125 @@
+#include "common.hip.h"
+
+namespace {
+
+__global__ __launch_bounds__(kBlock) void HET_rgat_fold_params(const float* __restrict__ W, const float* __restrict__ attn_r,
+                                                               const float* __restrict__ loop_w, int RH, int K, int D, int X,
+                                                               float* __restrict__ wa, float* __restrict__ Wt,
+                                                               float* __restrict__ loop_wt) {
+  const int64_t n_wa = (int64_t)RH * K, n_wt = n_wa * D, n_loop = loop_w ? (int64_t)X * K : 0;
+  const int64_t total = n_wa + n_wt + n_loop;
+  for (int64_t t = (int64_t)blockIdx.x * kBlock + threadIdx.x; t < total; t += (int64_t)gridDim.x * kBlock) {
+    if (t < n_wa) {
+      const float* w = W + t * D;
+      const float* a = attn_r + (t / K) * D;
+      float s = 0.f;
+      for (int d = 0; d < D; ++d) s = fmaf(w[d], a[d], s);
+      wa[t] = s;
+    } else if (t < n_wa + n_wt) {
+      const int64_t u = t - n_wa;
+      const int k = (int)(u % K), d = (int)((u / K) % D);
+      const int64_t rh = u / ((int64_t)K * D);
+      Wt[u] = W[(rh * K + k) * D + d];
+    } else {
+      const int64_t u = t - n_wa - n_wt;
+      const int k = (int)(u % K), x = (int)(u / K);
+      loop_wt[u] = loop_w[(int64_t)k * X + x];
+    }
+  }
+}
+
+constexpr int kAttnCols = 4;
+
+__global__ __launch_bounds__(kBlock) void HET_rgat_fold_params_backward(const float* __restrict__ W, const float* __restrict__ attn_r,
+                                                                        const float* __restrict__ grad_wa, int RH, int K, int D,
+                                                                        float* __restrict__ grad_W, float* __restrict__ grad_attn_r,
+                                                                        int nb_elem, const float* __restrict__ part,
+                                                                        const int* __restrict__ part_rel, int64_t P, int X,
+                                                                        float* __restrict__ grad_attn_l) {
+  if ((int)blockIdx.x < nb_elem) {
+    const int64_t n_w = (int64_t)RH * K * D, total = n_w + (int64_t)RH * D;
+    for (int64_t t = (int64_t)blockIdx.x * kBlock + threadIdx.x; t < total; t += (int64_t)nb_elem * kBlock) {
+      if (t < n_w) {
+        const int d = (int)(t % D);
+        const int64_t rhk = t / D;
+        grad_W[t] = fmaf(grad_wa[rhk], attn_r[(rhk / K) * D + d], grad_W[t]);
+      } else {
+        const int64_t u = t - n_w, rh = u / D;
+        const int d = (int)(u % D);
+        float s[8] = {0.f, 0.f, 0.f, 0.f, 0.f, 0.f, 0.f, 0.f};
+        for (int k = 0; k < K; ++k) s[k & 7] = fmaf(W[(rh * K + k) * D + d], grad_wa[rh * K + k], s[k & 7]);
+        grad_attn_r[u] = ((s[0] + s[4]) + (s[2] + s[6])) + ((s[1] + s[5]) + (s[3] + s[7]));
+      }
+    }
+    return;
+  }
+  __shared__ float4 red[kBlock];
+  constexpr int U = 4;
+  const int b = (int)blockIdx.x - nb_elem, groups = X / kAttnCols;
+  const int r = b / groups, c0 = (b % groups) * kAttnCols;
+  float4 acc = make_float4(0.f, 0.f, 0.f, 0.f);
+  for (int64_t p0 = threadIdx.x; p0 < P; p0 += (int64_t)kBlock * U) {
+    bool take[U];
+    float4 v[U];
+#pragma unroll
+    for (int u = 0; u < U; ++u) {
+      const int64_t p = p0 + (int64_t)u * kBlock;
+      take[u] = p < P && part_rel[p] == r;
+    }
+#pragma unroll
+    for (int u = 0; u < U; ++u)
+      v[u] = take[u] ? ld4(part + (p0 + (int64_t)u * kBlock) * X + c0) : make_float4(0.f, 0.f, 0.f, 0.f);
+#pragma unroll
+    for (int u = 0; u < U; ++u)
+      if (take[u]) { acc.x += v[u].x; acc.y += v[u].y; acc.z += v[u].z; acc.w += v[u].w; }
+  }
+  red[threadIdx.x] = acc;
+  __syncthreads();
+  for (int o = kBlock / 2; o > 0; o >>= 1) {
+    if ((int)threadIdx.x < o) {
+      const float4 a = red[threadIdx.x], c = red[threadIdx.x + o];
+      red[threadIdx.x] = make_float4(a.x + c.x, a.y + c.y, a.z + c.z, a.w + c.w);
+    }
+    __syncthreads();
+  }
+  if (threadIdx.x == 0) {
+    float* o = grad_attn_l + (int64_t)r * X + c0;
+    const float4 a = ld4(o), t = red[0];
+    st4(o, make_float4(a.x + t.x, a.y + t.y, a.z + t.z, a.w + t.w));
+  }
+}
+
+}
+
+extern "C" int het_rgat_fold_params(const float* weights, const float* attn_r, const float* loop_w, int64_t num_rels, int64_t H,
+                                    int64_t K, int64_t D, float* wa, float* weights_t, float* loop_wt, het_stream stream) {
+  const char* op = "het_rgat_fold_params";
+  HET_REQUIRE(weights && attn_r && wa && weights_t && (loop_w == nullptr) == (loop_wt == nullptr), "%s: null argument", op);
+  HET_REQUIRE(num_rels > 0 && H > 0 && K > 0 && D > 0 && num_rels * H * K * D < (1ll << 31), "%s: bad sizes", op);
+  const int64_t X = H * D, total = num_rels * H * K * (D + 1) + (loop_w ? X * K : 0);
+  hipLaunchKernelGGL(HET_rgat_fold_params, dim3(grid_for(total)), dim3(kBlock), 0, (hipStream_t)stream, weights, attn_r, loop_w,
+                     (int)(num_rels * H), (int)K, (int)D, (int)X, wa, weights_t, loop_wt);
+  HET_LAUNCH_CHECK("HET_rgat_fold_params");
+  return HET_OK;
+}
+
+extern "C" int het_rgat_fold_params_backward(const float* weights, const float* attn_r, const float* grad_wa, int64_t num_rels,
+                                             int64_t H, int64_t K, int64_t D, float* grad_weights, float* grad_attn_r,
+                                             const float* attn_part, const int32_t* attn_part_rel, int64_t attn_part_rows,
+                                             float* grad_attn_l, het_stream stream) {
+  const char* op = "het_rgat_fold_params_backward";
+  HET_REQUIRE(weights && attn_r && grad_wa && grad_weights && grad_attn_r, "%s: null argument", op);
+  HET_REQUIRE(num_rels > 0 && H > 0 && K > 0 && D > 0 && num_rels * H * K * D < (1ll << 31), "%s: bad sizes", op);
+  const int64_t X = H * D;
+  const bool with_attn = attn_part_rows > 0;
+  HET_REQUIRE(attn_part_rows >= 0 && (!with_attn || (attn_part && attn_part_rel && grad_attn_l && X % kAttnCols == 0 &&
+                                                      aligned16(attn_part, grad_attn_l))),
+              "%s: the partial rows need attn_part, attn_part_rel and grad_attn_l, 16-byte aligned, rows of a multiple of 4 floats", op);
+  const int nb_elem = (int)grid_for(num_rels * H * (K + 1) * D);
+  const int64_t nb_attn = with_attn ? num_rels * (X / kAttnCols) : 0;
+  hipLaunchKernelGGL(HET_rgat_fold_params_backward, dim3((unsigned)(nb_elem + nb_attn)), dim3(kBlock), 0, (hipStream_t)stream, weights,
+                     attn_r, grad_wa, (int)(num_rels * H), (int)K, (int)D, grad_weights, grad_attn_r, nb_elem, attn_part, attn_part_rel,
+                     attn_part_rows, (int)X, grad_attn_l);
+  HET_LAUNCH_CHECK("HET_rgat_fold_params_backward");
+  return HET_OK;
+}
diff --git a/het_amd/kernels.py b/het_amd/kernels.py
--- a/het_amd/kernels.py
+++ b/het_amd/kernels.py
@@ -622,15 +622,29 @@
     return by_dst, by_srow, by_drow, None
 
 
+def rgat_aggregate_compact_prepare(groupings, er_c, sum, ret):
+    assert groupings[3] is not None, "rgat_aggregate_compact_prepare: the run-sum form only"
+    _chk("rgat_aggregate_compact_prepare", (er_c, sum, ret))
+    N, H = sum.shape[0], sum.shape[1]
+    D = ret.numel() // max(1, N * H)
+    q_rows = torch.empty((er_c.shape[0], H, D), dtype=ret.dtype, device=ret.device)
+    q_sum, q_ref = torch.empty_like(er_c), torch.empty_like(er_c)
+    _call(ret, "het_rgat_aggregate_compact_runs_prepare", _p(sum), _p(q_sum), N, er_c.shape[0], H, _stream(ret))
+    return q_rows, q_sum, q_ref
+
+
 def rgat_aggregate_compact(groupings, feat_c, el_c, er_c, sum, ret, slope, h_inout=None, num_rels=None, attn_l=None,
-                           feat_rel_ptrs=None):
+                           feat_rel_ptrs=None, prepared=None):
     _chk("rgat_aggregate_compact", tuple(t for t in (feat_c, el_c, er_c, sum, ret, h_inout) if t is not None))
     N, H = sum.shape[0], sum.shape[1]
     D = ret.numel() // max(1, N * H)
     if groupings[3] is not None:
         S_col = er_c.shape[0]
-        q_rows = torch.empty((S_col, H, D), dtype=ret.dtype, device=ret.device)
-        q_sum, q_ref = torch.empty_like(er_c), torch.empty_like(er_c)
+        if prepared is not None:
+            q_rows, q_sum, q_ref = prepared
+        else:
+            q_rows = torch.empty((S_col, H, D), dtype=ret.dtype, device=ret.device)
+            q_sum, q_ref = torch.empty_like(er_c), torch.empty_like(er_c)
         with torch.cuda.device(ret.device):
             nbytes = int(_lib.lib().het_rgat_aggregate_compact_runs_workspace(groupings[0].handle, groupings[3].handle, int(num_rels), H, D,
                                                                               _stream(ret)))
@@ -642,11 +656,12 @@
             _chk("rgat_aggregate_compact", (attn_l,), (feat_rel_ptrs,))
             lst = _derived_get("rel_ptrs_host", (feat_rel_ptrs,), lambda: feat_rel_ptrs.tolist())
             host_ptrs = (C.c_int64 * len(lst))(*lst)
-        _call(ret, "het_rgat_aggregate_compact_runs", groupings[0].handle, groupings[3].handle, int(num_rels), _p(feat_c), _p(el_c),
+        _call(ret, "het_rgat_aggregate_compact_runs" if prepared is None else "het_rgat_aggregate_compact_runs_prepared", groupings[0].handle, groupings[3].handle, int(num_rels), _p(feat_c), _p(el_c),
               _p(er_c), _p(sum), _p(ret), N, H, D, float(slope), _p(h_inout), 0 if h_inout is None else h_inout.shape[0],
               _p(q_rows), _p(q_sum), _p(q_ref), S_col, _p(attn_l) if host_ptrs is not None else None, host_ptrs, _p(ws), nbytes,
               _stream(ret))
         return q_rows, q_sum, q_ref
+    assert prepared is None, "prepared comes with the run-sum form"
     nbytes = int(_lib.lib().het_rgat_aggregate_compact_workspace(groupings[0].handle, H, D))
     ws = torch.empty((nbytes + 3) // 4, dtype=torch.float32, device=ret.device) if nbytes else None
     _call(ret, "het_rgat_aggregate_compact", groupings[0].handle, _p(feat_c), _p(el_c), _p(er_c), _p(sum), _p(ret), N, H, D,
@@ -752,7 +767,7 @@
 
 def rgat_backward_compact(groupings, feat_c, el_c, er_c, sum, ret, gradout, grad_feat_c, grad_el_c, grad_er_c, slope,
                           fold_attn_l=None, row_rel_ptrs=None, grad_bias=None, bias_rows=0, runs=None, drow_nodes=None,
-                          grad_attn_l=None):
+                          grad_attn_l=None, attn_partials=False):
     _chk("rgat_backward_compact", tuple(t for t in (feat_c, el_c, er_c, sum, ret, gradout, grad_feat_c, grad_el_c, grad_er_c,
                                                     fold_attn_l, grad_bias, grad_attn_l) + (tuple(runs) if runs else ()) if t is not None),
          tuple(t for t in (row_rel_ptrs, drow_nodes) if t is not None))
@@ -772,11 +787,62 @@
             _p(fold_attn_l), _p(row_rel_ptrs), 0 if row_rel_ptrs is None else row_rel_ptrs.numel() - 1, _p(grad_bias),
             int(bias_rows), N, feat_c.shape[0], er_c.shape[0], H, D, float(slope))
     tail = (_p(ws), ws.numel() * 4, _stream(ret))
+    if runs and attn_partials:
+        info = (C.c_int64 * 2)()
+        _call(ret, "het_rgat_backward_compact_runs_partials", groupings[1].handle, _p(runs[0]), _p(runs[1]), _p(runs[2]), _p(drow_nodes),
+              *head, _p(grad_attn_l), *tail[:2], info, tail[2])
+        return ws, int(info[0]), int(info[1])
+    assert not attn_partials, "attn_partials comes with the run-sum form"
     if runs:
         _call(ret, "het_rgat_backward_compact_runs", groupings[1].handle, _p(runs[0]), _p(runs[1]), _p(runs[2]), _p(drow_nodes), *head,
               _p(grad_attn_l), *tail)
     else:
         _call(ret, "het_rgat_backward_compact", groupings[1].handle, groupings[2].handle, *head, *tail)
+
+
+def rgat_fold_params_ok(W, loop_w=None) -> bool:
+    return W.is_cuda and W.dtype == torch.float32 and W.dim() == 4 and (loop_w is None or (loop_w.dtype == torch.float32 and loop_w.dim() == 2))
+
+
+def rgat_fold_params(W, attn_r, loop_w=None, out=None):
+    _chk("rgat_fold_params", tuple(t for t in (W, attn_r, loop_w) if t is not None))
+    R, H, Kd, D = W.shape
+    assert attn_r.numel() == R * H * D and (loop_w is None or loop_w.shape[0] == Kd)
+    if out is None:
+        out = (torch.empty((R, H, Kd), dtype=W.dtype, device=W.device), torch.empty((R, H, D, Kd), dtype=W.dtype, device=W.device),
+               None if loop_w is None else torch.empty((loop_w.shape[1], Kd), dtype=W.dtype, device=W.device))
+    wa, Wt, loop_wt = out
+    _chk("rgat_fold_params", tuple(t for t in out if t is not None))
+    assert (loop_wt is None) == (loop_w is None)
+    _call(W, "het_rgat_fold_params", _p(W), _p(attn_r), _p(loop_w), R, H, Kd, D, _p(wa), _p(Wt), _p(loop_wt), _stream(W))
+    return wa, Wt, loop_wt
+
+
+def rgat_fold_params_backward(W, attn_r, grad_wa, grad_W, grad_attn_r, attn_partials=None, grad_attn_l=None):
+    _chk("rgat_fold_params_backward", tuple(t for t in (W, attn_r, grad_wa, grad_W, grad_attn_r, grad_attn_l) if t is not None))
+    R, H, Kd, D = W.shape
+    assert grad_wa.numel() == R * H * Kd and grad_W.shape == W.shape and grad_attn_r.numel() == R * H * D
+    part = rel = None
+    rows = 0
+    if attn_partials is not None and len(attn_partials) == 3:
+        ws, off, rows = attn_partials
+        if rows:
+            assert grad_attn_l is not None and off + rows * (H * D + 1) * 4 <= ws.numel() * 4
+            part, rel = C.c_void_p(ws.data_ptr() + off), C.c_void_p(ws.data_ptr() + off + rows * H * D * 4)
+    elif attn_partials is not None:
+        pt, rl = attn_partials
+        _chk("rgat_fold_params_backward", (pt,))
+        rows = pt.shape[0]
+        assert grad_attn_l is not None and pt.shape[1] == H * D and rl.dtype == torch.int32 and rl.numel() == rows and rl.is_contiguous()
+        part, rel = _p(pt), _p(rl)
+    _call(W, "het_rgat_fold_params_backward", _p(W), _p(attn_r), _p(grad_wa), R, H, Kd, D, _p(grad_W), _p(grad_attn_r), part, rel, rows,
+          _p(grad_attn_l), _stream(W))
+
+
+def rgat_attn_grad_finish(part, rel, grad_attn_l):
+    _chk("rgat_attn_grad_finish", (part, grad_attn_l))
+    assert rel.dtype == torch.int32 and rel.is_contiguous() and rel.numel() == part.shape[0]
+    _call(part, "het_rgat_attn_grad_finish", _p(part), _p(rel), part.shape[0], part.shape[1], _p(grad_attn_l), _stream(part))
 
 
 def hgt_fold_source_weights(k_lin, v_lin, rel_att, rel_msg, rel_pri, src_type, transpose_att: bool):
diff --git a/include/het_amd.h b/include/het_amd.h
--- a/include/het_amd.h
+++ b/include/het_amd.h
@@ -260,6 +260,12 @@
                                          int64_t num_rels, int64_t H, int64_t dk, int64_t K_in, int transpose_att, float* grad_k_lin,
                                          float* grad_v_lin, float* grad_att, float* grad_msg, float* grad_pri, het_stream stream);
 
+int het_rgat_fold_params(const float* weights, const float* attn_r, const float* loop_w, int64_t num_rels, int64_t H, int64_t K,
+                         int64_t D, float* wa, float* weights_t, float* loop_wt, het_stream stream);
+int het_rgat_fold_params_backward(const float* weights, const float* attn_r, const float* grad_wa, int64_t num_rels, int64_t H,
+                                  int64_t K, int64_t D, float* grad_weights, float* grad_attn_r, const float* attn_part,
+                                  const int32_t* attn_part_rel, int64_t attn_part_rows, float* grad_attn_l, het_stream stream);
+
 int het_rgat_aggregate_compact(const het_grouping* by_dst, const float* feat_c, const float* el_c, const float* er_c,
                                float* sum, float* ret, int64_t num_nodes, int64_t H, int64_t D, double slope,
                                float* h_inout, int64_t h_rows, void* workspace, int64_t workspace_bytes, het_stream stream);
@@ -289,6 +295,25 @@
                                    float* grad_attn_l, void* workspace, int64_t workspace_bytes, het_stream stream);
 int64_t het_rgat_backward_compact_runs_workspace(const het_grouping* by_srow, int64_t num_nodes, int64_t num_dst_rows, int64_t H,
                                                  int64_t D, int with_bias, int with_attn_grad, het_stream stream);
+
+int het_rgat_aggregate_compact_runs_prepare(float* sum, float* q_sum, int64_t num_nodes, int64_t num_dst_rows, int64_t H,
+                                            het_stream stream);
+int het_rgat_aggregate_compact_runs_prepared(const het_grouping* by_dst, const het_grouping* by_dst_rel, int64_t num_rels,
+                                             const float* feat_c, const float* el_c, const float* er_c, float* sum, float* ret,
+                                             int64_t num_nodes, int64_t H, int64_t D, double slope, float* h_inout, int64_t h_rows,
+                                             float* q_rows, float* q_sum, float* q_ref, int64_t num_dst_rows, const float* attn_l,
+                                             const int64_t* feat_rel_ptrs_host, void* workspace, int64_t workspace_bytes,
+                                             het_stream stream);
+int het_rgat_backward_compact_runs_partials(const het_grouping* by_srow, const float* q_rows, const float* q_sum, const float* q_ref,
+                                            const int64_t* drow_nodes, const float* feat_c, const float* el_c, const float* er_c,
+                                            const float* sum, const float* ret, const float* gradout, float* grad_feat_c,
+                                            float* grad_el_c, float* grad_er_c, const float* fold_attn_l, const int64_t* row_rel_ptrs,
+                                            int64_t num_rels, float* grad_bias, int64_t bias_rows, int64_t num_nodes,
+                                            int64_t num_src_rows, int64_t num_dst_rows, int64_t H, int64_t D, double slope,
+                                            float* grad_attn_l, void* workspace, int64_t workspace_bytes, int64_t* attn_part_info,
+                                            het_stream stream);
+int het_rgat_attn_grad_finish(const float* attn_part, const int32_t* attn_part_rel, int64_t attn_part_rows, int64_t X,
+                              float* grad_attn_l, het_stream stream);
 
 int het_rows_matmul_backward_dx(const int64_t* rel_ptrs, int64_t num_rels, const int64_t* gather_idx, const int64_t* g_rows,
                                 int64_t num_rows, const float* weights_t, const float* gradout, float* grad_x, int64_t H,
```

Result: no change. 6064 million edges/s, median of 6 (+0.6%).
